# jasvob/BundleAdjustment_Benchmarks

Hardware: AMD Instinct MI355X
Metric: LM iterations/sec (higher is better)
Workload: dtype f64; 1 GPU; CHOLESKY solver, BAL problem-257-65132 (K=225911) synthetic(seed=1004), f64

## Files before the change

### bundleadjustment_benchmarks_amd/csrc/ba_internal.h

```cpp
#ifndef BA_INTERNAL_H
#define BA_INTERNAL_H

#include "../../include/ba_mi355x.h"

#include <cstdint>
#include <vector>

struct ba_problem {
    int N = 0, M = 0, K = 0;
    std::vector<int> cam_idx, pt_idx;
    std::vector<double> meas;
    std::vector<double> cams9;
    std::vector<double> pts;
};

struct ba_structure {
    int N = 0;
    int M = 0, K = 0;
    int p0 = 0, p1 = 0;
    int o0 = 0, o1 = 0;
    int Ml = 0, Kl = 0;
    bool was_sorted = true;
    std::vector<int> perm;
    std::vector<int> obs_cam, obs_pt;
    std::vector<int> pt_ptr;
    int kmax = 0;
    std::vector<int> qr_pts;
    int qr_bucket_ptr[6] = {0, 0, 0, 0, 0, 0};
    int npairs = 0;
    std::vector<int> pair_hi, pair_lo;
    long long E = 0;
    std::vector<int> ent_r, ent_c;
    int chunk_len = 64;
    int nchunks = 0;
    std::vector<int> chunk_ptr;
    std::vector<int> chunk_pair;
    std::vector<int> pair_chunk_ptr;
    int ndchunks = 0;
    std::vector<int> dchunk_ptr;
    std::vector<int> dchunk_cam;
    std::vector<int> cam_dchunk_ptr;
    std::vector<int> cam_obs;
};

int ba_build_structure(const ba_problem *p, int shard_rank, int shard_world, int chunk_len, int dchunk_len, ba_structure *out, bool pairs = true);

int ba_covisibility(int N, int M, const int *pt_ptr, const int *obs_cam, int track_max, std::vector<int> &pairs, std::vector<int> &weight);


#define BA_CHUNK 64
#define BA_CHUNK_SINGLE (1 << 16)
#define BA_SHARE_CHUNK 256
#define BA_SHARE_LOCAL 8

void ba_plan_eval_ranges(const ba_structure &s, std::vector<int> &eb);

struct ba_schur_plan {
    int grid = 1, nband = 1;
    std::vector<int> wave_ptr;
    std::vector<int> chunk_info;
    std::vector<int> ent;
    std::vector<int> red_pairs;
};
void ba_plan_schur(const ba_structure &s, int wgs_per_cu, int num_cus, int bands, int window, ba_schur_plan &out);

struct ba_forest_plan {
    int ntrees = 0, nodes = 0, kept = 0, dropped = 0, largest = 0, width = 6;
    std::vector<int> tree_ptr, node_cam, node_par ;
    std::vector<int> node_rec;
    std::vector<unsigned char> in_tree;
    std::vector<int> edge_ptr, edge_oo;
};
int ba_plan_forest(const ba_structure &s, const std::vector<int> &rp_pairs, int kind, int max_tree, ba_forest_plan &out);

struct ba_share_plan {
    int nslots = 0, nwide = 0, largest = 0;
    std::vector<int> desc;
    std::vector<int> wide;
};
void ba_plan_share_slots(int ngroups, int nchunks, const int *gptr, const int *cptr, const int *cgrp, ba_share_plan &out);

void ba_plan_relpose_csr(int N, int n, const int *pairs, std::vector<int> &ptr, std::vector<int> &inc);

size_t ba_plan_owner_offsets(int Dp, int nb, int world, std::vector<int> &off);

int ba_rccl_init(void **comm_out, const void *id128, int rank, int world);
void ba_rccl_destroy(void *comm);
int ba_rccl_allreduce(void *comm, void *buf, size_t count, int f64, int op, void *stream);
int ba_rccl_broadcast(void *comm, void *buf, size_t count, int f64, int root, void *stream);
int ba_rccl_reduce_scatter(void *comm, void *buf, size_t count_per_rank, int f64, int rank, void *stream);

#endif
```

### bundleadjustment_benchmarks_amd/csrc/ba_kernels.hip.h

```cpp
#ifndef BA_KERNELS_HIP_H
#define BA_KERNELS_HIP_H

#include <hip/hip_runtime.h>

#include "ba_internal.h"
#include "ba_mfma.hip.h"

#define BA_REC 32
#define BA_REC_DINV 27
#define BA_SLAB 96
#define BA_EPS_PSI 1e-15

__device__ __forceinline__ double tsqrt(double x) { return sqrt(x); }
__device__ __forceinline__ float tsqrt(float x) { return sqrtf(x); }
__device__ __forceinline__ double tsin(double x) { return sin(x); }
__device__ __forceinline__ float tsin(float x) { return sinf(x); }
__device__ __forceinline__ double tcos(double x) { return cos(x); }
__device__ __forceinline__ float tcos(float x) { return cosf(x); }
#ifndef BA_SENTINEL_DEFINED
#define BA_SENTINEL_DEFINED
template <typename T> __device__ __forceinline__ T ba_sentinel();
template <> __device__ __forceinline__ double ba_sentinel<double>() { return __hiloint2double(-1, -1); }
template <> __device__ __forceinline__ float ba_sentinel<float>() { return __int_as_float(-1); }
__device__ __forceinline__ bool ba_is_sentinel(double v) { return __double2hiint(v) == -1 && __double2loint(v) == -1; }
// ... 346 lines not shown
            T U[6] = {0, 0, 0, 0, 0, 0}, g[3] = {0, 0, 0};
            for (int s = 0; s < kk; s++) {
#pragma unroll
                for (int q = 0; q < 6; q++) U[q] += cu[q][tl + s];
#pragma unroll
                for (int q = 0; q < 3; q++) g[q] -= cu[6 + q][tl + s];
            }
#pragma unroll
            for (int q = 0; q < 6; q++) fa.U0[(size_t)q * Ml + pj] = U[q];
#pragma unroll
            for (int q = 0; q < 3; q++) fa.gp[(size_t)q * Ml + pj] = g[q];
            if (FUSE >= 2) {
                const ba_chol3_t<T> c3 = ba_chol3<T>(U[0], U[1], U[2], U[3], U[4], U[5], g[0], g[1], g[2], *fa.lam);
                const size_t M = (size_t)Ml;
                fa.dinv[pj] = c3.i0; fa.dinv[M + pj] = c3.i1; fa.dinv[2 * M + pj] = c3.i2;
                fa.tvec[pj] = c3.t0; fa.tvec[M + pj] = c3.t1; fa.tvec[2 * M + pj] = c3.t2;
                fa.tri[pj] = 1; fa.tri[M + pj] = c3.l10; fa.tri[2 * M + pj] = c3.l20;
                fa.tri[3 * M + pj] = 1; fa.tri[4 * M + pj] = c3.l21; fa.tri[5 * M + pj] = 1;
                pf[0][tl] = c3.l10; pf[1][tl] = c3.l20; pf[2][tl] = c3.l21; pf[3][tl] = c3.i0; pf[4][tl] = c3.i1; pf[5][tl] = c3.i2;
            }
        }
        if constexpr (FUSE >= 2) {
            __syncthreads();
            if constexpr (COOP) {
                static_assert(16 * ba_stage<T, BA_REC>::S <= 9 * 256 / 4 && 16 * ba_stage<T, 20>::S <= 9 * 256 / 4, "a wavefront's image");
                const int w0 = 64 * (tl >> 6), left = b1 - b0 - w0;
                const int nw = __builtin_amdgcn_readfirstlane(left < 0 ? 0 : left > 64 ? 64 : left);
                T *img = &cu[0][0] + (tl >> 6) * (9 * 256 / 4);
                {
                    T a[20];
#pragma unroll
                    for (int q = 0; q < 18; q++) a[q] = Aj[q];
                    a[18] = ej[0]; a[19] = ej[1];
                    ba_store_run<T, 20, 16>(img, a, nw, JcA + (size_t)(b0 + w0) * 20);
                }
                T z[BA_REC];
                if (valid) {
                    const int fl = pfirst - b0;
                    ba_chol_z<T>(Aj, Bj, pf[0][fl], pf[1][fl], pf[2][fl], pf[3][fl], pf[4][fl], pf[5][fl], z);
                }
                ba_store_run<T, BA_REC, 16>(img, z, nw, fa.rec + (size_t)(b0 + w0) * BA_REC);
            } else if (valid) {
                const int fl = pfirst - b0;
                ba_chol_record<T>(Aj, Bj, pf[0][fl], pf[1][fl], pf[2][fl], pf[3][fl], pf[4][fl], pf[5][fl], fa.rec + (size_t)i * BA_REC);
            }
            if (blockIdx.x == 0 && threadIdx.x == 0) *fa.fresh = 1;
        }
    }
}

template <typename T>
__global__ __launch_bounds__(256) void k_stats(int K, int N, int Ml, const T *__restrict__ cam, const T *__restrict__ pts,
                                               const int *__restrict__ obs_cam, const int *__restrict__ obs_pt,
                                               const T *__restrict__ meas, T tau, T *__restrict__ partial )
{
    __shared__ T red[4];
    const int i = blockIdx.x * 256 + threadIdx.x;
    T v0 = 0, v1 = 0, v2 = 0, v3 = 0;
    if (i < K) {
        const int ci = obs_cam[i], pj = obs_pt[i];
        T c[15];
#pragma unroll
        for (int k = 0; k < 15; k++) c[k] = cam[(size_t)k * N + ci];
        const T X0 = pts[pj], X1 = pts[(size_t)Ml + pj], X2 = pts[2 * (size_t)Ml + pj];
        const T XX0 = c[0] * X0 + c[1] * X1 + c[2] * X2 + c[9];
        const T XX1 = c[3] * X0 + c[4] * X1 + c[5] * X2 + c[10];
        const T XX2 = c[6] * X0 + c[7] * X1 + c[8] * X2 + c[11];
        const T xu0 = XX0 / XX2, xu1 = XX1 / XX2;
        const T r2u = xu0 * xu0 + xu1 * xu1;
        const T kr = 1 + c[13] * r2u + c[14] * r2u * r2u;
        const T d0 = c[12] * (kr * xu0) - meas[i], d1 = c[12] * (kr * xu1) - meas[(size_t)K + i];
        const T err = tsqrt(d0 * d0 + d1 * d1);
        const T tau2 = tau * tau, tau4 = tau2 * tau2;
        v0 = err;
        if (err <= tau) { v1 = err; v2 = 1; }
        const T q2 = err, q4 = q2 * q2;
        v3 = (q2 < tau2) ? q2 * ((T)3.0 - (T)3.0 * q2 / tau2 + q4 / tau4) / (T)6.0 : tau2 / (T)6.0;
    }
    v0 = block_reduce<T, false>(v0, red);
    v1 = block_reduce<T, false>(v1, red);
    v2 = block_reduce<T, false>(v2, red);
    v3 = block_reduce<T, false>(v3, red);
    if (threadIdx.x == 0) {
        const size_t g = gridDim.x;
        partial[blockIdx.x] = v0; partial[g + blockIdx.x] = v1; partial[2 * g + blockIdx.x] = v2; partial[3 * g + blockIdx.x] = v3;
    }
}

struct ba_red_job { const void *src; int n; int op; int dst; };
struct ba_red_jobs { ba_red_job j[8]; };

template <typename T> __device__ __forceinline__ void ba_reduce_job(const ba_red_job &jb, T *__restrict__ scal, T *red)
{
    const T *src = (const T *)jb.src;
    T a = 0;
    if (jb.op == 0) {
        for (int k = threadIdx.x; k < jb.n; k += 256) a += src[k];
        a = block_reduce<T, false>(a, red);
    } else {
        for (int k = threadIdx.x; k < jb.n; k += 256) a = tmax(a, src[k]);
        a = block_reduce<T, true>(a, red);
    }
    if (threadIdx.x == 0) scal[jb.dst] = a;
}

template <typename T> __global__ __launch_bounds__(256) void k_reduce_scalars(ba_red_jobs jobs, T *__restrict__ scal, const int *__restrict__ go = nullptr,
                                                                              long long *__restrict__ stamp = nullptr)
{
    __shared__ T red[4];
    if (!(go && *go == 0)) ba_reduce_job<T>(jobs.j[blockIdx.x], scal, red);
    if (stamp && blockIdx.x == 0 && threadIdx.x == 0) *stamp = (long long)wall_clock64();
}

template <typename T>
__device__ __forceinline__ void ba_point_prep_block(int bid, int Ml, int K, const int *__restrict__ pt_ptr, const T *__restrict__ Jp,
                                                    const T *__restrict__ r, T *__restrict__ U0, T *__restrict__ gp, T *__restrict__ partial_dmax)
{
    __shared__ T red[4];
    const int j = bid * 256 + threadIdx.x;
    T dm = 0;
    if (j < Ml) {
        T U[6] = {0, 0, 0, 0, 0, 0}, g[3] = {0, 0, 0};
        const int e = pt_ptr[j + 1];
        for (int i = pt_ptr[j]; i < e; i++) {
            T B[6];
#pragma unroll
            for (int q = 0; q < 6; q++) B[q] = Jp[(size_t)q * K + i];
            const T r0 = r[i], r1 = r[(size_t)K + i];
            T u[9];
            ba_pt_terms<T>(B, r0, r1, u);
#pragma unroll
            for (int q = 0; q < 6; q++) U[q] += u[q];
#pragma unroll
            for (int q = 0; q < 3; q++) g[q] -= u[6 + q];
        }
#pragma unroll
        for (int q = 0; q < 6; q++) U0[(size_t)q * Ml + j] = U[q];
#pragma unroll
        for (int q = 0; q < 3; q++) gp[(size_t)q * Ml + j] = g[q];
        dm = tmax(U[0], tmax(U[3], U[5]));
    }
    dm = block_reduce<T, true>(dm, red);
    if (threadIdx.x == 0) partial_dmax[bid] = dm;
}
template <typename T>
__global__ __launch_bounds__(256) void k_point_prep(int Ml, int K, const int *__restrict__ pt_ptr, const T *__restrict__ Jp,
                                                    const T *__restrict__ r, T *__restrict__ U0, T *__restrict__ gp,
                                                    T *__restrict__ partial_dmax, const int *__restrict__ go = nullptr)
{
    if (go && *go == 0) return;
    ba_point_prep_block<T>(blockIdx.x, Ml, K, pt_ptr, Jp, r, U0, gp, partial_dmax);
}

template <typename T>
__device__ __forceinline__ void ba_cam_gram_block(int bid, int ndchunks, int K, const int *__restrict__ dchunk_ptr, const int *__restrict__ cam_obs,
                                                  const T *__restrict__ JcA, T *__restrict__ dslab)
{
    __shared__ T xch[8][27][33];
    const int gl = threadIdx.x >> 5, g = bid * 8 + gl, sub = threadIdx.x & 31;
    const bool gok = g < ndchunks;
    const int e0 = gok ? dchunk_ptr[g] : 0, len = gok ? dchunk_ptr[g + 1] - e0 : 0;
    T v[54];
#pragma unroll
    for (int q = 0; q < 54; q++) v[q] = 0;
    if (sub < len) {
        const T *rec = JcA + (size_t)cam_obs[e0 + sub] * 20;
        T a0[9], a1[9];
#pragma unroll
        for (int c = 0; c < 9; c++) { a0[c] = rec[c]; a1[c] = rec[9 + c]; }
        const T r0 = rec[18], r1 = rec[19];
        int q = 0;
#pragma unroll
        for (int c = 0; c < 9; c++)
#pragma unroll
            for (int c2 = 0; c2 <= c; c2++) v[q++] = a0[c] * a0[c2] + a1[c] * a1[c2];
#pragma unroll
        for (int c = 0; c < 9; c++) v[45 + c] = -(a0[c] * r0 + a1[c] * r1);
    }
#pragma unroll
    for (int pass = 0; pass < 2; pass++) {
        __syncthreads();
#pragma unroll
        for (int q = 0; q < 27; q++) xch[gl][q][sub] = v[27 * pass + q];
        __syncthreads();
        if (gok && sub < 27) {
            T a = 0;
#pragma unroll
            for (int l = 0; l < 32; l++) a += xch[gl][sub][l];
            dslab[(size_t)g * BA_SLAB + 27 * pass + sub] = a;
        }
    }
}
template <typename T>
__global__ __launch_bounds__(256) void k_cam_gram(int ndchunks, int K, const int *__restrict__ dchunk_ptr,
                                                  const int *__restrict__ cam_obs, const T *__restrict__ JcA,
                                                  T *__restrict__ dslab, const int *__restrict__ go = nullptr)
{
    if (go && *go == 0) return;
    ba_cam_gram_block<T>(blockIdx.x, ndchunks, K, dchunk_ptr, cam_obs, JcA, dslab);
}
template <typename T>
__global__ __launch_bounds__(256) void k_grad_prep(int gM, int Ml, int K, const int *__restrict__ pt_ptr, const T *__restrict__ Jp, const T *__restrict__ r,
                                                   T *__restrict__ U0, T *__restrict__ gp, T *__restrict__ partial_dmax, int ndchunks,
                                                   const int *__restrict__ dchunk_ptr, const int *__restrict__ cam_obs, const T *__restrict__ JcA,
                                                   T *__restrict__ dslab, const int *__restrict__ go = nullptr)
{
    if (go && *go == 0) return;
    if ((int)blockIdx.x < gM) ba_point_prep_block<T>(blockIdx.x, Ml, K, pt_ptr, Jp, r, U0, gp, partial_dmax);
    else ba_cam_gram_block<T>(blockIdx.x - gM, ndchunks, K, dchunk_ptr, cam_obs, JcA, dslab);
}

template <typename T>
__global__ __launch_bounds__(256) void k_cam_gram_reduce(int N, const int *__restrict__ cam_dchunk_ptr,
                                                         const T *__restrict__ dslab, T *__restrict__ V ,
                                                         T *__restrict__ gc , const int *__restrict__ go = nullptr,
                                                         ba_red_job tail = ba_red_job{nullptr, 0, 0, 0}, T *__restrict__ scal = nullptr,
                                                         long long *__restrict__ stamp = nullptr)
{
    __shared__ T red[4];
    if (tail.src && blockIdx.x == gridDim.x - 1) {
        if (!(go && *go == 0)) ba_reduce_job<T>(tail, scal, red);
        if (stamp && threadIdx.x == 0) *stamp = (long long)wall_clock64();
        return;
    }
    if (go && *go == 0) return;
    const int idx = blockIdx.x * 256 + threadIdx.x;
    const int a = idx / BA_SLAB, e = idx - a * BA_SLAB;
    if (a >= N || e >= 54) return;
    T s4[4] = {0, 0, 0, 0};
    const int c0 = cam_dchunk_ptr[a], c1 = cam_dchunk_ptr[a + 1];
    int c = c0;
    for (; c + 15 < c1; c += 16) {
        T x[16];
#pragma unroll
        for (int u = 0; u < 16; u++) x[u] = dslab[(size_t)(c + u) * BA_SLAB + e];
#pragma unroll
        for (int u = 0; u < 16; u++) s4[u & 3] += x[u];
    }
    for (; c + 3 < c1; c += 4) {
#pragma unroll
        for (int u = 0; u < 4; u++) s4[u] += dslab[(size_t)(c + u) * BA_SLAB + e];
    }
    for (; c < c1; c++) s4[0] += dslab[(size_t)c * BA_SLAB + e];
    const T s = (s4[0] + s4[1]) + (s4[2] + s4[3]);
    if (e < 45) {
        int rr = 0;
        while ((rr + 1) * (rr + 2) / 2 <= e) rr++;
        const int cc = e - rr * (rr + 1) / 2;
        V[(size_t)a * 81 + 9 * rr + cc] = s;
        V[(size_t)a * 81 + 9 * cc + rr] = s;
    } else
        gc[9 * a + e - 45] = s;
}

template <typename T> __global__ __launch_bounds__(256) void k_vdiag(int N, const T *__restrict__ V, T *__restrict__ out)
{
    const int c = blockIdx.x * 256 + threadIdx.x;
    if (c < 9 * N) out[c] = V[(size_t)(c / 9) * 81 + 10 * (c % 9)];
}

template <typename T, bool MARQ = false, bool COOP = false>
__global__ __launch_bounds__(256) void k_elim_chol(int K, int Ml, const int *__restrict__ obs_pt, const int *__restrict__ pt_ptr,
                                                   const T *__restrict__ JcA , const T *__restrict__ Jp, const T *__restrict__ U0,
                                                   const T *__restrict__ gp, const T *__restrict__ lam, T *__restrict__ rec,
                                                   T *__restrict__ dinv, T *__restrict__ tvec, T *__restrict__ tri,
                                                   const int *__restrict__ fresh = nullptr ,
                                                   ba_damp_args<T> da = ba_damp_args<T>{})
{
    if (fresh && *fresh != 0) return;
    const int i0 = blockIdx.x * 256 + threadIdx.x;
    if (!COOP && i0 >= K) return;
    const int w0 = (int)blockIdx.x * 256 + (threadIdx.x & 192);
    if (COOP && w0 >= K) return;
    const bool valid = i0 < K;
    const int i = valid ? i0 : K - 1;
    const T lambda = *lam;
    const int j = obs_pt[i];
    const size_t M = (size_t)Ml;
    ba_chol3_t<T> c3;
    if constexpr (MARQ) {
        const T u0 = U0[j], u3 = U0[3 * M + j], u5 = U0[5 * M + j];
        c3 = ba_chol3<T>(u0, U0[M + j], U0[2 * M + j], u3, U0[4 * M + j], u5, gp[j], gp[M + j], gp[2 * M + j],
                         ba_damp<true, T>(lambda, u0, da), ba_damp<true, T>(lambda, u3, da), ba_damp<true, T>(lambda, u5, da));
    } else
        c3 = ba_chol3<T>(U0[j], U0[M + j], U0[2 * M + j], U0[3 * M + j], U0[4 * M + j], U0[5 * M + j],
                         gp[j], gp[M + j], gp[2 * M + j], lambda);
    if (valid && i == pt_ptr[j]) {
        dinv[j] = c3.i0; dinv[M + j] = c3.i1; dinv[2 * M + j] = c3.i2;
        tvec[j] = c3.t0; tvec[M + j] = c3.t1; tvec[2 * M + j] = c3.t2;
        tri[j] = 1; tri[M + j] = c3.l10; tri[2 * M + j] = c3.l20;
        tri[3 * M + j] = 1; tri[4 * M + j] = c3.l21; tri[5 * M + j] = 1;
    }
    T A[18], B[6];
#pragma unroll
    for (int q = 0; q < 6; q++) B[q] = Jp[(size_t)q * K + i];
    {
        typedef T vec_t __attribute__((ext_vector_type(16 / sizeof(T))));
        constexpr int VW = 16 / sizeof(T);
        const vec_t *src = (const vec_t *)(JcA + (size_t)i * 20);
#pragma unroll
        for (int q = 0; q < 20 / VW; q++) {
            const vec_t v = src[q];
#pragma unroll
            for (int u = 0; u < VW; u++)
                if (VW * q + u < 18) A[VW * q + u] = v[u];
        }
    }
    if constexpr (COOP) {
        __shared__ alignas(16) T stage[4][16 * ba_stage<T, BA_REC>::S];
        const int nw = __builtin_amdgcn_readfirstlane(K - w0 > 64 ? 64 : K - w0);
        T z[BA_REC];
        ba_chol_z<T>(A, B, c3.l10, c3.l20, c3.l21, c3.i0, c3.i1, c3.i2, z);
        ba_store_run<T, BA_REC, 16>(stage[threadIdx.x >> 6], z, nw, rec + (size_t)w0 * BA_REC);
    } else
    ba_chol_record<T>(A, B, c3.l10, c3.l20, c3.l21, c3.i0, c3.i1, c3.i2, rec + (size_t)i * BA_REC);
}

template <typename T, int LPP> __device__ __forceinline__ T group_sum(T v)
{
#pragma unroll
    for (int off = LPP / 2; off > 0; off >>= 1) v += __shfl_xor(v, off, LPP);
    return v;
}

template <typename T, int LPP, int SL>
__global__ __launch_bounds__(256) void k_elim_qr(int npts, const int *__restrict__ pt_list, int Ml, int K, const int *__restrict__ pt_ptr,
                                                 const T *__restrict__ Jc, const T *__restrict__ Jp, const T *__restrict__ r,
                                                 const T *__restrict__ lam, T *__restrict__ rec, T *__restrict__ dinv,
                                                 T *__restrict__ tvec, T *__restrict__ tri, const int *__restrict__ go = nullptr,
                                                 T *__restrict__ q1obs = nullptr ,
                                                 T *__restrict__ q1lam = nullptr ,
                                                 int *__restrict__ pperm = nullptr )
{
    if (go && *go == 0) return;
    const int gid = (blockIdx.x * 256 + threadIdx.x) / LPP, lg = threadIdx.x % LPP;
    const int j = pt_list[gid < npts ? gid : npts - 1];
    const int b = pt_ptr[j], k = pt_ptr[j + 1] - b;
    const T sl = tsqrt(*lam);
    T V[SL][6], Q[SL][6];
    bool ok[SL];
#pragma unroll
    for (int s = 0; s < SL; s++) {
// ... 154 lines not shown
        }
    }
    T Ql[3][3] = {{1, 0, 0}, {0, 1, 0}, {0, 0, 1}}, QR[3][3] = {{0, 0, 0}, {0, 0, 0}, {0, 0, 0}};
#pragma unroll
    for (int h = 2; h >= 0; h--)
#pragma unroll
        for (int c = 0; c < 3; c++) {
            const T w = (Ql[h][c] + W[h][0] * QR[0][c] + W[h][1] * QR[1][c] + W[h][2] * QR[2][c]) * tau[h];
            Ql[h][c] -= w;
#pragma unroll
            for (int r = 0; r < 3; r++) QR[r][c] -= W[h][r] * w;
        }
    const T m0 = tvec0[j], m1 = tvec0[(size_t)Ml + j], m2 = tvec0[2 * (size_t)Ml + j];
    T t[3];
#pragma unroll
    for (int c = 0; c < 3; c++) t[c] = QR[0][c] * m0 + QR[1][c] * m1 + QR[2][c] * m2;
    if (i == pt_ptr[j]) {
#pragma unroll
        for (int c = 0; c < 3; c++) { dinv[(size_t)c * Ml + j] = 1; tvec[(size_t)c * Ml + j] = t[c]; }
        tri[j] = Rt[0][0]; tri[(size_t)Ml + j] = Rt[0][1]; tri[2 * (size_t)Ml + j] = Rt[0][2];
        tri[3 * (size_t)Ml + j] = Rt[1][1]; tri[4 * (size_t)Ml + j] = Rt[1][2]; tri[5 * (size_t)Ml + j] = Rt[2][2];
        if (mQl) {
#pragma unroll
            for (int h = 0; h < 3; h++)
#pragma unroll
                for (int c = 0; c < 3; c++) { mQl[9 * (size_t)j + 3 * h + c] = Ql[h][c]; mQR[9 * (size_t)j + 3 * h + c] = QR[h][c]; }
        }
    }
    const T *z = rec0 + (size_t)i * BA_REC;
    T *o = rec + (size_t)i * BA_REC;
#pragma unroll
    for (int c = 0; c < 9; c++) {
        const T a0 = z[3 * c], a1 = z[3 * c + 1], a2 = z[3 * c + 2];
        const T z0 = a0 * QR[0][0] + a1 * QR[1][0] + a2 * QR[2][0], z1 = a0 * QR[0][1] + a1 * QR[1][1] + a2 * QR[2][1],
                z2 = a0 * QR[0][2] + a1 * QR[1][2] + a2 * QR[2][2];
        o[3 * c] = z0; o[3 * c + 1] = z1; o[3 * c + 2] = z2;
    }
    o[BA_REC_DINV] = 1; o[BA_REC_DINV + 1] = 1; o[BA_REC_DINV + 2] = 1;
}

template <typename T>
__global__ __launch_bounds__(256) void k_more_build(int K, int Ml, int D, const int *__restrict__ obs_cam, const int *__restrict__ obs_pt,
                                                    const int *__restrict__ pt_ptr, const T *__restrict__ rec0, const T *__restrict__ rec,
                                                    const T *__restrict__ mQl, const T *__restrict__ mQR, const T *__restrict__ tvec0,
                                                    const T *__restrict__ tvec, T *__restrict__ A, size_t lda)
{
    const int ia = blockIdx.x * 256 + threadIdx.x;
    if (ia >= K) return;
    const int j = obs_pt[ia], a = obs_cam[ia], b = pt_ptr[j], e = pt_ptr[j + 1];
    for (int i2 = b; i2 < ia; i2++)
        if (obs_cam[i2] == a) return;
    const size_t r0 = 6 * (size_t)j;
    T Ql[9], QR[9];
#pragma unroll
    for (int q = 0; q < 9; q++) { Ql[q] = mQl[9 * (size_t)j + q]; QR[q] = mQR[9 * (size_t)j + q]; }
    T z0[27], z[27];
#pragma unroll
    for (int q = 0; q < 27; q++) { z0[q] = rec0[(size_t)ia * BA_REC + q]; z[q] = rec[(size_t)ia * BA_REC + q]; }
    for (int i2 = ia + 1; i2 < e; i2++)
        if (obs_cam[i2] == a) {
#pragma unroll
            for (int q = 0; q < 27; q++) { z0[q] += rec0[(size_t)i2 * BA_REC + q]; z[q] += rec[(size_t)i2 * BA_REC + q]; }
        }
    T *colbase = A + (size_t)(9 * a) * lda + r0;
#pragma unroll
    for (int c = 0; c < 9; c++) {
        const T z_0 = z[3 * c], z_1 = z[3 * c + 1], z_2 = z[3 * c + 2];
#pragma unroll
        for (int rr = 0; rr < 3; rr++) {
            colbase[(size_t)c * lda + rr] = -(Ql[3 * rr] * z_0 + Ql[3 * rr + 1] * z_1 + Ql[3 * rr + 2] * z_2);
            colbase[(size_t)c * lda + 3 + rr] = z0[3 * c + rr] - (QR[3 * rr] * z_0 + QR[3 * rr + 1] * z_1 + QR[3 * rr + 2] * z_2);
        }
    }
    if (ia == pt_ptr[j]) {
        const size_t M = (size_t)Ml;
        const T m0 = tvec0[j], m1 = tvec0[M + j], m2 = tvec0[2 * M + j], t0 = tvec[j], t1 = tvec[M + j], t2 = tvec[2 * M + j];
        const T mq[3] = {m0, m1, m2};
        T *rhs = A + (size_t)D * lda + r0;
#pragma unroll
        for (int rr = 0; rr < 3; rr++) {
            rhs[rr] = -(Ql[3 * rr] * t0 + Ql[3 * rr + 1] * t1 + Ql[3 * rr + 2] * t2);
            rhs[3 + rr] = mq[rr] - (QR[3 * rr] * t0 + QR[3 * rr + 1] * t1 + QR[3 * rr + 2] * t2);
        }
    }
}
template <typename T>
__global__ __launch_bounds__(256) void k_more_tail(int Ml, int D, const T *__restrict__ R22buf, const T *__restrict__ lam, T *__restrict__ A, size_t lda)
{
    const int c = blockIdx.x;
    const size_t rR = 6 * (size_t)Ml, rL = rR + (size_t)D;
    const int top = c < D ? c : D - 1;
    for (int i = threadIdx.x; i <= top; i += 256) A[(size_t)c * lda + rR + i] = R22buf[(size_t)c * D + i];
    if (c < D && threadIdx.x == 0) A[(size_t)c * lda + rL + c] = tsqrt(*lam);
}
template <typename T>
__global__ __launch_bounds__(256) void k_copy_r22(int D, const T *__restrict__ A, size_t lda, T *__restrict__ R22buf, const int *__restrict__ go)
{
    if (go && *go == 0) return;
    const int c = blockIdx.x;
    const int top = c < D ? c : D - 1;
    for (int i = threadIdx.x; i < D; i += 256) R22buf[(size_t)c * D + i] = i <= top ? A[(size_t)c * lda + i] : (T)0;
}

template <typename T>
__global__ __launch_bounds__(256) void k_dbg_resid(int rows, int D, const T *__restrict__ A, size_t lda, const T *__restrict__ y, T *__restrict__ r)
{
    const int i = blockIdx.x * 256 + threadIdx.x;
    if (i >= rows) return;
    T a = A[(size_t)D * lda + i];
    for (int c = 0; c < D; c++) a -= A[(size_t)c * lda + i] * y[c];
    r[i] = a;
}
template <typename T>
__global__ __launch_bounds__(256) void k_dbg_atv(int rows, int D, const T *__restrict__ A, size_t lda, const T *__restrict__ v, T *__restrict__ out)
{
    __shared__ T red[4];
    const int c = blockIdx.x;
    T a = 0;
    for (int r = threadIdx.x; r < rows; r += 256) a += A[(size_t)c * lda + r] * v[r];
    a = block_reduce<T, false>(a, red);
    if (threadIdx.x == 0) out[c] = a;
}

typedef int ba_v2i __attribute__((ext_vector_type(2)));
__device__ __forceinline__ double ba_bufload(__amdgpu_buffer_rsrc_t r, unsigned off, const double *)
{
    return __builtin_bit_cast(double, __builtin_amdgcn_raw_buffer_load_b64(r, (int)off, 0, 0));
}
__device__ __forceinline__ float ba_bufload(__amdgpu_buffer_rsrc_t r, unsigned off, const float *)
{
    return __builtin_bit_cast(float, __builtin_amdgcn_raw_buffer_load_b32(r, (int)off, 0, 0));
}
typedef int ba_v4i __attribute__((ext_vector_type(4)));
__device__ __forceinline__ void ba_bufload3(__amdgpu_buffer_rsrc_t r, unsigned off, double &x0, double &x1, double &x2)
{
    const ba_v4i lo = __builtin_amdgcn_raw_buffer_load_b128(r, (int)off, 0, 0);
    const ba_v2i hi = __builtin_amdgcn_raw_buffer_load_b64(r, (int)(off + 16), 0, 0);
    x0 = __builtin_bit_cast(double, ba_v2i{lo.x, lo.y});
    x1 = __builtin_bit_cast(double, ba_v2i{lo.z, lo.w});
    x2 = __builtin_bit_cast(double, hi);
}
__device__ __forceinline__ void ba_bufload3(__amdgpu_buffer_rsrc_t r, unsigned off, float &x0, float &x1, float &x2)
{
    x0 = ba_bufload(r, off, (const float *)nullptr);
    x1 = ba_bufload(r, off + 4, (const float *)nullptr);
    x2 = ba_bufload(r, off + 8, (const float *)nullptr);
}
template <typename T, bool SCALED >
__global__ __launch_bounds__(256) __attribute__((amdgpu_waves_per_eu(4))) void k_schur_pairs(const int *__restrict__ wave_ptr, int nband, const int4 *__restrict__ chunk_info,
                                                     const int2 *__restrict__ ent, const T *__restrict__ rec, unsigned rec_bytes,
                                                     const T *__restrict__ tvec, int Ml, T *__restrict__ slab, const T *__restrict__ V,
                                                     const T *__restrict__ gc, int D, int ld, T *__restrict__ S)
{
    const int lane = threadIdx.x & 63;
    const int wq = ((blockIdx.x % nband) * (gridDim.x / nband) + blockIdx.x / nband) * 4 + (threadIdx.x >> 6);
    int slot = wave_ptr[wq];
    const int slot1 = wave_ptr[wq + 1];
    if (slot >= slot1) return;
    const __amdgpu_buffer_rsrc_t rsrc = __builtin_amdgcn_make_buffer_rsrc(const_cast<T *>(rec), 0, (int)rec_bytes, 0x00020000);
    constexpr unsigned SZ = sizeof(T), RB = BA_REC * SZ, OOB = 0xfffffff0u - 64 * SZ;
    const int i = lane & 15, k = lane >> 4;
    const bool la = i < 9;
    const unsigned lane_off = 3 * i * SZ;
    typedef typename ba_acc<T>::type acc_t;
    auto entry_of = [&](const int4 ci) {
        const int n = ci.y & 0xffff;
        return ent[ci.x + (lane < n ? lane : n - 1)];
    };
    int4 ci0 = chunk_info[slot];
    int4 ci1 = chunk_info[min(slot + 1, slot1 - 1)];
    int2 en0 = entry_of(ci0);
    for (; slot < slot1; slot++) {
        const int2 en1 = entry_of(ci1);
        const int4 ci2 = chunk_info[min(slot + 2, slot1 - 1)];
        const int n = ci0.y & 0xffff;
        const int hi = ci0.z & 0xffff, lo = (unsigned)ci0.z >> 16, g = ci0.w;
        const bool diag = hi == lo;
        const int ia_l = en0.x, ib_l = en0.y;
        acc_t acc;
#pragma unroll
        for (int v = 0; v < 4; v++) acc[v] = 0;
        constexpr int GB = 2;
        struct batch_t { T a[3 * GB], d[3 * GB], b[3 * GB]; };
        auto fetch = [&](int t0, batch_t &o) {
#pragma unroll
            for (int u = 0; u < GB; u++) {
                const int e = 4 * (t0 + u) + k;
                const bool ok = e < n;
                const int es = ok ? e : n - 1;
                const int ia = __shfl(ia_l, es, 64), ibr = __shfl(ib_l, es, 64);
                const bool self = ibr < 0;
                const unsigned ra = (unsigned)ia * RB, rb = (unsigned)(self ? ia : ibr) * RB;
                const unsigned oa = (ok && la) ? ra + lane_off : OOB, ob = (ok && la) ? rb + lane_off : OOB;
                const unsigned od = (ok && la) ? ra + BA_REC_DINV * SZ : OOB;
                ba_bufload3(rsrc, oa, o.a[3 * u], o.a[3 * u + 1], o.a[3 * u + 2]);
                if (SCALED) ba_bufload3(rsrc, od, o.d[3 * u], o.d[3 * u + 1], o.d[3 * u + 2]);
                ba_bufload3(rsrc, ob, o.b[3 * u], o.b[3 * u + 1], o.b[3 * u + 2]);
                if (diag && i == 9 && ok && self) {
#pragma unroll
                    for (int m = 0; m < 3; m++) o.b[3 * u + m] = tvec[(size_t)m * Ml + (~ibr)];
                }
            }
        };
        auto multiply = [&](const batch_t &o) {
#pragma unroll
            for (int q = 0; q < 3 * GB; q++) acc = ba_mfma(SCALED ? o.a[q] * o.d[q] : o.a[q], o.b[q], acc);
        };
        const int ngroups = (n + 3) >> 2;
        batch_t b0, b1;
        fetch(0, b0);
        for (int t0 = 0;;) {
            if (t0 + GB < ngroups) fetch(t0 + GB, b1);
            multiply(b0);
            t0 += GB;
            if (t0 >= ngroups) break;
            if (t0 + GB < ngroups) fetch(t0 + GB, b0);
            multiply(b1);
            t0 += GB;
            if (t0 >= ngroups) break;
        }
        if (ci0.y & BA_CHUNK_SINGLE) {
#pragma unroll
            for (int v = 0; v < 4; v++) {
                const int r = ba_crow<T>(k, v);
                if (r >= 9) continue;
                if (i < 9) {
                    T val = -acc[v];
                    if (diag) val += V[(size_t)hi * 81 + 9 * r + i];
                    S[(size_t)(9 * lo + i) * ld + 9 * hi + r] = val;
                } else if (i == 9 && diag) {
                    const T gg = gc[9 * hi + r];
                    S[(size_t)(9 * hi + r) * ld + D] = gg - acc[v];
                    S[(size_t)(9 * hi + r) * ld + D + 1] = gg;
                }
            }
        } else {
            T *o = slab + (size_t)g * BA_SLAB;
#pragma unroll
            for (int v = 0; v < 4; v++) {
                const int r = ba_crow<T>(k, v);
                if (r >= 9) continue;
                if (i < 9) o[9 * r + i] = acc[v];
                else if (i == 9) o[81 + r] = acc[v];
            }
        }
        ci0 = ci1; ci1 = ci2; en0 = en1;
    }
}

template <typename T, bool MARQ = false>
__global__ __launch_bounds__(192) void k_schur_reduce(int nred, const int *__restrict__ red_pairs, int D, int ld, const int *__restrict__ pair_hi,
                                                      const int *__restrict__ pair_lo, const int *__restrict__ pair_chunk_ptr,
                                                      const T *__restrict__ slab, const T *__restrict__ V,
                                                      const T *__restrict__ gc, T *__restrict__ S, const T *__restrict__ lam = nullptr,
                                                      int post_blocks = 0, int Dp = 0, T *__restrict__ gc_out = nullptr, T *__restrict__ xarm = nullptr,
                                                      ba_damp_args<T> da = ba_damp_args<T>{})
{
    if (post_blocks && blockIdx.x >= gridDim.x - post_blocks) {
        const int c = (blockIdx.x - (gridDim.x - post_blocks)) * 3 + (threadIdx.x >> 6), lane = threadIdx.x & 63;
        if (c >= Dp) return;
        T *col = S + (size_t)c * ld;
        if (lane == 0) {
            xarm[c] = ba_sentinel<T>();
            xarm[Dp + c] = ba_sentinel<T>();
            if (c < D) gc_out[c] = gc[c];
        }
        if (c < D) {
            for (int rr = D + 1 + lane; rr < Dp; rr += 64) col[rr] = 0;
        } else {
            for (int rr = c + lane; rr < Dp; rr += 64) col[rr] = (rr == c) ? (T)1 : (T)0;
        }
        return;
    }
    const int idx = blockIdx.x * 192 + threadIdx.x;
    const int q = idx / BA_SLAB, e = idx - q * BA_SLAB;
    if (q >= nred || e >= 90) return;
    const int p = red_pairs[q];
    const int hi = pair_hi[p], lo = pair_lo[p];
    if (e >= 81 && hi != lo) return;
    T s4[4] = {0, 0, 0, 0};
    const int c1 = pair_chunk_ptr[p + 1];
    int c = pair_chunk_ptr[p];
    for (; c + 15 < c1; c += 16) {
        T x[16];
#pragma unroll
        for (int u = 0; u < 16; u++) x[u] = slab[(size_t)(c + u) * BA_SLAB + e];
#pragma unroll
        for (int u = 0; u < 16; u++) s4[u & 3] += x[u];
    }
    for (; c + 3 < c1; c += 4) {
#pragma unroll
        for (int u = 0; u < 4; u++) s4[u] += slab[(size_t)(c + u) * BA_SLAB + e];
    }
    for (; c < c1; c++) s4[0] += slab[(size_t)c * BA_SLAB + e];
    const T s = (s4[0] + s4[1]) + (s4[2] + s4[3]);
    if (e < 81) {
        const int rr = e / 9, cc = e - 9 * rr;
        T v = -s;
        if (hi == lo) v += V[(size_t)hi * 81 + e];
        if constexpr (MARQ) { if (lam && hi == lo && rr == cc) v += ba_damp<true, T>(*lam, V[(size_t)hi * 81 + e], da); }
        else if (lam && hi == lo && rr == cc) v += *lam;
        S[(size_t)(9 * lo + cc) * ld + 9 * hi + rr] = v;
    } else {
        const int cc = e - 81;
        const T g = gc[9 * hi + cc];
        S[(size_t)(9 * hi + cc) * ld + D] = g - s;
        if (!lam) S[(size_t)(9 * hi + cc) * ld + D + 1] = g;
    }
}

template <typename T, bool MARQ = false>
__global__ __launch_bounds__(256) void k_post_reduce(int D, int Dp, int ld, const T *__restrict__ lam, T *__restrict__ S, T *__restrict__ gc_out,
                                                     T *__restrict__ xarm, const T *__restrict__ V = nullptr, ba_damp_args<T> da = ba_damp_args<T>{})
{
    const int c = blockIdx.x * 4 + (threadIdx.x >> 6), lane = threadIdx.x & 63;
    if (c >= Dp) return;
    T *col = S + (size_t)c * ld;
    if (lane == 0) {
        xarm[c] = ba_sentinel<T>();
        xarm[Dp + c] = ba_sentinel<T>();
    }
    if (c < D) {
        if (lane == 0) {
            col[c] += ba_damp<MARQ, T>(*lam, MARQ ? V[(size_t)(c / 9) * 81 + 10 * (c % 9)] : (T)0, da);
            gc_out[c] = col[D + 1];
        }
        for (int rr = D + 1 + lane; rr < Dp; rr += 64) col[rr] = 0;
    } else {
        for (int rr = c + lane; rr < Dp; rr += 64) col[rr] = (rr == c) ? (T)1 : (T)0;
    }
}

template <typename T, bool UNPACK>
__global__ __launch_bounds__(256) void k_pack_lower(int Dp, int ld, T *__restrict__ S, T *__restrict__ buf, size_t ntail, T *__restrict__ scal,
                                                    int eloc, int etot)
{
    if (blockIdx.x == 0 && blockIdx.y == 0 && threadIdx.x == 0) {
        if (UNPACK) scal[etot] = buf[ntail];
        else buf[ntail] = scal[eloc];
    }
    const int c = blockIdx.y;
    const int p = c >> 6, r0 = p << 6;
    const int h = Dp - r0;
    const size_t off = (size_t)64 * ((size_t)p * Dp - (size_t)32 * p * (p - 1)) + (size_t)(c - r0) * h;
    for (int r = blockIdx.x * 256 + threadIdx.x; r < h; r += gridDim.x * 256) {
        if (UNPACK) S[(size_t)c * ld + r0 + r] = buf[off + r];
        else buf[off + r] = S[(size_t)c * ld + r0 + r];
    }
}

template <typename T, bool UNPACK>
__global__ __launch_bounds__(256) void k_pack_owner(int Dp, int D, int ld, T *__restrict__ S, T *__restrict__ buf, const int *__restrict__ own_off,
                                                    int world, int rank, size_t small, T *__restrict__ scal, int eloc, int etot)
{
    const int c = blockIdx.y;
    const int p = c >> 6, r0 = p << 6;
    const int h = Dp - r0;
    if (blockIdx.x == 0 && threadIdx.x == 0) {
        if (c == 0) { if (UNPACK) scal[etot] = buf[small + D]; else buf[small + D] = scal[eloc]; }
        if (c < D) { if (UNPACK) S[(size_t)c * ld + D + 1] = buf[small + c]; else buf[small + c] = S[(size_t)c * ld + D + 1]; }
    }
    if (UNPACK && p % world != rank) return;
    const size_t off = (size_t)64 * (size_t)own_off[p] + (size_t)(c - r0) * h;
    for (int r = blockIdx.x * 256 + threadIdx.x; r < h; r += gridDim.x * 256) {
        if (UNPACK) { if (r0 + r != D + 1 || c >= D) S[(size_t)c * ld + r0 + r] = buf[off + r]; }
        else buf[off + r] = S[(size_t)c * ld + r0 + r];
    }
}

template <typename T, int NB, bool UNSTAGE>
__global__ __launch_bounds__(256) void k_panel_stage(int h, int p0, int ld, T *__restrict__ S, T *__restrict__ Wp, T *__restrict__ Winv, T *__restrict__ stage)
{
    const int y = blockIdx.y;
    if (y == 2 * NB) {
        for (int q = blockIdx.x * 256 + threadIdx.x; q < NB * NB; q += gridDim.x * 256) {
            if (UNSTAGE) Winv[q] = stage[(size_t)2 * h * NB + q]; else stage[(size_t)2 * h * NB + q] = Winv[q];
        }
        return;
    }
    const int j = y < NB ? y : y - NB;
    T *src = (y < NB ? S + (size_t)(p0 + j) * ld : Wp + (size_t)j * ld) + p0;
    T *dst = stage + (size_t)(y < NB ? 0 : h * NB) + (size_t)j * h;
    for (int r = blockIdx.x * 256 + threadIdx.x; r < h; r += gridDim.x * 256) {
        if (UNSTAGE) src[r] = dst[r]; else dst[r] = src[r];
    }
}

struct ba_cam_retract_args { int N; const void *cam, *dxc, *gc; void *cam_test, *scal; int dst; };
struct ba_fix_args { const unsigned short *cmask; const unsigned char *pfix; };
template <typename T> struct ba_damp_diag { const T *U0, *V; ba_damp_args<T> da; };
template <typename T, bool MASK = false, bool MARQ = false>
__device__ __forceinline__ void ba_retract_cams(int N, const T *__restrict__ cam, const T *__restrict__ dxc, const T *__restrict__ gc,
                                                const T *__restrict__ lam, T *__restrict__ cam_test, T *__restrict__ scal, int dst, T *red,
                                                const unsigned short *__restrict__ cmask = nullptr, ba_damp_diag<T> dg = ba_damp_diag<T>{});

template <typename T, int LPP, bool MASK = false, bool MARQ = false>
__global__ __launch_bounds__(256) void k_backsub(int Ml, const int *__restrict__ pt_ptr, const int *__restrict__ obs_cam,
                                                 const T *__restrict__ rec, const T *__restrict__ dinv, const T *__restrict__ tvec,
                                                 const T *__restrict__ tri, const T *__restrict__ dxc, const T *__restrict__ gp,
                                                 const T *__restrict__ pts, const T *__restrict__ lam, T *__restrict__ dxp, T *__restrict__ pts_test,
// ... 3 lines not shown
{
    __shared__ T red[4];
    if (cr.N > 0 && (int)blockIdx.x == npart) {
        ba_retract_cams<T, MASK, MARQ>(cr.N, (const T *)cr.cam, (const T *)cr.dxc, (const T *)cr.gc, lam, (T *)cr.cam_test, (T *)cr.scal, cr.dst, red,
                                       fx.cmask, dg);
        return;
    }
    const int gid = (blockIdx.x * 256 + threadIdx.x) / LPP, lg = threadIdx.x % LPP;
    const int j = gid < Ml ? gid : Ml - 1;
    const int b = pt_ptr[j], e = pt_ptr[j + 1];
    T s0 = 0, s1 = 0, s2 = 0;
    for (int i = b + lg; i < e; i += LPP) {
        const T *Z = rec + (size_t)i * BA_REC;
        const int ci = obs_cam[i];
        const T *dc = dxc + 9 * ci;
        const unsigned cm = MASK ? (unsigned)fx.cmask[ci] : 0u;
#pragma unroll
        for (int c = 0; c < 9; c++) {
            const T d = (MASK && ((cm >> c) & 1u)) ? (T)0 : dc[c];
            s0 += Z[3 * c] * d; s1 += Z[3 * c + 1] * d; s2 += Z[3 * c + 2] * d;
        }
    }
    s0 = group_sum<T, LPP>(s0); s1 = group_sum<T, LPP>(s1); s2 = group_sum<T, LPP>(s2);
    T rho = 0, dn = 0;
    if (gid < Ml && lg == 0 && b == e) {
        dxp[j] = 0; dxp[(size_t)Ml + j] = 0; dxp[2 * (size_t)Ml + j] = 0;
        pts_test[j] = pts[j]; pts_test[(size_t)Ml + j] = pts[(size_t)Ml + j]; pts_test[2 * (size_t)Ml + j] = pts[2 * (size_t)Ml + j];
    } else if (gid < Ml && lg == 0) {
        const T lambda = *lam;
        const T u0 = (tvec[j] - s0) * dinv[j], u1 = (tvec[(size_t)Ml + j] - s1) * dinv[(size_t)Ml + j],
                u2 = (tvec[2 * (size_t)Ml + j] - s2) * dinv[2 * (size_t)Ml + j];
        const T y2 = u2 / tri[5 * (size_t)Ml + j];
        const T y1 = (u1 - tri[4 * (size_t)Ml + j] * y2) / tri[3 * (size_t)Ml + j];
        const T y0 = (u0 - tri[(size_t)Ml + j] * y1 - tri[2 * (size_t)Ml + j] * y2) / tri[j];
        const int pp = pperm[j], q0 = pp & 3, q1 = (pp >> 2) & 3;
        T x0 = q0 == 0 ? y0 : q1 == 0 ? y1 : y2, x1 = q0 == 1 ? y0 : q1 == 1 ? y1 : y2, x2 = q0 == 2 ? y0 : q1 == 2 ? y1 : y2;
        const bool pfixed = MASK && fx.pfix[j] != 0;
        if (pfixed) { x0 = 0; x1 = 0; x2 = 0; }
        dxp[j] = x0; dxp[(size_t)Ml + j] = x1; dxp[2 * (size_t)Ml + j] = x2;
        pts_test[j] = pfixed ? pts[j] : pts[j] + x0;
        pts_test[(size_t)Ml + j] = pfixed ? pts[(size_t)Ml + j] : pts[(size_t)Ml + j] + x1;
        pts_test[2 * (size_t)Ml + j] = pfixed ? pts[2 * (size_t)Ml + j] : pts[2 * (size_t)Ml + j] + x2;
        if constexpr (MARQ) {
            const T d0 = ba_damp<true, T>(lambda, dg.U0[j], dg.da), d1 = ba_damp<true, T>(lambda, dg.U0[3 * (size_t)Ml + j], dg.da),
                    d2 = ba_damp<true, T>(lambda, dg.U0[5 * (size_t)Ml + j], dg.da);
            rho = x0 * (d0 * x0 + gp[j]) + x1 * (d1 * x1 + gp[(size_t)Ml + j]) + x2 * (d2 * x2 + gp[2 * (size_t)Ml + j]);
        } else
        rho = x0 * (lambda * x0 + gp[j]) + x1 * (lambda * x1 + gp[(size_t)Ml + j]) + x2 * (lambda * x2 + gp[2 * (size_t)Ml + j]);
        dn = x0 * x0 + x1 * x1 + x2 * x2;
    }
    rho = block_reduce<T, false>(rho, red);
    dn = block_reduce<T, false>(dn, red);
    if (threadIdx.x == 0) { partial[blockIdx.x] = rho; partial[npart + blockIdx.x] = dn; }
}

template <typename T, bool MASK, bool MARQ>
__device__ __forceinline__ void ba_retract_cams(int N, const T *__restrict__ cam, const T *__restrict__ dxc,
                                                const T *__restrict__ gc, const T *__restrict__ lam, T *__restrict__ cam_test,
                                                T *__restrict__ scal, int dst, T *red, const unsigned short *__restrict__ cmask,
                                                ba_damp_diag<T> dg)
{
    const T lambda = *lam;
    T rho = 0, dn = 0;
    for (int a = threadIdx.x; a < N; a += 256) {
        T p[9];
        const unsigned cm = MASK ? (unsigned)cmask[a] : 0u;
#pragma unroll
        for (int c = 0; c < 9; c++) {
            p[c] = dxc[9 * a + c];
            if (MASK && ((cm >> c) & 1u)) {
                p[c] = 0;
                ((T *)dxc)[9 * a + c] = 0;
            }
            if constexpr (MARQ) rho += p[c] * (ba_damp<true, T>(lambda, dg.V[(size_t)a * 81 + 10 * c], dg.da) * p[c] + gc[9 * a + c]);
            else rho += p[c] * (lambda * p[c] + gc[9 * a + c]);
            dn += p[c] * p[c];
        }
        T R0[9];
#pragma unroll
        for (int c = 0; c < 9; c++) R0[c] = cam[(size_t)c * N + a];
        const T th = tsqrt(p[3] * p[3] + p[4] * p[4] + p[5] * p[5]);
        T dR[9] = {1, 0, 0, 0, 1, 0, 0, 0, 1};
        if (th > (T)1e-6) {
            const T J[9] = {0, -p[5], p[4], p[5], 0, -p[3], -p[4], p[3], 0};
            const T c1 = tsin(th) / th, c2 = ((T)1.0 - tcos(th)) / (th * th);
#pragma unroll
            for (int rr = 0; rr < 3; rr++)
#pragma unroll
                for (int cc = 0; cc < 3; cc++) {
                    T j2 = 0;
#pragma unroll
                    for (int k = 0; k < 3; k++) j2 += J[3 * rr + k] * J[3 * k + cc];
                    dR[3 * rr + cc] = dR[3 * rr + cc] + c1 * J[3 * rr + cc] + c2 * j2;
                }
        }
        if (MASK && (cm & 0x38u)) {
#pragma unroll
            for (int c = 0; c < 9; c++) cam_test[(size_t)c * N + a] = R0[c];
        } else {
#pragma unroll
        for (int rr = 0; rr < 3; rr++)
#pragma unroll
            for (int cc = 0; cc < 3; cc++) {
                T s = 0;
#pragma unroll
                for (int k = 0; k < 3; k++) s += dR[3 * rr + k] * R0[3 * k + cc];
                cam_test[(size_t)(3 * rr + cc) * N + a] = s;
            }
        }
        if constexpr (MASK) {
#pragma unroll
            for (int c = 0; c < 9; c++) {
                if (c >= 3 && c < 6) continue;
                const size_t o = (size_t)(c < 3 ? 9 + c : 6 + c) * N + a;
                cam_test[o] = ((cm >> c) & 1u) ? cam[o] : cam[o] + p[c];
            }
        } else {
#pragma unroll
        for (int c = 0; c < 3; c++) cam_test[(size_t)(9 + c) * N + a] = cam[(size_t)(9 + c) * N + a] + p[c];
        cam_test[(size_t)12 * N + a] = cam[(size_t)12 * N + a] + p[6];
        cam_test[(size_t)13 * N + a] = cam[(size_t)13 * N + a] + p[7];
        cam_test[(size_t)14 * N + a] = cam[(size_t)14 * N + a] + p[8];
        }
    }
    rho = block_reduce<T, false>(rho, red);
    dn = block_reduce<T, false>(dn, red);
    if (threadIdx.x == 0) { scal[dst] = rho; scal[dst + 1] = dn; }
}

template <typename T, bool MASK = false, bool MARQ = false>
__global__ __launch_bounds__(256) void k_retract_cams(int N, const T *__restrict__ cam, const T *__restrict__ dxc,
                                                      const T *__restrict__ gc, const T *__restrict__ lam, T *__restrict__ cam_test,
                                                      T *__restrict__ scal, int dst, const unsigned short *__restrict__ cmask = nullptr,
                                                      ba_damp_diag<T> dg = ba_damp_diag<T>{})
{
    __shared__ T red[4];
    ba_retract_cams<T, MASK, MARQ>(N, cam, dxc, gc, lam, cam_test, scal, dst, red, cmask, dg);
}

#define BA_LM_RING 64
#define BA_DEV_FAILED (-100)
template <typename T> struct ba_lm_dev {
    T lambda, lambda_inc, energy, hist0, hist1;
    T lam_min, lam_max, tol_fun, inc_base;
    int iter, trials, fun_evals, status, stop;
    int go;
    int fresh;
    int max_iter, max_fun_ev, max_trials, deverr;
    long long t_ctl, t_end;
    int timed;
    int prev_go;
    int prev_code;
    int rec_fresh;
};
struct ba_lm_row { double iter, accepted, f, rho, lambda, lambda_used, e_test, dx_norm, trial_ticks, ctl_ticks_prev, prev_go, stop; };
struct ba_lm_host { int done, stop, status, pad; ba_lm_row rows[BA_LM_RING]; };
struct ba_lm_slots { int energy, etest, rho_p, rho_c, dn_p, dn_c, lambda, err, guard, world; };

#define BA_LM_JOBS 3
template <typename T>
__global__ __launch_bounds__(256 * BA_LM_JOBS) void k_lm_control(T *__restrict__ scal, ba_lm_dev<T> *__restrict__ lm, ba_lm_host *__restrict__ host,
                                                                 ba_lm_slots sl, ba_red_jobs jobs, int njobs)
{
    if (njobs > 0) {
        __shared__ T red[BA_LM_JOBS][4];
        const int q = threadIdx.x >> 8, t = threadIdx.x & 255;
        T a = 0;
        if (q < njobs) {
            const T *src = (const T *)jobs.j[q].src;
            for (int k = t; k < jobs.j[q].n; k += 256) a += src[k];
        }
        a = wave_reduce<T, false>(a);
        if ((t & 63) == 0) red[q][t >> 6] = a;
        __syncthreads();
        if (threadIdx.x == 0)
            for (int j = 0; j < njobs; j++) scal[jobs.j[j].dst] = ((red[j][0] + red[j][1]) + red[j][2]) + red[j][3];
    }
    if (threadIdx.x != 0) return;
    const long long now = (long long)wall_clock64();
    ba_lm_dev<T> s = *lm;
    if (s.stop) {
        if (s.go) lm->go = 0;
        return;
    }
    if (s.fresh) {
        s.energy = scal[sl.energy];
        s.fresh = 0;
        s.fun_evals++;
    }
    const T e_test = scal[sl.etest];
    const T rs = scal[sl.rho_p] + scal[sl.rho_c];
    const T dn = scal[sl.dn_p] + scal[sl.dn_c];
    s.fun_evals++;
    const int t = s.trials++;
    const T lam_used = s.lambda;
    ba_lm_row row;
    row.trial_ticks = s.timed ? (double)(now - s.t_end) : -1.0;
    row.ctl_ticks_prev = s.timed ? (double)(s.t_end - s.t_ctl) : -1.0;
    row.prev_go = s.prev_go;
    s.t_ctl = now;
    s.timed = 1;
    row.iter = s.iter; row.f = (double)s.energy; row.lambda_used = (double)lam_used; row.e_test = (double)e_test; row.dx_norm = sqrt((double)dn);
    int go = 0;
    bool failed = false;
    if (scal[sl.guard] != (T)(sl.world * s.prev_code)) {
        s.deverr = BA_DEVERR_DIVERGED;
        failed = true;
    } else if (scal[sl.err] != (T)0) {
        s.deverr = scal[sl.err] >= (T)BA_DEVERR_SWEEP ? BA_DEVERR_SWEEP : BA_DEVERR_ROW_FLAG;
        failed = true;
    }
    scal[sl.err] = 0;
    if (failed) {
        s.status = BA_DEV_FAILED;
        s.stop = 1;
        row.accepted = 0; row.rho = 0; row.lambda = (double)s.lambda;
    } else if (e_test < s.energy) {
        const T rho = (s.energy - e_test) / rs;
        const T tmv = (T)2.0 * rho - (T)1.0;
        const T mul = (T)1.0 - tmv * tmv * tmv;
        const T third = (T)1.0 / (T)3.0;
        s.lambda *= (mul > third ? mul : third);
        s.lambda = s.lambda > s.lam_min ? s.lambda : s.lam_min;
        row.accepted = 1; row.rho = (double)rho; row.lambda = (double)s.lambda;
        s.lambda_inc = s.inc_base;
        s.energy = e_test;
        if (s.iter % 2) s.hist1 = s.energy; else s.hist0 = s.energy;
        const T maxf = s.hist0 > s.hist1 ? s.hist0 : s.hist1;
        const T diff = s.energy > maxf ? s.energy - maxf : maxf - s.energy;
        if (s.iter > 2 && diff < s.tol_fun * s.energy) {
            s.status = 0;
            s.stop = 1;
        } else {
            go = 1;
            s.iter++;
            s.fresh = 1;
            if (s.iter > s.max_iter) { s.status = 3; s.stop = 1; }
            else if (s.fun_evals > s.max_fun_ev) { s.status = 2; s.stop = 1; }
        }
    } else {
        row.accepted = 0; row.rho = 0; row.lambda = (double)s.lambda;
        if (s.lambda > s.lam_max) { s.status = 1; s.stop = 1; }
        else {
            s.lambda *= s.lambda_inc;
            s.lambda_inc = sizeof(T) == 8 ? (T)pow((double)s.lambda_inc, 1.5) : (T)powf((float)s.lambda_inc, 1.5f);
        }
    }
    if (!s.stop && s.max_trials > 0 && s.trials >= s.max_trials) { s.stop = 1; s.status = -1; }
    s.go = go;
    s.prev_go = go;
    s.prev_code = (row.accepted != 0 ? 1 : 0) + 2 * (s.stop != 0 ? 1 : 0);
    scal[sl.guard] = (T)s.prev_code;
    scal[sl.lambda] = s.lambda;
    row.stop = failed ? 2.0 : (s.stop ? 1.0 : 0.0);
    s.rec_fresh = 0;
    *lm = s;
    host->rows[t % BA_LM_RING] = row;
    host->stop = s.stop;
    host->status = s.status;
    __threadfence_system();
    __hip_atomic_store(&host->done, t + 1, __ATOMIC_RELEASE, __HIP_MEMORY_SCOPE_SYSTEM);
}

__global__ void k_spin(long long ticks)
{
    const long long t0 = (long long)wall_clock64();
    while ((long long)wall_clock64() - t0 < ticks) __builtin_amdgcn_s_sleep(64);
}

template <typename T>
__global__ __launch_bounds__(256) void k_commit(int ncam, int npts, const T *__restrict__ cam_test, const T *__restrict__ pts_test,
                                                T *__restrict__ cam, T *__restrict__ pts, const int *__restrict__ go)
{
    if (go && *go == 0) return;
    const int idx = blockIdx.x * 256 + threadIdx.x;
    if (idx < ncam) cam[idx] = cam_test[idx];
    else if (idx - ncam < npts) pts[idx - ncam] = pts_test[idx - ncam];
}

#endif
```

### bundleadjustment_benchmarks_amd/csrc/ba_solver.hip

```cpp
#include "ba_internal.h"
#include "ba_kernels.hip.h"
#include "ba_dense.hip.h"
#include "ba_qr.hip.h"
#include "ba_pcg.hip.h"
#include "ba_cov.hip.h"
#include "ba_pcg_multi.hip.h"
#include "ba_pcg_share.hip.h"
#include "ba_prior.hip.h"
#include "ba_relpose.hip.h"

#include <algorithm>
#include <chrono>
#include <cmath>
#include <cstdio>
#include <cstdlib>
#include <cstring>
#include <new>
#include <numeric>
#include <string>
#include <type_traits>

#define HIPCHK(x)                                                                                   \
    do {                                                                                            \
        hipError_t e_ = (x);                                                                        \
        if (e_ != hipSuccess) {                                                                     \
            fprintf(stderr, "ba_mi355x: %s failed: %s (%s:%d)\n", #x, hipGetErrorString(e_), __FILE__, __LINE__); \
            return BA_ERR_HIP;                                                                      \
        }                                                                                           \
    } while (0)

namespace {

constexpr int NB = BA_NB;
constexpr int NAUG = 3;
constexpr int NSCAL = 24;
enum { SC_ENERGY = 0, SC_DMAX_P = 1, SC_ETEST = 2, SC_RHO_P = 3, SC_DN_P = 4,
       SC_GUARD = 5 ,
       SC_ERR = 6 ,
       SC_DMAX_C = 7, SC_ST0 = 8 , SC_LAMBDA = 12 ,
       SC_ZERO = 13 ,
       SC_ELOC = 15 ,
       SC_RHO_C = 16, SC_DN_C = 17 };
constexpr int N_STEP_SCALARS = 5;
enum { EV_T0 = 0, EV_T1, EV_T2, EV_T3, EV_T4, EV_T5, EV_T6, EV_L0, EV_L1, EV_N };
constexpr int RING_EV = 8;
constexpr int RING_NE = 6;

template <typename F> void with_flag(bool b, F &&f)
{
    if (b) f(std::bool_constant<true>{});
    else f(std::bool_constant<false>{});
}
template <typename F> void with_flags(bool a, bool b, F &&f)
{
    with_flag(a, [&](auto A) { with_flag(b, [&](auto B) { f(A, B); }); });
}
template <int V> using int_c = std::integral_constant<int, V>;

template <typename T> struct DevBuf {
    T *p = nullptr;
    size_t n = 0;
    int alloc(size_t count)
    {
        n = count;
        if (count == 0) return BA_OK;
        hipError_t e = hipMalloc((void **)&p, sizeof(T) * count);
        if (e != hipSuccess) { p = nullptr; return e == hipErrorOutOfMemory ? BA_ERR_NOMEM : BA_ERR_HIP; }
        return BA_OK;
    }
    int upload(const std::vector<T> &h)
    {
        int rc = alloc(h.size());
        if (rc) return rc;
        if (!h.empty() && hipMemcpy(p, h.data(), sizeof(T) * h.size(), hipMemcpyHostToDevice) != hipSuccess) return BA_ERR_HIP;
        return BA_OK;
    }
    int upload_ints(const std::vector<int> &h)
    {
        static_assert(sizeof(T) % sizeof(int) == 0 && std::is_trivially_copyable<T>::value, "not a record of ints");
        int rc = alloc(h.size() / (sizeof(T) / sizeof(int)));
        if (rc) return rc;
        if (!h.empty() && hipMemcpy(p, h.data(), sizeof(int) * h.size(), hipMemcpyHostToDevice) != hipSuccess) return BA_ERR_HIP;
        return BA_OK;
    }
    void release()
    {
        if (p) (void)hipFree(p);
        p = nullptr; n = 0;
    }
    void swap(DevBuf &o) { std::swap(p, o.p); std::swap(n, o.n); }
    ~DevBuf() { release(); }
};

struct SolverBase {
    virtual ~SolverBase() {}
    virtual int init(const ba_problem *p, ba_solver_kind kind, int rank, int world) = 0;
    virtual int linearize(double *energy, double *diag_max) = 0;
    virtual int try_step(double lambda, double *e_test, double *rho_scale, double *dx_norm) = 0;
    virtual int accept() = 0;
    virtual int stats(double *out4) = 0;
    virtual int get(int what, double *out, size_t n) = 0;
    virtual int set_state(const double *cam15, const double *pts) = 0;
    virtual void set_stream_hook() {}
    virtual int minimize(const ba_lm_params *lm, ba_trial_cb cb, void *user, ba_result *out) = 0;
    virtual int time_phase(int phase, int reps, double lambda, double *ms) = 0;
    virtual int selftest(int which) = 0;
    virtual int set_pcg(int max_iter, double rel_tol) = 0;
    virtual int pcg_stats(ba_pcg_stats *out, int reset) = 0;
    virtual int set_pcg_model_tol(double eta) = 0;
    virtual int pcg_stop_stats(ba_pcg_stop_stats *out, int reset) = 0;
    virtual int set_damping(int kind, double diag_min, double diag_max) = 0;
    virtual int get_damping(int *kind, double *diag_min, double *diag_max) = 0;
    virtual int set_precond(int kind, int max_tree) = 0;
    virtual int precond_info(long long *out6, int *fallback_trees) = 0;
    virtual int set_shared(const int *group_of) = 0;
    virtual int shared_info(long long *out4) = 0;
    virtual int set_constant(const unsigned short *cam_mask, const unsigned char *pt_fixed) = 0;
    virtual int set_loss(int kind, double scale) = 0;
    virtual int set_obs_weights(const double *w) = 0;
    virtual int set_priors(int type, int n, const int *ids, const double *x0, const double *info) = 0;
    virtual int prior_energy(double *out3) = 0;
    virtual int set_relposes(int n, const int *pairs, const double *R0, const double *t0, const double *Lr, const double *Lt) = 0;
    virtual int relpose_energy(double *out2) = 0;
    virtual size_t device_bytes() const = 0;
    virtual int cov_compute(double lambda) = 0;
    virtual int cov_get(int n_pairs, const int *cam_pairs, double *cam_cov, int n_pts, const int *pt_ids, double *pt_cov) = 0;
    virtual int cov_timing(double *ms4) = 0;
    virtual int cov_pcg(double lambda, int max_iter, double rel_tol, int n_pairs, const int *cam_pairs, double *cam_cov, int n_pts, const int *pt_ids,
                        double *pt_cov, ba_cov_pcg_stats *stats) = 0;
    bool poisoned = false;
    int recoveries = 0;
    ba_allreduce_fn ar_fn = nullptr;
    void *ar_user = nullptr;
    void *comm = nullptr;
    hipStream_t st = nullptr;
    bool own_stream = false;
    bool keep = false;
    ba_structure sx;
    ba_timing tm{};
    int rank = 0, world = 1;
};

template <typename T> void host_rodrigues(const T *om, T *R)
{
    const T th = std::sqrt(om[0] * om[0] + om[1] * om[1] + om[2] * om[2]);
    for (int i = 0; i < 9; i++) R[i] = (i % 4 == 0) ? (T)1 : (T)0;
    if (std::fabs(th) > (T)1e-6) {
        const T J[9] = {0, -om[2], om[1], om[2], 0, -om[0], -om[1], om[0], 0};
        T J2[9];
        for (int i = 0; i < 3; i++)
            for (int j = 0; j < 3; j++) {
                T a = 0;
                for (int k = 0; k < 3; k++) a += J[i * 3 + k] * J[k * 3 + j];
                J2[i * 3 + j] = a;
            }
        const T c1 = std::sin(th) / th, c2 = ((T)1.0 - std::cos(th)) / (th * th);
        for (int i = 0; i < 9; i++) R[i] = R[i] + c1 * J[i] + c2 * J2[i];
    }
}

template <typename T> struct Solver final : SolverBase {
    ba_solver_kind kind = BA_CHOLESKY;
    int N = 0, D = 0, Dp = 0, ld = 0, Ml = 0, Kl = 0;
    T tau = (T)0.5;
    DevBuf<int> d_obs_cam, d_obs_pt, d_pt_ptr, d_pair_hi, d_pair_lo, d_pair_chunk_ptr,
        d_dchunk_ptr, d_cam_dchunk_ptr, d_cam_obs, d_qr_pts, d_flags, d_pperm ;
    DevBuf<int4> d_chunk_info;
    DevBuf<int2> d_ent;
    DevBuf<int> d_wave_ptr;
    DevBuf<int> d_red_pairs;
    int schur_window = 0;
    int nred = 0;
    bool no_fold = false;
    bool rec_coop = true;
    int schur_grid = 1, schur_wgs = 4 , schur_bands = 8, schur_nband = 1;
    DevBuf<T> d_r, d_Jc, d_Jp, d_JcA, d_U0, d_gp, d_V, d_gc, d_rec0, d_dinv0, d_tvec0, d_tri0;
    DevBuf<T> d_cam[2], d_pts[2], d_meas, d_gcg, d_dslab, d_rec, d_dinv, d_tvec, d_tri,
        d_slab, d_S, d_pack, d_Skeep, d_Wp, d_Winv, d_dxc, d_dxp, d_part_e, d_part_pm, d_part_bs, d_part_st, d_scal;
    DevBuf<ba_lm_dev<T>> d_lm;
    DevBuf<T> d_qA, d_qtau, d_q1obs, d_q1lam;
    size_t q_lda = 0, q_tau_stride = 0;
    hipStream_t st_qr = nullptr;
    hipEvent_t ev_qr[2] = {nullptr, nullptr};
    ba_qr_side qr_side() const
    {
        ba_qr_side sd;
        sd.st2 = st_qr; sd.ev_chunk = ev_qr[0]; sd.ev_apply = ev_qr[1];
        return sd;
    }
    int q_rows = 0;
    bool more_qr_on = true;
    bool dense_qr() const { return kind == BA_QRKIT || kind == BA_QRSPQR || more_qr(); }
    bool chol_elim() const { return kind == BA_CHOLESKY || kind == BA_ITERSCHUR; }
    bool iterative() const { return kind == BA_ITERSCHUR; }
    bool more_qr() const { return kind == BA_MOREQR && more_qr_on; }
    DevBuf<T> d_mQl, d_mQR, d_R22;
    int outer_rows() const { return 2 * Kl + 3 * Ml + D; }
    int inner_rows() const { return more_qr() ? 6 * Ml + 2 * D : outer_rows(); }
    DevBuf<T> d_qB;
    size_t qb_ld() const { return (size_t)world * D + 64; }
    size_t qb_nmat() const { return qb_ld() * (size_t)(D + 1); }
    size_t qb_count() const { return qb_nmat() + (size_t)D + 1; }
    ba_lm_host *h_log = nullptr, *d_log = nullptr;
    T h_scal[NSCAL];
    T *h_lam = nullptr;
    hipGraphExec_t g_trial = nullptr, g_a = nullptr, g_b = nullptr, g_ctl = nullptr;
    bool use_graph = true;
    hipEvent_t ev[EV_N] = {};
    struct EvSlot { hipEvent_t e[RING_NE]; };
    EvSlot ring[RING_EV] = {};
    int gK = 0, gM = 0, gB = 0;
    int gE = 0;
    bool fuse = false;
    DevBuf<int> d_eb;
    bool have_step = false;
    bool step_level = false;
    int num_cus = 256;
    double wall_khz = 1e5;
    bool safe_factor = false;
    ba_ldlt_plan ldlt_plan;
    DevBuf<int> d_ldlt_jobs;
    int fault_rowflag = 0;
    double spin_next_s = 0;
    double watchdog_s = 600;

    ~Solver() override
    {
        if (poisoned) return;
        for (auto &e : ev)
            if (e) (void)hipEventDestroy(e);
        for (auto &sl : ring)
            for (auto &e : sl.e)
                if (e) (void)hipEventDestroy(e);
        drop_trial_graphs();
        if (h_lam) (void)hipHostFree(h_lam);
        if (h_log) (void)hipHostFree((void *)h_log);
        if (comm) ba_rccl_destroy(comm);
        if (own_stream && st) (void)hipStreamDestroy(st);
        if (st_qr) (void)hipStreamDestroy(st_qr);
        for (hipEvent_t e : ev_qr) if (e) (void)hipEventDestroy(e);
    }

    int init(const ba_problem *p, ba_solver_kind k, int rk, int wd) override
    {
        kind = k; rank = rk; world = wd;
        more_qr_on = !(getenv("BA_MOREQR_QR") != nullptr && atoi(getenv("BA_MOREQR_QR")) == 0);
        if (iterative() && wd > 1) return BA_ERR_ARG;
        int rc = ba_build_structure(p, rk, wd, BA_CHUNK, 32 , &sx,  !iterative());
        if (rc) return rc;
        N = p->N; D = 9 * N; Ml = sx.Ml; Kl = sx.Kl;
        Dp = ((D + NAUG + NB - 1) / NB) * NB;
        ld = Dp + 64;
        gK = (Kl + 255) / 256; gM = (Ml + 255) / 256;
        if (gK < 1) gK = 1;
        if (gM < 1) gM = 1;
        gB = (int)(((size_t)Ml * 8 + 255) / 256);
        if (gB < 1) gB = 1;
        gE = gK;
        std::vector<int> eb;
        ba_plan_eval_ranges(sx, eb);
        if (!eb.empty()) {
            gE = (int)eb.size() - 1;
            if ((rc = d_eb.upload(eb))) return rc;
            fuse = getenv("BA_NO_FUSE") == nullptr;
        }
        if (!chol_elim() && sx.kmax > 1024) return BA_ERR_ARG;
        if (!st) { HIPCHK(hipStreamCreateWithFlags(&st, hipStreamNonBlocking)); own_stream = true; }
        for (auto &e : ev) HIPCHK(hipEventCreate(&e));
        for (auto &sl : ring)
            for (auto &e : sl.e) HIPCHK(hipEventCreate(&e));
        HIPCHK(hipHostMalloc((void **)&h_lam, sizeof(T)));
        HIPCHK(hipHostMalloc((void **)&h_log, sizeof(ba_lm_host), hipHostMallocMapped | hipHostMallocCoherent));
        memset((void *)h_log, 0, sizeof(ba_lm_host));
        HIPCHK(hipHostGetDevicePointer((void **)&d_log, (void *)h_log, 0));
        use_graph = getenv("BA_NO_GRAPH") == nullptr;
        no_fold = getenv("BA_NO_FOLD") != nullptr;
        rec_coop = getenv("BA_REC_PLAIN") == nullptr;
        dbg_qrcheck = getenv("BA_DBG_QRCHECK") != nullptr;
        dist_factor = getenv("BA_DIST_FACTOR") != nullptr && atoi(getenv("BA_DIST_FACTOR")) != 0;
        if (const char *wd = getenv("BA_WATCHDOG_S")) { const double v = atof(wd); if (v > 0) watchdog_s = v; }
        {
            int dev = 0;
            hipDeviceProp_t pr;
            if (hipGetDevice(&dev) == hipSuccess && hipGetDeviceProperties(&pr, dev) == hipSuccess && pr.multiProcessorCount > 0)
                num_cus = pr.multiProcessorCount;
            int khz = 0;
            if (hipDeviceGetAttribute(&khz, hipDeviceAttributeWallClockRate, dev) == hipSuccess && khz > 0) wall_khz = khz;
        }
#define UP(buf, vec) if ((rc = buf.upload(vec))) return rc
        UP(d_obs_cam, sx.obs_cam); UP(d_obs_pt, sx.obs_pt); UP(d_pt_ptr, sx.pt_ptr); UP(d_pair_hi, sx.pair_hi);
        UP(d_pair_lo, sx.pair_lo);
        UP(d_pair_chunk_ptr, sx.pair_chunk_ptr); UP(d_dchunk_ptr, sx.dchunk_ptr); UP(d_cam_dchunk_ptr, sx.cam_dchunk_ptr);
        UP(d_cam_obs, sx.cam_obs); UP(d_qr_pts, sx.qr_pts);
#undef UP
        if (!iterative()) {
            if ((unsigned long long)Kl * BA_REC * sizeof(T) > (256ull << 20)) { schur_wgs = 2; schur_window = 1; }
            if (const char *ev = getenv("BA_SCHUR_WGS")) schur_wgs = std::max(1, std::min(8, atoi(ev)));
            if (const char *ev = getenv("BA_SCHUR_BANDS")) schur_bands = atoi(ev);
            if (const char *ev = getenv("BA_SCHUR_WINDOW")) schur_window = std::max(0, atoi(ev));
            if (N > 65535) return BA_ERR_ARG;
            if ((unsigned long long)Kl * BA_REC * sizeof(T) >= 0xf0000000ull) return BA_ERR_ARG;
            {
                int nb = 0;
                const hipError_t oe = kind == BA_CHOLESKY ? hipOccupancyMaxActiveBlocksPerMultiprocessor(&nb, k_schur_pairs<T, true>, 256, 0)
                                                          : hipOccupancyMaxActiveBlocksPerMultiprocessor(&nb, k_schur_pairs<T, false>, 256, 0);
                if (oe == hipSuccess && nb >= 1) schur_wgs = std::min(schur_wgs, nb);
            }
            ba_schur_plan sp;
            ba_plan_schur(sx, schur_wgs, num_cus, schur_bands, schur_window, sp);
            schur_grid = sp.grid; schur_nband = sp.nband;
            if ((rc = d_wave_ptr.upload(sp.wave_ptr))) return rc;
            nred = (int)sp.red_pairs.size();
            if ((rc = d_red_pairs.upload(sp.red_pairs))) return rc;
            static_assert(sizeof(int4) == 4 * sizeof(int) && sizeof(int2) == 2 * sizeof(int), "ba_schur_plan: 4 ints per chunk, 2 per entry");
            if ((rc = d_chunk_info.upload_ints(sp.chunk_info)) || (rc = d_ent.upload_ints(sp.ent))) return rc;
        }
        std::vector<T> cam((size_t)15 * N), pts((size_t)3 * (Ml > 0 ? Ml : 1)), meas((size_t)2 * (Kl > 0 ? Kl : 1));
        for (int i = 0; i < N; i++) {
            const double *c = &p->cams9[9 * (size_t)i];
            T om[3] = {(T)c[0], (T)c[1], (T)c[2]}, R[9];
            host_rodrigues<T>(om, R);
            for (int q = 0; q < 9; q++) cam[(size_t)q * N + i] = R[q];
            for (int q = 0; q < 3; q++) cam[(size_t)(9 + q) * N + i] = (T)c[3 + q];
            const T f = (T)c[6], k1 = (T)c[7], k2 = (T)c[8], f2 = f * f;
            cam[(size_t)12 * N + i] = -f / (T)1.0;
            cam[(size_t)13 * N + i] = k1 * f2;
            cam[(size_t)14 * N + i] = k2 * f2 * f2;
        }
        for (int j = 0; j < Ml; j++)
            for (int q = 0; q < 3; q++) pts[(size_t)q * Ml + j] = (T)p->pts[3 * (size_t)(sx.p0 + j) + q];
        for (int i = 0; i < Kl; i++) {
            const int src = sx.perm[sx.o0 + i];
            meas[i] = (T)p->meas[2 * (size_t)src];
            meas[(size_t)Kl + i] = (T)p->meas[2 * (size_t)src + 1];
        }
        if ((rc = d_cam[0].upload(cam)) || (rc = d_cam[1].upload(cam)) || (rc = d_pts[0].upload(pts)) ||
            (rc = d_pts[1].upload(pts)) || (rc = d_meas.upload(meas)))
            return rc;
        const size_t K1 = Kl > 0 ? Kl : 1, M1 = Ml > 0 ? Ml : 1;
#define AL(buf, n) if ((rc = buf.alloc(n))) return rc
        AL(d_r, 2 * K1); if (!chol_elim()) AL(d_Jc, 18 * K1);  AL(d_JcA, 20 * K1); AL(d_Jp, 6 * K1); AL(d_U0, 6 * M1); AL(d_gp, 3 * M1);
        AL(d_V, (size_t)81 * N); AL(d_gc, (size_t)D);
        if (kind == BA_MOREQR) { AL(d_rec0, (size_t)BA_REC * K1); AL(d_dinv0, 3 * M1); AL(d_tvec0, 3 * M1); AL(d_tri0, 6 * M1); }
        if ((rc = d_lm.alloc(1))) return rc;
        if ((rc = d_pperm.upload(std::vector<int>(M1, 0 | (1 << 2) | (2 << 4))))) return rc;
        if (dense_qr()) {
            {
                int dev = 0, lim = 0;
                HIPCHK(hipGetDevice(&dev));
                HIPCHK(hipDeviceGetAttribute(&lim, hipDeviceAttributeMaxSharedMemoryPerBlock, dev));
                if (sizeof(T) * ((size_t)D + 64 + 64 * 64) > (size_t)lim) return BA_ERR_ARG;
            }
            {
                const char *ev = getenv("BA_QR_HW_SQRT");
                const int on = ev ? atoi(ev) : 0;
                HIPCHK(hipMemcpyToSymbol(HIP_SYMBOL(ba_qr_hw_sqrt_flag), &on, sizeof(int)));
            }
            q_rows = std::max(outer_rows(), inner_rows());
            if (more_qr()) { AL(d_mQl, 9 * M1); AL(d_mQR, 9 * M1); AL(d_R22, (size_t)D * (D + 1)); }
            if (!getenv("BA_QR_ONE_STREAM")) {
                HIPCHK(hipStreamCreateWithFlags(&st_qr, hipStreamNonBlocking));
                for (auto &e : ev_qr) HIPCHK(hipEventCreateWithFlags(&e, hipEventDisableTiming));
            }
            q_lda = (size_t)q_rows + 64;
            q_tau_stride = (size_t)((std::max(q_rows, world * D) + ba_qr_cfg<T>::CH - 1) / ba_qr_cfg<T>::CH + 2) * BA_QR_PB * BA_QR_PB;
            AL(d_qA, q_lda * (size_t)(D + 1)); AL(d_qtau, BA_QR_TAU_LEVELS * q_tau_stride); AL(d_q1obs, 6 * K1); AL(d_q1lam, 9 * M1);
            if (world > 1) AL(d_qB, qb_count());
        }
        AL(d_gcg, (size_t)D); AL(d_dslab, (size_t)BA_SLAB * (sx.ndchunks > 0 ? sx.ndchunks : 1));
        AL(d_rec, (size_t)BA_REC * K1); AL(d_dinv, 3 * M1); AL(d_tvec, 3 * M1); AL(d_tri, 6 * M1);
        if (iterative()) {
            pcg_gc = (N + 255) / 256; pcg_gq = (int)(((size_t)9 * N + 255) / 256);
            if (pcg_gc < 1) pcg_gc = 1;
            if (pcg_gq < 1) pcg_gq = 1;
            AL(d_dxc, (size_t)D); AL(d_dxp, 3 * M1);
            AL(d_pcg_M, (size_t)81 * N); AL(d_pcg_b, (size_t)D); AL(d_pcg_r, (size_t)D); AL(d_pcg_z, (size_t)D); AL(d_pcg_p, (size_t)D);
            AL(d_pcg_y, (size_t)D); AL(d_pcg_w, 3 * M1);
            if ((rc = d_pcg_part.alloc((size_t)6 * pcg_gc + 2 * (size_t)pcg_gq))) return rc;
            if ((rc = d_pcg.alloc(1))) return rc;
            HIPCHK(hipMemset(d_pcg.p, 0, sizeof(ba_pcg_dev)));
        } else {
            AL(d_slab, (size_t)BA_SLAB * (sx.nchunks > 0 ? sx.nchunks : 1));
            AL(d_S, (size_t)ld * (Dp + 64)); AL(d_Wp, (size_t)ba_ldlt_wp_panels(D, NB) * ld * NB);  AL(d_Winv, (size_t)((D + NB - 1) / NB) * NB * NB); AL(d_dxc, (size_t)2 * Dp + 2 * NB);  AL(d_dxp, 3 * M1);
            if ((rc = d_flags.alloc((size_t)Dp / NB + 2))) return rc;
            ldlt_plan = ba_ldlt_make_plan(D + 1, D, NB);
            if ((rc = d_ldlt_jobs.upload(ldlt_plan.jobs))) return rc;
            ldlt_plan.d_jobs = d_ldlt_jobs.p;
        }
        AL(d_part_e, (size_t)gE); AL(d_part_pm, (size_t)gM);
        AL(d_part_bs, (size_t)2 * gB); AL(d_part_st, (size_t)4 * gK); AL(d_scal, NSCAL);
#undef AL
        if (d_S.p) HIPCHK(hipMemset(d_S.p, 0, sizeof(T) * d_S.n));
        if (d_Wp.p) HIPCHK(hipMemset(d_Wp.p, 0, sizeof(T) * d_Wp.n));
        HIPCHK(hipMemset(d_scal.p, 0, sizeof(T) * NSCAL));
        HIPCHK(hipMemset(d_dxc.p, 0, sizeof(T) * d_dxc.n));
        HIPCHK(hipMemset(d_part_bs.p, 0, sizeof(T) * d_part_bs.n));
        HIPCHK(hipMemset(d_part_e.p, 0, sizeof(T) * d_part_e.n));
        HIPCHK(hipMemset(d_part_pm.p, 0, sizeof(T) * d_part_pm.n));
        HIPCHK(hipDeviceSynchronize());
        return BA_OK;
    }

    int allreduce(void *buf, size_t count, int op)
    {
        if (world <= 1 && !comm) return BA_OK;
        if (comm) return ba_rccl_allreduce(comm, buf, count, sizeof(T) == 8, op, (void *)st);
        if (!ar_fn) return BA_ERR_COMM;
        return ar_fn(ar_user, buf, count, sizeof(T) == 8 ? BA_F64 : BA_F32, op, (void *)st) ? BA_ERR_COMM : BA_OK;
    }
    bool sharded() const { return world > 1 || comm != nullptr; }
    int bcast(void *buf, size_t count, int root)
    {
        if (world <= 1 && !comm) return BA_OK;
        if (comm) return ba_rccl_broadcast(comm, buf, count, sizeof(T) == 8, root, (void *)st);
        if (!ar_fn) return BA_ERR_COMM;
        return ar_fn(ar_user, buf, count, sizeof(T) == 8 ? BA_F64 : BA_F32, BA_OP_BCAST | (root << 8), (void *)st) ? BA_ERR_COMM : BA_OK;
    }
    int reduce_scatter(void *buf, size_t count_per_rank)
    {
        if (world <= 1 && !comm) return BA_OK;
        if (comm) return ba_rccl_reduce_scatter(comm, buf, count_per_rank, sizeof(T) == 8, rank, (void *)st);
        if (!ar_fn) return BA_ERR_COMM;
        return ar_fn(ar_user, buf, count_per_rank, sizeof(T) == 8 ? BA_F64 : BA_F32, BA_OP_REDUCE_SCATTER, (void *)st) ? BA_ERR_COMM : BA_OK;
    }

    int fetch_scalars()
    {
        HIPCHK(hipMemcpyAsync(h_scal, d_scal.p, sizeof(T) * NSCAL, hipMemcpyDeviceToHost, st));
        HIPCHK(hipStreamSynchronize(st));
        return check_device_error();
    }

    int check_device_error()
    {
        if (h_scal[SC_ERR] == (T)0) return BA_OK;
        report_device_error((int)h_scal[SC_ERR]);
        h_scal[SC_ERR] = 0;
        (void)hipMemsetAsync(d_scal.p + SC_ERR, 0, sizeof(T), st);
        return BA_ERR_HIP;
    }
    static void report_device_error(int code)
    {
        fprintf(stderr, "ba_mi355x: device error %d: %s\n", code,
                code == BA_DEVERR_DIVERGED ? "k_lm_control: the shards did not take the same accept / stop decision"
                : code >= BA_DEVERR_SWEEP  ? "k_ldlt_backflow: an unknown of the backward sweep was never published"
                                           : "k_ldlt_step: the look-ahead update of a row block was never announced");
    }

    double ev_ms(hipEvent_t a, hipEvent_t b)
    {
        float ms = 0;
        if (hipEventElapsedTime(&ms, a, b) != hipSuccess) return 0;
        return ms;
    }
    double ev_ms(int a, int b) { return ev_ms(ev[a], ev[b]); }

    void launch_eval(bool jac, int which, const int *go = nullptr, bool commit = false, bool fused = false)
    {
        const T tau2 = loss_scale * loss_scale;
        ba_fuse_args<T> fa{};
        fa.eb = d_eb.p;
        fa.pt_ptr = d_pt_ptr.p; fa.lam = d_scal.p + SC_LAMBDA; fa.U0 = d_U0.p; fa.gp = d_gp.p;
        fa.rec = d_rec.p; fa.dinv = d_dinv.p; fa.tvec = d_tvec.p; fa.tri = d_tri.p; fa.fresh = &d_lm.p->rec_fresh;
        fa.cmask = d_cmask.p; fa.pfix = d_pfix.p;
        fa.wobs = d_wobs.p; fa.loss = loss_kind; fa.lscale = loss_scale;
        const bool eval_coop = rec_coop && !(sizeof(T) == 4 && gE <= 2 * num_cus);
        auto launch = [&](auto JAC, auto FUSE, auto SOA, auto MASK, auto MODEL) {
            hipLaunchKernelGGL((k_eval<T, JAC(), FUSE(), SOA(), MASK(), MODEL()>), dim3(gE), dim3(256), 0, st, Kl, N, Ml, d_cam[which].p, d_pts[which].p,
                               d_obs_cam.p, d_obs_pt.p, d_meas.p, tau2, d_r.p, d_Jc.p, d_Jp.p, d_JcA.p, d_part_e.p, go, commit ? d_cam[0].p : (T *)nullptr,
                               commit ? d_pts[0].p : (T *)nullptr, fa);
        };
        auto linearisation = [&](auto FUSE, auto SOA) {
            with_flags(masked, model(), [&](auto MASK, auto MODEL) { launch(std::true_type{}, FUSE, SOA, MASK, MODEL); });
        };
        constexpr std::false_type aos{};
        constexpr std::true_type soa{};
        if (!jac) with_flag(model(), [&](auto MODEL) { launch(std::false_type{}, int_c<0>{}, soa, std::false_type{}, MODEL); });
        else if (chol_elim()) {
            if (!(fused && fuse)) linearisation(int_c<0>{}, aos);
            else if (eval_coop) linearisation(int_c<3>{}, aos);
            else linearisation(int_c<2>{}, aos);
        }
        else if (fused && fuse) linearisation(int_c<1>{}, soa);
        else linearisation(int_c<0>{}, soa);
    }

    void launch_grad(const int *go = nullptr, const ba_red_job *tail = nullptr, bool points = true )
    {
        if (!points) {
            if (sx.ndchunks > 0)
                hipLaunchKernelGGL((k_cam_gram<T>), dim3((sx.ndchunks + 7) / 8), dim3(256), 0, st, sx.ndchunks, Kl,
                                   d_dchunk_ptr.p, d_cam_obs.p, d_JcA.p, d_dslab.p, go);
        } else if (sx.ndchunks > 0 && gM <= 2 * num_cus && !no_fold)
            hipLaunchKernelGGL((k_grad_prep<T>), dim3(gM + (sx.ndchunks + 7) / 8), dim3(256), 0, st, gM, Ml, Kl, d_pt_ptr.p, d_Jp.p, d_r.p, d_U0.p, d_gp.p,
                               d_part_pm.p, sx.ndchunks, d_dchunk_ptr.p, d_cam_obs.p, d_JcA.p, d_dslab.p, go);
        else {
            hipLaunchKernelGGL((k_point_prep<T>), dim3(gM), dim3(256), 0, st, Ml, Kl, d_pt_ptr.p, d_Jp.p, d_r.p, d_U0.p, d_gp.p, d_part_pm.p, go);
            if (sx.ndchunks > 0)
                hipLaunchKernelGGL((k_cam_gram<T>), dim3((sx.ndchunks + 7) / 8), dim3(256), 0, st, sx.ndchunks, Kl,
                                   d_dchunk_ptr.p, d_cam_obs.p, d_JcA.p, d_dslab.p, go);
        }
        hipLaunchKernelGGL((k_cam_gram_reduce<T>), dim3((N * BA_SLAB + 255) / 256 + (tail ? 1 : 0)), dim3(256), 0, st, N, d_cam_dchunk_ptr.p,
                           d_dslab.p, d_V.p, d_gc.p, go, tail ? *tail : ba_red_job{nullptr, 0, 0, 0}, d_scal.p, tail ? &d_lm.p->t_end : (long long *)nullptr);
    }

    void launch_linearisation(int which, const int *go, bool commit, bool fused, const ba_red_job *tail, bool points)
    {
        launch_eval(true, which, go, commit, fused);
        launch_grad(go, tail, points);
        if (priors()) launch_prior(true, which, go);
        if (relposes()) launch_relpose(true, which, go);
    }

    int linearize(double *energy, double *diag_max) override
    {
        int rc;
        cov_valid = false;
        if ((rc = linearize_enqueue(diag_max != nullptr, nullptr))) return rc;
        mask_pending = false;
        if (more_qr() && (rc = more_outer_finish(nullptr))) return rc;
        if (sharded()) {
            HIPCHK(hipMemcpyAsync(d_scal.p + SC_ENERGY, d_scal.p + SC_ELOC, sizeof(T), hipMemcpyDeviceToDevice, st));
            if ((rc = allreduce(d_scal.p + SC_ENERGY, 1, 0))) return rc;
        }
        if (diag_max && (rc = allreduce(d_scal.p + SC_DMAX_P, 1, 1))) return rc;
        if ((rc = fetch_scalars())) return rc;
        HIPCHK(hipGetLastError());
        tm.linearize_ms += ev_ms(EV_L0, EV_L1);
        tm.n_linearize++;
        if (energy) *energy = (double)h_scal[SC_ENERGY];
        if (diag_max) *diag_max = std::max((double)h_scal[SC_DMAX_P], (double)h_scal[SC_DMAX_C]);
        have_lin = true;
        return BA_OK;
    }

    int linearize_enqueue(bool want_dmax, const int *go)
    {
        int rc;
        if (!go) HIPCHK(hipEventRecord(ev[EV_L0], st));
        ba_red_jobs jobs{};
        int nj = 0;
        jobs.j[nj++] = {d_part_e.p, gE + 3 * gP + 2 * gR, 0, sharded() ? SC_ELOC : SC_ENERGY};
        const bool tail = go != nullptr && !want_dmax && kind != BA_MOREQR && !priors() && !relposes();
        const bool fz = fuse && go != nullptr && !want_dmax;
        launch_linearisation(go ? 1 : 0, go, go != nullptr, fz, tail ? &jobs.j[0] : nullptr, !fz);
        if (kind == BA_MOREQR) {
            launch_elim_qr(d_scal.p + SC_ZERO, d_rec0.p, d_dinv0.p, d_tvec0.p, d_tri0.p, go,  more_qr());
            if (more_qr() && (rc = launch_more_outer(go))) return rc;
        }
        if (tail) { have_step = false; return BA_OK; }
        if (want_dmax) {
            T *tmp = d_dxc.p;
            hipLaunchKernelGGL((k_vdiag<T>), dim3((D + 255) / 256), dim3(256), 0, st, N, d_V.p, tmp);
            if ((rc = allreduce(tmp, (size_t)D, 0))) return rc;
            jobs.j[nj++] = {d_part_pm.p, gM + gP, 1, SC_DMAX_P};
            jobs.j[nj++] = {tmp, D, 1, SC_DMAX_C};
        }
        hipLaunchKernelGGL((k_reduce_scalars<T>), dim3(nj), dim3(256), 0, st, jobs, d_scal.p, go, &d_lm.p->t_end);
        if (!go) HIPCHK(hipEventRecord(ev[EV_L1], st));
        have_step = false;
        return BA_OK;
    }

    void launch_eliminate()
    {
        if (chol_elim()) {
            with_flags(marq(), rec_coop, [&](auto MARQ, auto COOP) {
                hipLaunchKernelGGL((k_elim_chol<T, MARQ(), COOP()>), dim3(gK), dim3(256), 0, st, Kl, Ml, d_obs_pt.p, d_pt_ptr.p, d_JcA.p, d_Jp.p,
                                   d_U0.p, d_gp.p, d_scal.p + SC_LAMBDA, d_rec.p, d_dinv.p, d_tvec.p, d_tri.p,
                                   fused_records() ? (const int *)&d_lm.p->rec_fresh : (const int *)nullptr, damp_args());
            });
        } else if (kind == BA_MOREQR) {
            if (Kl > 0)
                hipLaunchKernelGGL((k_more_trial<T>), dim3(gK), dim3(256), 0, st, Kl, Ml, d_obs_pt.p, d_pt_ptr.p, d_scal.p + SC_LAMBDA,
                                   d_rec0.p, d_tri0.p, d_tvec0.p, d_rec.p, d_dinv.p, d_tvec.p, d_tri.p, d_mQl.p, d_mQR.p);
        } else {
            launch_elim_qr(d_scal.p + SC_LAMBDA, d_rec.p, d_dinv.p, d_tvec.p, d_tri.p, nullptr, dense_qr());
        }
    }

    void launch_elim_qr(const T *lam, T *rec, T *dinv, T *tvec, T *tri, const int *go, bool thin_q = false)
    {
        T *qo = thin_q ? d_q1obs.p : nullptr, *ql = thin_q ? d_q1lam.p : nullptr;
#define BA_QR(B, L, SLOTS)                                                                                                       \
        if (sx.qr_bucket_ptr[B + 1] > sx.qr_bucket_ptr[B]) {                                                                   \
            const int np_ = sx.qr_bucket_ptr[B + 1] - sx.qr_bucket_ptr[B];                                                       \
            hipLaunchKernelGGL((k_elim_qr<T, L, SLOTS>), dim3(((size_t)np_ * L + 255) / 256), dim3(256), 0, st, np_,           \
                               d_qr_pts.p + sx.qr_bucket_ptr[B], Ml, Kl, d_pt_ptr.p, d_Jc.p, d_Jp.p, d_r.p, lam, rec, dinv, tvec, tri, go, qo, ql, d_pperm.p); \
        }
        BA_QR(0, 8, 4)
        BA_QR(1, 16, 4)
        BA_QR(2, 32, 4)
        BA_QR(3, 64, 4)
        BA_QR(4, 64, 16)
#undef BA_QR
    }

    bool post_folded() const { return !sharded() && nred > 0 && !no_fold; }
    bool ctl_reduces() const { return !sharded() && !no_fold; }

    void launch_schur()
    {
        const T *lamf = post_folded() ? d_scal.p + SC_LAMBDA : nullptr;
        if (sx.nchunks > 0) {
            const dim3 gp(schur_grid);
#define BA_PAIRS(SC) hipLaunchKernelGGL((k_schur_pairs<T, SC>), gp, dim3(256), 0, st, d_wave_ptr.p, schur_nband, d_chunk_info.p, d_ent.p, d_rec.p, \
                                                  (unsigned)(sizeof(T) * d_rec.n), d_tvec.p, Ml, d_slab.p, d_V.p, d_gc.p, D, ld, d_S.p)
            if (kind == BA_CHOLESKY) BA_PAIRS(true); else BA_PAIRS(false);
#undef BA_PAIRS
        }
        const int post_blocks = lamf ? (Dp + 2) / 3 : 0;
        const long long nthr = (long long)nred * BA_SLAB;
        if (nred > 0)
            with_flag(marq(), [&](auto MARQ) {
                hipLaunchKernelGGL((k_schur_reduce<T, MARQ()>), dim3((unsigned)((nthr + 191) / 192) + post_blocks), dim3(192), 0, st, nred, d_red_pairs.p, D,
                                   ld, d_pair_hi.p, d_pair_lo.p, d_pair_chunk_ptr.p, d_slab.p, d_V.p, d_gc.p, d_S.p, lamf, post_blocks, Dp, d_gcg.p, d_dxc.p,
                                   damp_args());
            });
        if (relposes())
            hipLaunchKernelGGL((k_relpose_schur<T>), dim3((unsigned)(((size_t)n_rp * 36 + 255) / 256)), dim3(256), 0, st, n_rp, (const int *)d_rp_pair.p,
                               (const T *)d_rp_rec.p, ld, d_S.p);
    }

    bool dist_factor = false;
    DevBuf<T> d_stage;
    DevBuf<int> d_own_off;
    size_t own_chunk = 0;
    bool dist_on() const { return dist_factor && sharded() && !dense_qr(); }
    int dist_setup()
    {
        if (d_own_off.p) return BA_OK;
        static_assert(NB == 64, "k_pack_owner counts its offsets in units of 64 scalars");
        std::vector<int> off;
        own_chunk = ba_plan_owner_offsets(Dp, NB, world, off);
        int rc;
        if ((rc = d_own_off.upload(off))) return rc;
        if ((rc = d_pack.alloc((size_t)world * own_chunk + (size_t)D + 2))) return rc;
        return d_stage.alloc((size_t)(2 * (size_t)ld + NB) * NB);
    }
    size_t dist_small_off() const { return (size_t)world * own_chunk; }
    int launch_dist_pack()
    {
        int rc;
        if ((rc = dist_setup())) return rc;
        HIPCHK(hipMemsetAsync(d_pack.p, 0, sizeof(T) * (size_t)world * own_chunk, st));
        const dim3 g((Dp + 255) / 256 > 8 ? 8 : (Dp + 255) / 256, Dp);
        hipLaunchKernelGGL((k_pack_owner<T, false>), g, dim3(256), 0, st, Dp, D, ld, d_S.p, d_pack.p, d_own_off.p, world, rank, dist_small_off(), d_scal.p,
                           (int)SC_ELOC, (int)SC_ENERGY);
        return BA_OK;
    }
    int launch_dist_unpack()
    {
        const dim3 g((Dp + 255) / 256 > 8 ? 8 : (Dp + 255) / 256, Dp);
        hipLaunchKernelGGL((k_pack_owner<T, true>), g, dim3(256), 0, st, Dp, D, ld, d_S.p, d_pack.p, d_own_off.p, world, rank, dist_small_off(), d_scal.p,
                           (int)SC_ELOC, (int)SC_ENERGY);
        return BA_OK;
    }
    int dist_exchange()
    {
        int rc;
        if ((rc = reduce_scatter(d_pack.p, own_chunk))) return rc;
        return allreduce(d_pack.p + dist_small_off(), (size_t)D + 1, 0);
    }
    int launch_factor_solve_dist()
    {
        const int nrows = D + 1, ncols = D, nblk = (ncols + NB - 1) / NB;
        int rc;
        for (int p = 0; p < nblk; p++) {
            const int p0 = p * NB, below = nrows - (p0 + NB), npanel = below > 0 ? (below + 63) / 64 : 1, owner = p % world;
            const int h = Dp - p0;
            T *wcol = d_Wp.p, *winv = d_Winv.p + (size_t)p * NB * NB;
            const dim3 gs((h + 255) / 256, 2 * NB + 1);
            if (owner == rank) {
                hipLaunchKernelGGL((k_ldlt_panel<T, NB>), dim3(npanel), dim3(256), 0, st, nrows, ncols, ld, p0, d_S.p, wcol, winv, (int *)nullptr, 0);
                hipLaunchKernelGGL((k_panel_stage<T, NB, false>), gs, dim3(256), 0, st, h, p0, ld, d_S.p, wcol, winv, d_stage.p);
            }
            if ((rc = bcast(d_stage.p, (size_t)(2 * h + NB) * NB, owner))) return rc;
            if (owner != rank) hipLaunchKernelGGL((k_panel_stage<T, NB, true>), gs, dim3(256), 0, st, h, p0, ld, d_S.p, wcol, winv, d_stage.p);
            const int p1 = p0 + NB;
            if (p1 < ncols) {
                const int nti = (nrows - p1 + 63) / 64, ntj = (ncols - p1 + 63) / 64;
                hipLaunchKernelGGL((k_ldlt_update<T, NB>), dim3(ntj, nti), dim3(256), 0, st, nrows, ncols, ld, p0, d_S.p, (const T *)wcol, world, rank);
            }
        }
        ba_ldlt_backsweep<T, NB>(st, D, ld, D, d_S.p, d_Winv.p, d_dxc.p, d_dxc.p + Dp,  true, num_cus, d_scal.p + SC_ERR,  true);
        return BA_OK;
    }
    void launch_factor_solve() { launch_factor(); launch_backsweep(); }

    void launch_qrkit_build()
    {
        if (more_qr()) { launch_more_build(); return; }
        (void)hipMemsetAsync(d_qA.p, 0, sizeof(T) * d_qA.n, st);
        const int nthr = std::max(Kl, D);
        hipLaunchKernelGGL((k_qrkit_build<T>), dim3((nthr + 255) / 256), dim3(256), 0, st, Kl, Ml, D, d_obs_cam.p, d_obs_pt.p, d_pt_ptr.p, d_Jc.p, d_r.p,
                           d_rec.p, d_q1obs.p, d_q1lam.p, d_tvec.p, d_scal.p + SC_LAMBDA, d_qA.p, q_lda, rank == 0 ? 1 : 0);
    }
    void launch_more_build()
    {
        (void)hipMemsetAsync(d_qA.p, 0, sizeof(T) * d_qA.n, st);
        if (Kl > 0)
            hipLaunchKernelGGL((k_more_build<T>), dim3(gK), dim3(256), 0, st, Kl, Ml, D, d_obs_cam.p, d_obs_pt.p, d_pt_ptr.p, d_rec0.p, d_rec.p, d_mQl.p, d_mQR.p,
                               d_tvec0.p, d_tvec.p, d_qA.p, q_lda);
        if (rank == 0) hipLaunchKernelGGL((k_more_tail<T>), dim3(D + 1), dim3(256), 0, st, Ml, D, d_R22.p, d_scal.p + SC_LAMBDA, d_qA.p, q_lda);
    }
    int launch_more_outer(const int *go)
    {
        (void)hipMemsetAsync(d_qA.p, 0, sizeof(T) * d_qA.n, st);
        if (Kl > 0)
            hipLaunchKernelGGL((k_qrkit_build<T>), dim3((std::max(Kl, D) + 255) / 256), dim3(256), 0, st, Kl, Ml, D, d_obs_cam.p, d_obs_pt.p, d_pt_ptr.p, d_Jc.p, d_r.p,
                               d_rec0.p, d_q1obs.p, d_q1lam.p, d_tvec0.p, d_scal.p + SC_ZERO, d_qA.p, q_lda, 0, go);
        ba_qr_side sd = qr_side();
        sd.go = go;
        ba_qr_factor<T>(st, d_qA.p, q_lda, outer_rows(), D, d_qtau.p, q_tau_stride, sd);
        if (sharded()) {
            int rc;
            if (!d_qB.p && (rc = d_qB.alloc(qb_count()))) return rc;
            HIPCHK(hipMemsetAsync(d_qB.p, 0, sizeof(T) * qb_nmat(), st));
            hipLaunchKernelGGL((k_qr_stack_pack<T>), dim3(D + 2), dim3(256), 0, st, (const T *)d_qA.p, q_lda, D, rank, d_qB.p, qb_ld(), qb_nmat(), (const T *)d_gc.p,
                               (const T *)d_scal.p, (int)SC_ELOC);
        }
        return BA_OK;
    }
    int more_outer_finish(const int *go)
    {
        if (sharded()) {
            int rc;
            if ((rc = allreduce(d_qB.p, qb_count(), 0))) return rc;
            ba_qr_side sd = qr_side();
            sd.go = go;
            ba_qr_factor<T>(st, d_qB.p, qb_ld(), world * D, D, d_qtau.p, q_tau_stride, sd);
            hipLaunchKernelGGL((k_copy_r22<T>), dim3(D + 1), dim3(256), 0, st, D, (const T *)d_qB.p, qb_ld(), d_R22.p, go);
        } else
            hipLaunchKernelGGL((k_copy_r22<T>), dim3(D + 1), dim3(256), 0, st, D, (const T *)d_qA.p, q_lda, d_R22.p, go);
        return BA_OK;
    }
    bool dbg_qrcheck = false;
    DevBuf<T> d_qAcopy, d_dbgr, d_dbg2;
    void launch_qrkit_solve()
    {
        const bool chk = dbg_qrcheck && step_level;
        if (chk) {
            if (!d_qAcopy.p) { (void)d_qAcopy.alloc(d_qA.n); (void)d_dbgr.alloc(q_lda); (void)d_dbg2.alloc((size_t)2 * D); }
            (void)hipMemcpyAsync(d_qAcopy.p, d_qA.p, sizeof(T) * d_qA.n, hipMemcpyDeviceToDevice, st);
        }
        ba_qr_solve<T>(st, d_qA.p, q_lda, inner_rows(), D, d_qtau.p, q_tau_stride, d_dxc.p, qr_side());
        if (chk) {
            const int rows = inner_rows();
            hipLaunchKernelGGL((k_dbg_resid<T>), dim3((rows + 255) / 256), dim3(256), 0, st, rows, D, (const T *)d_qAcopy.p, q_lda, (const T *)d_dxc.p, d_dbgr.p);
            hipLaunchKernelGGL((k_dbg_atv<T>), dim3(D), dim3(256), 0, st, rows, D, (const T *)d_qAcopy.p, q_lda, (const T *)d_dbgr.p, d_dbg2.p);
            hipLaunchKernelGGL((k_dbg_atv<T>), dim3(D), dim3(256), 0, st, rows, D, (const T *)d_qAcopy.p, q_lda, (const T *)(d_qAcopy.p + (size_t)D * q_lda), d_dbg2.p + D);
        }
        (void)hipMemcpyAsync(d_gcg.p, d_gc.p, sizeof(T) * (size_t)D, hipMemcpyDeviceToDevice, st);
    }
    int launch_qr_stack_pack()
    {
        int rc;
// ... 254 lines not shown
        with_flag(marq(), [&](auto MARQ) {
            hipLaunchKernelGGL((k_pcg_prec_reduce<T, MARQ()>), dim3((unsigned)(((size_t)N * BA_SLAB + 255) / 256)), dim3(256), 0, st, N, d_cam_dchunk_ptr.p,
                               d_dslab.p, d_V.p, d_gc.p, d_scal.p + SC_LAMBDA, Bm ? Bm : d_pcg_M.p, rhs ? rhs : d_pcg_b.p, gc_out ? gc_out : d_gcg.p,
                               damp_args());
        });
    }
    void launch_pcg_prep()
    {
        launch_pcg_blocks();
        if (share_on()) launch_share<false>(d_pcg_b.p);
        const bool forest = forest_on();
        if (forest) {
            if (fo.width == 9) launch_forest_edges();
            launch_forest_factor();
        }
        with_flag(forest, [&](auto FOREST) {
            hipLaunchKernelGGL((k_pcg_prec_inv<T, FOREST()>), dim3(pcg_gc), dim3(256), 0, st, N, d_pcg_M.p, d_pcg_b.p, d_dxc.p, d_pcg_r.p, d_pcg_z.p, d_pcg_p.p,
                               pcg_part_rz(), pcg_part_rr(), FOREST() ? (const unsigned char *)fo.in_tree.p : nullptr);
        });
        if (forest) launch_forest_apply<true>(pcg_part_rz() + pcg_gc);
        if (share_on()) launch_share<false>(d_pcg_z.p);
        if (qstop_on()) hipLaunchKernelGGL(k_pcg_start_q, dim3(1), dim3(256), 0, st, pcg_part_rr(), pcg_gc, d_pcg.p, d_pcg_part_s.p);
        else
        hipLaunchKernelGGL(k_pcg_start, dim3(1), dim3(256), 0, st, pcg_part_rr(), pcg_gc, d_pcg.p);
    }
    template <bool FINAL> void launch_pcg_matvec(int k, double tol2)
    {
        const T *lam = d_scal.p + SC_LAMBDA;
        if (Ml > 0)
            with_flag(!FINAL && qstop_on(), [&](auto QS) {
                if constexpr (decltype(QS)::value)
                    hipLaunchKernelGGL((k_pcg_point_q<T, 8>), dim3((unsigned)(((size_t)Ml * 8 + 255) / 256)), dim3(256), 0, st, k, Ml, d_pt_ptr.p, d_obs_cam.p,
                                       d_rec.p, d_dinv.p, d_pcg_z.p, d_pcg_p.p, pcg_part_rz(), pcg_part_rr(), pcg_gc, pcg_gz(), tol2, d_pcg.p, d_pcg_w.p,
                                       pcg_eta, (const double *)d_pcg_part_s.p);
                else
            hipLaunchKernelGGL((k_pcg_point<T, 8, FINAL>), dim3((unsigned)(((size_t)Ml * 8 + 255) / 256)), dim3(256), 0, st, k, Ml, d_pt_ptr.p, d_obs_cam.p,
                               d_rec.p, d_dinv.p, d_pcg_z.p, d_pcg_p.p, d_dxc.p, pcg_part_rz(), pcg_part_rr(), pcg_gc, pcg_gz(), tol2, d_pcg.p, d_pcg_w.p);
            });
        if (sx.ndchunks > 0)
            hipLaunchKernelGGL((k_pcg_cam_chunks<T, FINAL>), dim3((sx.ndchunks + 7) / 8), dim3(256), 0, st, sx.ndchunks, d_dchunk_ptr.p, d_cam_obs.p,
                               d_obs_pt.p, d_rec.p, Ml, d_pcg_w.p, d_dslab.p, d_pcg.p);
        with_flag(marq(), [&](auto MARQ) {
            hipLaunchKernelGGL((k_pcg_cam<T, FINAL, MARQ()>), dim3(pcg_gq), dim3(256), 0, st, k, N, d_cam_dchunk_ptr.p, d_dslab.p, d_V.p, lam, d_pcg_z.p, d_pcg_p.p,
                               d_dxc.p, d_pcg_b.p, pcg_part_rz(), pcg_gz(), d_pcg_y.p, FINAL ? pcg_part_res() : pcg_part_py(), d_pcg.p, damp_args());
        });
        if (relposes())
            hipLaunchKernelGGL((k_pcg_relpose<T, FINAL>), dim3(pcg_gq), dim3(256), 0, st, k, N, relpose_csr(), (const T *)d_pcg_z.p, (const T *)d_pcg_p.p,
                               (const T *)d_dxc.p, (const T *)d_pcg_b.p, (const double *)pcg_part_rz(), pcg_gz(), d_pcg_y.p,
                               FINAL ? pcg_part_res() : pcg_part_py(), (const ba_pcg_dev *)d_pcg.p);
        if (share_on()) {
            launch_share<!FINAL>(d_pcg_y.p);
            if (FINAL)
                hipLaunchKernelGGL((k_pcg_share_res<T>), dim3(pcg_gq), dim3(256), 0, st, N, (const T *)d_pcg_b.p, (const T *)d_pcg_y.p, pcg_part_res());
        }
    }
    void launch_pcg_solve()
    {
        const double tol2 = pcg_rel_tol * pcg_rel_tol;
        for (int k = 0; k < pcg_max_iter; k++) {
            launch_pcg_matvec<false>(k, tol2);
            with_flag(forest_on(), [&](auto FOREST) {
                if (qstop_on())
                    hipLaunchKernelGGL((k_pcg_update_q<T, FOREST()>), dim3(pcg_gc), dim3(256), 0, st, k, N, d_pcg_M.p, d_pcg_y.p, d_pcg_z.p, d_pcg_p.p,
                                       d_dxc.p, d_pcg_r.p, pcg_part_rz(), pcg_part_rr(), pcg_part_py(), pcg_gc, pcg_gz(), pcg_gq, d_pcg.p,
                                       FOREST() ? (const unsigned char *)fo.in_tree.p : nullptr, (const T *)d_pcg_b.p, d_pcg_part_s.p);
                else
                hipLaunchKernelGGL((k_pcg_update<T, FOREST()>), dim3(pcg_gc), dim3(256), 0, st, k, N, d_pcg_M.p, d_pcg_y.p, d_pcg_z.p, d_pcg_p.p, d_dxc.p,
                                   d_pcg_r.p, pcg_part_rz(), pcg_part_rr(), pcg_part_py(), pcg_gc, pcg_gz(), pcg_gq, d_pcg.p,
                                   FOREST() ? (const unsigned char *)fo.in_tree.p : nullptr);
            });
            if (forest_on()) launch_forest_apply<false>(pcg_part_rz() + (size_t)((k + 1) % 3) * pcg_gz() + pcg_gc);
            if (share_on()) launch_share<true>(d_pcg_z.p);
        }
        launch_pcg_matvec<true>(pcg_max_iter, tol2);
        if (qstop_on())
            hipLaunchKernelGGL(k_pcg_finish_q, dim3(1), dim3(256), 0, st, pcg_max_iter, pcg_part_rr(), pcg_gc, pcg_part_res(), pcg_gq, tol2, d_pcg.p,
                               step_level ? (const int *)nullptr : (const int *)&d_lm.p->stop, (const double *)d_pcg_part_s.p);
        else
        hipLaunchKernelGGL(k_pcg_finish, dim3(1), dim3(256), 0, st, pcg_max_iter, pcg_part_rr(), pcg_gc, pcg_part_res(), pcg_gq, tol2, d_pcg.p,
                           step_level ? (const int *)nullptr : (const int *)&d_lm.p->stop);
    }
    int set_pcg(int max_iter, double rel_tol) override
    {
        if (!iterative() || max_iter < 1 || !(rel_tol > 0 && rel_tol < 1)) return BA_ERR_ARG;
        pcg_max_iter = max_iter; pcg_rel_tol = rel_tol;
        if (g_trial) { (void)hipGraphExecDestroy(g_trial); g_trial = nullptr; }
        return BA_OK;
    }
    int set_pcg_model_tol(double eta) override
    {
        if (!iterative() || !(eta >= 0 && eta < 1)) return BA_ERR_ARG;
        if (eta > 0 && !d_pcg_part_s.p) {
            HIPCHK(hipStreamSynchronize(st));
            int rc;
            if ((rc = d_pcg_part_s.alloc((size_t)3 * pcg_gc))) { d_pcg_part_s.release(); return rc; }
            HIPCHK(hipMemset(d_pcg_part_s.p, 0, sizeof(double) * d_pcg_part_s.n));
        }
        if (eta != pcg_eta && g_trial) { (void)hipGraphExecDestroy(g_trial); g_trial = nullptr; }
        pcg_eta = eta;
        return BA_OK;
    }
    int pcg_stop_stats(ba_pcg_stop_stats *out, int reset) override
    {
        if (!iterative()) return BA_ERR_ARG;
        ba_pcg_dev h{};
        HIPCHK(hipStreamSynchronize(st));
        HIPCHK(hipMemcpy(&h, d_pcg.p, sizeof h, hipMemcpyDeviceToHost));
        if (out) {
            out->by_residual = h.by_residual; out->by_model = h.by_model; out->at_cap = h.at_cap;
            out->last_rule = h.last_rule; out->last_zeta = h.last_zeta; out->last_model = h.last_model;
        }
        if (reset) {
            h.by_residual = 0; h.by_model = 0; h.at_cap = 0; h.last_rule = 0; h.last_zeta = 0; h.last_model = 0;
            HIPCHK(hipMemcpy(d_pcg.p, &h, sizeof h, hipMemcpyHostToDevice));
        }
        return BA_OK;
    }
    int damp_kind = BA_DAMP_IDENTITY;
    double damp_min = BA_DAMP_DIAG_MIN_DEFAULT, damp_max = BA_DAMP_DIAG_MAX_DEFAULT;
    bool damp_off = false;
    bool marq() const { return damp_kind == BA_DAMP_MARQUARDT && !damp_off; }
    ba_damp_args<T> damp_args() const { return ba_damp_args<T>{(T)damp_min, (T)damp_max}; }
    ba_damp_diag<T> damp_diag() const { return ba_damp_diag<T>{(const T *)d_U0.p, (const T *)d_V.p, damp_args()}; }
    struct DampOff {
        bool &f, was;
        explicit DampOff(bool &flag) : f(flag), was(flag) { f = true; }
        ~DampOff() { f = was; }
    };
    int set_damping(int k, double dmin, double dmax) override
    {
        if (k == BA_DAMP_IDENTITY) {
            if (damp_kind != k) drop_trial_graphs();
            damp_kind = k;
            return BA_OK;
        }
        if (k != BA_DAMP_MARQUARDT || !chol_elim() || sharded()) return BA_ERR_ARG;
        if (dmin == 0) dmin = BA_DAMP_DIAG_MIN_DEFAULT;
        if (dmax == 0) dmax = BA_DAMP_DIAG_MAX_DEFAULT;
        const T tmin_ = (T)dmin, tmax_ = (T)dmax;
        if (!(tmin_ > 0) || !(tmin_ <= tmax_) || !std::isfinite((double)tmin_) || !std::isfinite((double)tmax_)) return BA_ERR_ARG;
        drop_trial_graphs();
        damp_kind = k; damp_min = (double)tmin_; damp_max = (double)tmax_;
        return BA_OK;
    }
    int get_damping(int *k, double *dmin, double *dmax) override
    {
        if (k) *k = damp_kind;
        if (dmin) *dmin = damp_min;
        if (dmax) *dmax = damp_max;
        return BA_OK;
    }
    void drop_trial_graphs()
    {
        for (hipGraphExec_t *g : {&g_trial, &g_a, &g_b, &g_ctl})
            if (*g) { (void)hipGraphExecDestroy(*g); *g = nullptr; }
    }
    int pcg_stats(ba_pcg_stats *out, int reset) override
    {
        if (!iterative()) return BA_ERR_ARG;
        ba_pcg_dev h{};
        HIPCHK(hipStreamSynchronize(st));
        HIPCHK(hipMemcpy(&h, d_pcg.p, sizeof h, hipMemcpyDeviceToHost));
        if (out) {
            out->solves = h.solves; out->total_iters = h.total_iters; out->last_iters = h.last_iters;
            out->last_converged = h.last_converged; out->last_rel_residual = h.last_rel_residual;
        }
        if (reset) {
            h.solves = 0; h.total_iters = 0; h.last_iters = 0; h.last_converged = 0; h.last_rel_residual = 0;
            HIPCHK(hipMemcpy(d_pcg.p, &h, sizeof h, hipMemcpyHostToDevice));
        }
        return BA_OK;
    }
    template <typename B> static size_t bytes_of(const B &b) { return b.p ? sizeof(*b.p) * b.n : 0; }
    size_t device_bytes() const override
    {
        size_t n = 0;
        for (const auto *b : {&d_obs_cam, &d_obs_pt, &d_pt_ptr, &d_pair_hi, &d_pair_lo, &d_pair_chunk_ptr, &d_dchunk_ptr, &d_cam_dchunk_ptr, &d_cam_obs,
                              &d_qr_pts, &d_flags, &d_ldlt_jobs, &d_pperm, &d_wave_ptr, &d_red_pairs, &d_eb, &d_own_off})
            n += bytes_of(*b);
        for (const auto *b : {&d_r, &d_Jc, &d_Jp, &d_JcA, &d_U0, &d_gp, &d_V, &d_gc, &d_rec0, &d_dinv0, &d_tvec0, &d_tri0, &d_cam[0], &d_cam[1],
                              &d_pts[0], &d_pts[1], &d_meas, &d_gcg, &d_dslab, &d_rec, &d_dinv, &d_tvec, &d_tri, &d_slab, &d_S, &d_pack, &d_Skeep,
                              &d_Wp, &d_Winv, &d_dxc, &d_dxp, &d_part_e, &d_part_pm, &d_part_bs, &d_part_st, &d_scal, &d_qA, &d_qtau, &d_q1obs,
                              &d_q1lam, &d_mQl, &d_mQR, &d_R22, &d_qB, &d_qAcopy, &d_dbgr, &d_dbg2, &d_stage, &d_pcg_M, &d_pcg_b, &d_pcg_r,
                              &d_pcg_z, &d_pcg_p, &d_pcg_y, &d_pcg_w})
            n += bytes_of(*b);
        return n + bytes_of(d_chunk_info) + bytes_of(d_ent) + bytes_of(d_lm) + bytes_of(d_pcg_part) + bytes_of(d_pcg_part_s) + bytes_of(d_pcg) + bytes_of(d_cmask) +
               bytes_of(d_pfix) + bytes_of(d_cov) + bytes_of(d_cov_flag) + mc_bytes() + bytes_of(d_wobs) + prior_bytes() + relpose_bytes() + fo.bytes() + sh.bytes();
    }

    DevBuf<T> d_cov;
    DevBuf<int> d_cov_flag;
    bool cov_valid = false;
    bool have_lin = false;
    double cov_lambda = 0, cov_ms[4] = {0, 0, 0, 0};
    int cov_ld() const { return ((Dp + D + NAUG + NB - 1) / NB) * NB + 64; }
    size_t cov_nmat() const { return (size_t)cov_ld() * (Dp + 64); }
    T *cov_wp() const { return d_cov.p + cov_nmat(); }
    T *cov_winv() const { return cov_wp() + (size_t)cov_ld() * NB; }
    T *cov_dv() const { return cov_winv() + (size_t)((D + NB - 1) / NB) * NB * NB; }
    T *cov_sc() const { return cov_dv() + Dp; }
    T *cov_dxsave() const { return cov_sc() + Dp; }
    size_t cov_count() const { return cov_nmat() + (size_t)cov_ld() * NB + (size_t)((D + NB - 1) / NB) * NB * NB + 2 * (size_t)Dp + d_dxc.n; }

    void launch_cov_eliminate(int *flag)
    {
        launch_eliminate();
        if (masked && d_pfix.p)
            hipLaunchKernelGGL((k_cov_fixed_records<T>), dim3((std::max(Kl, Ml) + 255) / 256), dim3(256), 0, st, Kl, Ml, (int)BA_REC, (const int *)d_obs_pt.p,
                               (const unsigned char *)d_pfix.p, d_rec.p, d_dinv.p, d_tvec.p, d_tri.p);
        if (Ml <= 0) return;
        if (priors())
            hipLaunchKernelGGL((k_cov_points_check_u0<T>), dim3(gM), dim3(256), 0, st, Ml, (const T *)d_U0.p, (const unsigned char *)d_pfix.p,
                               (const T *)(d_scal.p + SC_LAMBDA), flag);
        else
            hipLaunchKernelGGL((k_cov_points_check<T>), dim3(gM), dim3(256), 0, st, Ml, Kl, (const int *)d_pt_ptr.p, (const T *)d_Jp.p,
                               (const unsigned char *)d_pfix.p, (const T *)(d_scal.p + SC_LAMBDA), flag);
    }
    bool cov_request_ok(int n_pairs, const int *cam_pairs, const double *cam_cov, int n_pts, const int *pt_ids, const double *pt_cov) const
    {
        if (n_pairs < 0 || n_pts < 0 || (n_pairs > 0 && (!cam_pairs || !cam_cov)) || (n_pts > 0 && (!pt_ids || !pt_cov))) return false;
        for (int q = 0; q < 2 * n_pairs; q++)
            if (cam_pairs[q] < 0 || cam_pairs[q] >= N) return false;
        for (int q = 0; q < n_pts; q++)
            if (pt_ids[q] < 0 || pt_ids[q] >= Ml) return false;
        return true;
    }

    int cov_compute(double lambda) override
    {
        if constexpr (!std::is_same<T, double>::value) return BA_ERR_ARG;
        else {
            if ((kind != BA_CHOLESKY && kind != BA_QRCHOL) || sharded() || !have_lin || mask_pending || !(lambda >= 0) || !std::isfinite(lambda))
                return BA_ERR_ARG;
            const DampOff identity(damp_off);
            cov_valid = false;
            int rc;
            if (!d_cov.p) {
                if ((rc = d_cov.alloc(cov_count())) || (rc = d_cov_flag.alloc(1))) {
                    (void)hipGetLastError();
                    d_cov.release(); d_cov_flag.release();
                    return rc;
                }
            }
            const int ldc = cov_ld();
            int flag = 0;
            HIPCHK(hipMemsetAsync(d_cov_flag.p, 0, sizeof(int), st));
            if ((rc = set_lambda((T)lambda))) return rc;
            HIPCHK(hipEventRecord(ev[EV_T0], st));
            HIPCHK(hipMemcpyAsync(cov_dxsave(), d_dxc.p, sizeof(T) * d_dxc.n, hipMemcpyDeviceToDevice, st));
            launch_cov_eliminate(d_cov_flag.p);
            launch_schur();
            launch_post_reduce();
            HIPCHK(hipMemcpyAsync(d_dxc.p, cov_dxsave(), sizeof(T) * d_dxc.n, hipMemcpyDeviceToDevice, st));
            HIPCHK(hipMemsetAsync(d_cov.p, 0, sizeof(T) * cov_nmat(), st));
            hipLaunchKernelGGL((k_cov_scale<T>), dim3((D + 255) / 256), dim3(256), 0, st, D, ld, (const T *)d_S.p, (const unsigned short *)d_cmask.p,
                               cov_sc(), d_cov_flag.p);
            hipLaunchKernelGGL((k_cov_stage<T>), dim3(((D + NB - 1) / NB) * NB), dim3(256), 0, st, D, Dp, ld, (const T *)d_S.p, (const T *)cov_sc(), ldc, d_cov.p);
            HIPCHK(hipEventRecord(ev[EV_T1], st));
            HIPCHK(hipMemcpyAsync(&flag, d_cov_flag.p, sizeof(int), hipMemcpyDeviceToHost, st));
            HIPCHK(hipStreamSynchronize(st));
            if (flag) return BA_ERR_SINGULAR;
            ba_ldlt_factor<T, NB>(st, Dp + D, ((D + NB - 1) / NB) * NB , ldc, d_cov.p, cov_wp(), cov_winv(), (int *)nullptr, 0, (T *)nullptr,  true, 0);
            HIPCHK(hipEventRecord(ev[EV_T2], st));
            hipLaunchKernelGGL((k_cov_diag<T>), dim3((Dp + 255) / 256), dim3(256), 0, st, D, Dp, ldc, (const T *)d_cov.p, (const T *)cov_sc(), cov_dv(), d_cov_flag.p);
            const int nt = (D + 63) / 64;
            hipLaunchKernelGGL((k_cov_syrk<T>), dim3(nt * (nt + 1) / 2), dim3(256), 0, st, D, Dp, ldc, d_cov.p, (const T *)cov_dv());
            HIPCHK(hipEventRecord(ev[EV_T3], st));
            HIPCHK(hipMemcpyAsync(&flag, d_cov_flag.p, sizeof(int), hipMemcpyDeviceToHost, st));
            HIPCHK(hipStreamSynchronize(st));
            HIPCHK(hipGetLastError());
            cov_ms[0] = ev_ms(EV_T0, EV_T1); cov_ms[1] = ev_ms(EV_T1, EV_T2); cov_ms[2] = ev_ms(EV_T2, EV_T3);
            if (flag) return BA_ERR_SINGULAR;
            cov_lambda = lambda;
            cov_valid = true;
            return BA_OK;
        }
    }

    int cov_get(int n_pairs, const int *cam_pairs, double *cam_cov, int n_pts, const int *pt_ids, double *pt_cov) override
    {
        if constexpr (!std::is_same<T, double>::value) return BA_ERR_ARG;
        else {
            if (!cov_valid || !cov_request_ok(n_pairs, cam_pairs, cam_cov, n_pts, pt_ids, pt_cov)) return BA_ERR_ARG;
            const int ldc = cov_ld();
            int rc;
            HIPCHK(hipStreamSynchronize(st));
            if (n_pairs > 0) {
                DevBuf<int> d_idx;
                DevBuf<double> d_out;
                if ((rc = d_idx.alloc((size_t)2 * n_pairs)) || (rc = d_out.alloc((size_t)81 * n_pairs))) { (void)hipGetLastError(); return rc; }
                HIPCHK(hipMemcpy(d_idx.p, cam_pairs, sizeof(int) * 2 * (size_t)n_pairs, hipMemcpyHostToDevice));
                hipLaunchKernelGGL((k_cov_get_cams<T>), dim3((unsigned)(((size_t)81 * n_pairs + 255) / 256)), dim3(256), 0, st, n_pairs, (const int *)d_idx.p, ldc,
                                   (const T *)d_cov.p, (const unsigned short *)d_cmask.p, d_out.p);
                HIPCHK(hipStreamSynchronize(st));
                HIPCHK(hipMemcpy(cam_cov, d_out.p, sizeof(double) * 81 * (size_t)n_pairs, hipMemcpyDeviceToHost));
            }
            if (n_pts > 0) {
                DevBuf<int> d_idx;
                DevBuf<double> d_out;
                if ((rc = d_idx.alloc((size_t)n_pts)) || (rc = d_out.alloc((size_t)9 * n_pts))) { (void)hipGetLastError(); return rc; }
                HIPCHK(hipMemcpy(d_idx.p, pt_ids, sizeof(int) * (size_t)n_pts, hipMemcpyHostToDevice));
                HIPCHK(hipEventRecord(ev[EV_T4], st));
                if (priors())
                    hipLaunchKernelGGL((k_cov_points_u0<T, true>), dim3(n_pts), dim3(64), 0, st, n_pts, (const int *)d_idx.p, Kl, (const int *)d_pt_ptr.p,
                                       (const int *)d_obs_cam.p, (const T *)d_JcA.p, (const T *)d_Jp.p, (const unsigned char *)d_pfix.p, (T)cov_lambda, ldc,
                                       (const T *)d_cov.p, d_out.p, (const T *)d_U0.p, Ml);
                else if (chol_elim())
// ... 365 lines not shown
            if ((rc = nlone.upload(lone))) { (void)hipGetLastError(); return rc; }
        }
        if (n > 0) {
            std::vector<int> hid(ids, ids + n);
            std::vector<T> hx((size_t)3 * n), hi((size_t)ni * n);
            for (size_t q = 0; q < hx.size(); q++) hx[q] = (T)x0[q];
            for (size_t q = 0; q < hi.size(); q++) hi[q] = (T)info[q];
            if ((rc = nid.upload(hid)) || (rc = nx0.upload(hx)) || (rc = ninfo.upload(hi))) { (void)hipGetLastError(); return rc; }
        }
        if (gp_new != gP) {
            if ((rc = npe.alloc((size_t)gE + 3 * (size_t)gp_new + 2 * (size_t)gR)) || (rc = npm.alloc((size_t)gM + gp_new)) ||
                (rc = npr.alloc(3 * (size_t)gp_new))) { (void)hipGetLastError(); return rc; }
            HIPCHK(hipMemset(npe.p, 0, sizeof(T) * npe.n));
            HIPCHK(hipMemset(npm.p, 0, sizeof(T) * npm.n));
            if (npr.p) HIPCHK(hipMemset(npr.p, 0, sizeof(T) * npr.n));
            d_part_e.swap(npe); d_part_pm.swap(npm); d_part_pr.swap(npr);
            gP = gp_new;
        }
        d_pr_id[type].swap(nid); d_pr_x0[type].swap(nx0); d_pr_info[type].swap(ninfo);
        if (type == 0) d_pr_lonely.swap(nlone);
        n_pr[type] = n;
        return model_changed();
    }
    int kept_energy(const T *part, int q, int g, double *out)
    {
        if (!chol_elim() || sharded() || !have_lin || mask_pending) return BA_ERR_ARG;
        std::vector<T> h;
        int rc;
        if (g > 0 && (rc = dl(part, (size_t)q * g, h))) return rc;
        for (int r = 0; r < q; r++) {
            T a = 0;
            for (int b = 0; b < g; b++) a += h[(size_t)r * g + b];
            out[r] = (double)a;
        }
        return BA_OK;
    }
    int prior_energy(double *out3) override { return kept_energy(d_part_pr.p, 3, gP, out3); }

    DevBuf<int> d_rp_pair, d_rp_ptr, d_rp_inc;
    DevBuf<T> d_rp_R0, d_rp_t0, d_rp_Lr, d_rp_Lt, d_rp_rec, d_part_rp;
    int n_rp = 0, gR = 0;
    bool relposes() const { return n_rp > 0; }
    size_t relpose_bytes() const
    {
        return bytes_of(d_rp_pair) + bytes_of(d_rp_ptr) + bytes_of(d_rp_inc) + bytes_of(d_rp_R0) + bytes_of(d_rp_t0) + bytes_of(d_rp_Lr) +
               bytes_of(d_rp_Lt) + bytes_of(d_rp_rec) + bytes_of(d_part_rp);
    }
    ba_relpose_csr<T> relpose_csr() const { return ba_relpose_csr<T>{d_rp_ptr.p, d_rp_inc.p, d_rp_pair.p, d_rp_rec.p}; }
    void launch_relpose(bool lin, int which, const int *go)
    {
        ba_relpose_args<T> ra{n_rp, d_rp_pair.p, d_rp_R0.p, d_rp_t0.p, d_rp_Lr.p, d_rp_Lt.p};
        with_flags(lin, masked && d_cmask.p, [&](auto LIN, auto MASKED) {
            hipLaunchKernelGGL((k_relpose<T, LIN(), LIN() && MASKED()>), dim3(gR), dim3(256), 0, st, ra, N, (const T *)d_cam[which].p, d_rp_rec.p,
                               d_part_e.p + gE + 3 * gP, d_part_rp.p, go, (const unsigned short *)d_cmask.p);
        });
        if (!lin) return;
        hipLaunchKernelGGL((k_relpose_gather<T>), dim3((unsigned)(((size_t)N * BA_RP_ENT + 255) / 256)), dim3(256), 0, st, N, relpose_csr(), d_V.p, d_gc.p, go);
    }
    int set_relposes(int n, const int *pairs, const double *R0, const double *t0, const double *Lr, const double *Lt) override
    {
        if (!chol_elim() || sharded() || n < 0 || (n > 0 && (!pairs || !R0 || !t0 || !Lr || !Lt))) return BA_ERR_ARG;
        {
            std::vector<long long> seen;
            seen.reserve((size_t)n);
            for (int q = 0; q < n; q++) {
                const int a = pairs[2 * q], b = pairs[2 * q + 1];
                if (a < 0 || b < 0 || a >= N || b >= N || a == b) return BA_ERR_ARG;
                seen.push_back((long long)std::max(a, b) * N + std::min(a, b));
            }
            std::sort(seen.begin(), seen.end());
            if (std::adjacent_find(seen.begin(), seen.end()) != seen.end()) return BA_ERR_ARG;
        }
        auto finite = [](const double *v, size_t cnt) {
            for (size_t q = 0; q < cnt; q++)
                if (!std::isfinite(v[q]) || !std::isfinite((T)v[q])) return false;
            return true;
        };
        if (n > 0 && !(finite(R0, (size_t)9 * n) && finite(t0, (size_t)3 * n) && finite(Lr, (size_t)9 * n) && finite(Lt, (size_t)9 * n))) return BA_ERR_ARG;
        for (int q = 0; q < n; q++) {
            const double *R = R0 + 9 * (size_t)q;
            double dev = 0;
            for (int i = 0; i < 3; i++)
                for (int j = 0; j < 3; j++)
                    dev = std::max(dev, std::fabs(R[3 * i] * R[3 * j] + R[3 * i + 1] * R[3 * j + 1] + R[3 * i + 2] * R[3 * j + 2] - (i == j ? 1.0 : 0.0)));
            const double det = R[0] * (R[4] * R[8] - R[5] * R[7]) - R[1] * (R[3] * R[8] - R[5] * R[6]) + R[2] * (R[3] * R[7] - R[4] * R[6]);
            if (!(dev <= 1e-6) || !(det > 0)) return BA_ERR_ARG;
        }
        HIPCHK(hipStreamSynchronize(st));
        const int gr_new = (n + 255) / 256;
        int rc;
        DevBuf<int> npair, nptr, ninc;
        DevBuf<T> nR0, nt0, nLr, nLt, nrec, npe, npr;
        if (n > 0) {
            std::vector<int> hp(pairs, pairs + 2 * (size_t)n), ptr, inc;
            ba_plan_relpose_csr(N, n, pairs, ptr, inc);
            auto conv = [](const double *v, size_t cnt) { std::vector<T> h(cnt); for (size_t q = 0; q < cnt; q++) h[q] = (T)v[q]; return h; };
            if ((rc = npair.upload(hp)) || (rc = nptr.upload(ptr)) || (rc = ninc.upload(inc)) || (rc = nR0.upload(conv(R0, (size_t)9 * n))) ||
                (rc = nt0.upload(conv(t0, (size_t)3 * n))) || (rc = nLr.upload(conv(Lr, (size_t)9 * n))) || (rc = nLt.upload(conv(Lt, (size_t)9 * n))) ||
                (rc = nrec.alloc((size_t)BA_RP_REC * n))) { (void)hipGetLastError(); return rc; }
            HIPCHK(hipMemset(nrec.p, 0, sizeof(T) * nrec.n));
        }
        std::vector<int> new_pairs(pairs, pairs + 2 * (size_t)n);
        Forest nf;
        if (iterative() && (rc = build_forest(new_pairs, precond_kind, precond_max_tree, nf))) return rc;
        if (gr_new != gR) {
            if ((rc = npe.alloc((size_t)gE + 3 * (size_t)gP + 2 * (size_t)gr_new)) || (rc = npr.alloc(2 * (size_t)gr_new))) { (void)hipGetLastError(); return rc; }
            HIPCHK(hipMemset(npe.p, 0, sizeof(T) * npe.n));
            if (npr.p) HIPCHK(hipMemset(npr.p, 0, sizeof(T) * npr.n));
            d_part_e.swap(npe); d_part_rp.swap(npr);
            gR = gr_new;
        }
        d_rp_pair.swap(npair); d_rp_ptr.swap(nptr); d_rp_inc.swap(ninc); d_rp_R0.swap(nR0); d_rp_t0.swap(nt0);
        d_rp_Lr.swap(nLr); d_rp_Lt.swap(nLt); d_rp_rec.swap(nrec);
        n_rp = n;
        fo.swap(nf);
        h_rp_pair.swap(new_pairs);
        return model_changed();
    }
    int relpose_energy(double *out2) override { return kept_energy(d_part_rp.p, 2, gR, out2); }

    ba_red_jobs test_energy_jobs() const
    {
        ba_red_jobs jobs{};
        jobs.j[0] = {d_part_e.p, gE + 3 * gP + 2 * gR, 0, SC_ETEST};
        jobs.j[1] = {d_part_bs.p, gB, 0, SC_RHO_P};
        jobs.j[2] = {d_part_bs.p + gB, gB, 0, SC_DN_P};
        return jobs;
    }
    void launch_test_energy(bool reduce = true)
    {
        launch_eval(false, 1);
        if (priors()) launch_prior(false, 1, nullptr);
        if (relposes()) launch_relpose(false, 1, nullptr);
        if (reduce) hipLaunchKernelGGL((k_reduce_scalars<T>), dim3(3), dim3(256), 0, st, test_energy_jobs(), d_scal.p, (const int *)nullptr);
    }

    size_t pack_count() const
    {
        const int nbc = Dp / NB;
        return (size_t)64 * ((size_t)nbc * Dp - (size_t)32 * nbc * (nbc - 1));
    }
    int launch_pack(bool unpack)
    {
        const size_t npk = pack_count();
        int rc;
        if (!d_pack.p && (rc = d_pack.alloc(npk + 1))) return rc;
        const dim3 gpk((Dp + 255) / 256 > 8 ? 8 : (Dp + 255) / 256, Dp);
        with_flag(unpack, [&](auto UNPACK) {
            hipLaunchKernelGGL((k_pack_lower<T, UNPACK()>), gpk, dim3(256), 0, st, Dp, ld, d_S.p, d_pack.p, npk, d_scal.p, (int)SC_ELOC, (int)SC_ENERGY);
        });
        return BA_OK;
    }

    void launch_assemble() { if (dense_qr()) launch_qrkit_build(); else launch_schur(); }
    int mark(int e) { if (step_level) HIPCHK(hipEventRecord(ev[e], st)); return BA_OK; }
    int launch_seg_a()
    {
        int rc;
        launch_eliminate();
        if ((rc = mark(EV_T1))) return rc;
        if (iterative()) { launch_pcg_prep(); return mark(EV_T2); }
        launch_assemble();
        if ((rc = mark(EV_T2))) return rc;
        if (dense_qr()) return sharded() ? launch_qr_stack_pack() : BA_OK;
        if (dist_on()) return launch_dist_pack();
        return sharded() ? launch_pack(false) : BA_OK;
    }
    int launch_seg_b()
    {
        int rc;
        if (dist_on()) { if ((rc = launch_dist_unpack())) return rc; }
        else if (sharded() && !dense_qr() && (rc = launch_pack(true))) return rc;
        if ((rc = mark(EV_T3))) return rc;
        if (iterative()) launch_pcg_solve();
        else if (dense_qr()) { if (sharded()) launch_qr_stack_solve(); else launch_qrkit_solve(); }
        else {
            launch_post_reduce();
            if (keep && step_level) {
                if (!d_Skeep.p && (rc = d_Skeep.alloc(d_S.n))) return rc;
                HIPCHK(hipMemcpyAsync(d_Skeep.p, d_S.p, sizeof(T) * d_S.n, hipMemcpyDeviceToDevice, st));
            }
            if (dist_on()) { if ((rc = launch_factor_solve_dist())) return rc; }
            else launch_factor_solve();
        }
        if ((rc = mark(EV_T4))) return rc;
        launch_backsub_retract();
        if (d_pr_lonely.n > 0) {
            with_flag(masked, [&](auto MASKED) {
                const unsigned char *pfix = MASKED() ? (const unsigned char *)d_pfix.p : nullptr;
                if (marq())
                    hipLaunchKernelGGL((k_prior_lonely_marq<T, MASKED()>), dim3(1), dim3(256), 0, st, (int)d_pr_lonely.n, (const int *)d_pr_lonely.p, Ml,
                                       (const T *)d_U0.p, (const T *)d_gp.p, (const T *)(d_scal.p + SC_LAMBDA), (const T *)d_pts[0].p, d_dxp.p, d_pts[1].p,
                                       d_part_bs.p, gB, pfix, damp_args());
                else
                    hipLaunchKernelGGL((k_prior_lonely<T, MASKED()>), dim3(1), dim3(256), 0, st, (int)d_pr_lonely.n, (const int *)d_pr_lonely.p, Ml,
                                       (const T *)d_U0.p, (const T *)d_gp.p, (const T *)(d_scal.p + SC_LAMBDA), (const T *)d_pts[0].p, d_dxp.p, d_pts[1].p,
                                       d_part_bs.p, gB, pfix);
            });
        }
        if ((rc = mark(EV_T5))) return rc;
        launch_test_energy(step_level || !ctl_reduces());
        return BA_OK;
    }
    int exchange() { return dist_on() ? dist_exchange() : allreduce(xchg_ptr(), xchg_count(), 0); }
    int launch_seg_ctl()
    {
        ba_lm_slots sl{SC_ENERGY, SC_ETEST, SC_RHO_P, SC_RHO_C, SC_DN_P, SC_DN_C, SC_LAMBDA, SC_ERR, SC_GUARD, world};
        hipLaunchKernelGGL((k_lm_control<T>), dim3(1), dim3(256 * BA_LM_JOBS), 0, st, d_scal.p, d_lm.p, d_log, sl, test_energy_jobs(), ctl_reduces() ? 3 : 0);
        int rc = linearize_enqueue(false, &d_lm.p->go);
        if (!rc && more_qr() && !sharded()) rc = more_outer_finish(&d_lm.p->go);
        return rc;
    }

    int try_step(double lambda_d, double *e_test, double *rho_scale, double *dx_norm) override
    {
        int rc;
        if (mask_pending) return BA_ERR_ARG;
        if ((rc = set_lambda((T)lambda_d))) return rc;
        HIPCHK(hipEventRecord(ev[EV_T0], st));
        step_level = true;
        if (!(rc = launch_seg_a()) && !(rc = exchange())) rc = launch_seg_b();
        step_level = false;
        if (rc) return rc;
        HIPCHK(hipEventRecord(ev[EV_T6], st));
        if ((rc = allreduce(d_scal.p + SC_ETEST, N_STEP_SCALARS, 0))) return rc;
        if ((rc = fetch_scalars())) return rc;
        HIPCHK(hipGetLastError());
        tm.eliminate_ms += ev_ms(EV_T0, EV_T1);
        tm.schur_ms += ev_ms(EV_T1, EV_T2);
        if (sharded()) tm.comm_ms += ev_ms(EV_T2, EV_T3);
        tm.factor_ms += ev_ms(EV_T3, EV_T4);
        tm.backsub_ms += ev_ms(EV_T4, EV_T5);
        tm.test_eval_ms += ev_ms(EV_T5, EV_T6);
        tm.trial_ms += ev_ms(EV_T0, EV_T6);
        tm.n_trials++;
        if (e_test) *e_test = (double)h_scal[SC_ETEST];
        if (rho_scale) *rho_scale = (double)(h_scal[SC_RHO_P] + h_scal[SC_RHO_C]);
        if (dx_norm) *dx_norm = std::sqrt((double)(h_scal[SC_DN_P] + h_scal[SC_DN_C]));
        have_step = true;
        return BA_OK;
    }

    int accept() override
    {
        if (!have_step) return BA_ERR_ARG;
        cov_valid = false;
        const int ncam = 15 * N, npts = 3 * Ml;
        hipLaunchKernelGGL((k_commit<T>), dim3((ncam + npts + 255) / 256), dim3(256), 0, st, ncam, npts, d_cam[1].p, d_pts[1].p, d_cam[0].p, d_pts[0].p,
                           (const int *)nullptr);
        HIPCHK(hipStreamSynchronize(st));
        have_step = false;
        return BA_OK;
    }

    int stats(double *out4) override
    {
        hipLaunchKernelGGL((k_stats<T>), dim3(gK), dim3(256), 0, st, Kl, N, Ml, d_cam[0].p, d_pts[0].p, d_obs_cam.p,
                           d_obs_pt.p, d_meas.p, tau, d_part_st.p);
        ba_red_jobs jobs{};
        for (int q = 0; q < 4; q++) jobs.j[q] = {d_part_st.p + (size_t)q * gK, gK, 0, SC_ST0 + q};
        hipLaunchKernelGGL((k_reduce_scalars<T>), dim3(4), dim3(256), 0, st, jobs, d_scal.p);
        int rc;
        if ((rc = allreduce(d_scal.p + SC_ST0, 4, 0))) return rc;
        if ((rc = fetch_scalars())) return rc;
        const double K = (double)sx.K;
        out4[0] = (double)(h_scal[SC_ST0] / (T)K);
        out4[1] = (double)(h_scal[SC_ST0 + 1] / h_scal[SC_ST0 + 2]);
        out4[2] = (double)h_scal[SC_ST0 + 2];
        out4[3] = (double)h_scal[SC_ST0 + 3];
        return BA_OK;
    }

    int dl(const T *src, size_t n, std::vector<T> &h)
    {
        h.resize(n);
        HIPCHK(hipStreamSynchronize(st));
        if (n) HIPCHK(hipMemcpy(h.data(), src, sizeof(T) * n, hipMemcpyDeviceToHost));
        return BA_OK;
    }

    static void soa_to_aos(const std::vector<T> &h, size_t n, int Q, double *out)
    {
        for (size_t i = 0; i < n; i++)
            for (int q = 0; q < Q; q++) out[Q * i + q] = h[q * n + i];
    }
    static std::vector<T> aos_to_soa(const double *in, size_t n, int Q)
    {
        std::vector<T> h(Q * n);
        for (size_t i = 0; i < n; i++)
            for (int q = 0; q < Q; q++) h[q * n + i] = (T)in[Q * i + q];
        return h;
    }

    int get(int what, double *out, size_t n) override
    {
        std::vector<T> h, h2;
        int rc;
        switch (what) {
        case BA_GET_RESIDUALS: {
            if (n != 2 * (size_t)Kl) return BA_ERR_ARG;
            if ((rc = dl(d_r.p, 2 * (size_t)Kl, h))) return rc;
            for (int i = 0; i < Kl; i++) { out[2 * (size_t)i] = h[i]; out[2 * (size_t)i + 1] = h[(size_t)Kl + i]; }
            return BA_OK;
        }
        case BA_GET_JC: {
            if (n != 18 * (size_t)Kl) return BA_ERR_ARG;
            if (chol_elim()) {
                if ((rc = dl(d_JcA.p, 20 * (size_t)Kl, h))) return rc;
                for (int i = 0; i < Kl; i++)
                    for (int q = 0; q < 18; q++) out[18 * (size_t)i + q] = h[20 * (size_t)i + q];
                return BA_OK;
            }
            if ((rc = dl(d_Jc.p, 18 * (size_t)Kl, h))) return rc;
            for (int i = 0; i < Kl; i++)
                for (int q = 0; q < 18; q++) out[18 * (size_t)i + q] = h[(size_t)q * Kl + i];
            return BA_OK;
        }
        case BA_GET_JP: {
            if (n != 6 * (size_t)Kl) return BA_ERR_ARG;
            if ((rc = dl(d_Jp.p, 6 * (size_t)Kl, h))) return rc;
            soa_to_aos(h, Kl, 6, out);
            return BA_OK;
        }
        case BA_GET_GRAD:
        case BA_GET_DX: {
            const bool grad = what == BA_GET_GRAD;
            if (n != 3 * (size_t)Ml + D) return BA_ERR_ARG;
            if ((rc = dl(grad ? d_gp.p : d_dxp.p, 3 * (size_t)Ml, h)) || (rc = dl(grad ? d_gc.p : d_dxc.p, D, h2))) return rc;
            soa_to_aos(h, Ml, 3, out);
            for (int c = 0; c < D; c++) out[3 * (size_t)Ml + c] = h2[c];
            return BA_OK;
        }
        case BA_GET_S:
        case BA_GET_RHS: {
            if (iterative()) {
                if (what == BA_GET_S || n != (size_t)D) return BA_ERR_ARG;
                if ((rc = dl(d_pcg_b.p, (size_t)D, h))) return rc;
                for (int c = 0; c < D; c++) out[c] = h[c];
                return BA_OK;
            }
            if (!d_Skeep.p) return BA_ERR_ARG;
            if ((rc = dl(d_Skeep.p, d_Skeep.n, h))) return rc;
            if (what == BA_GET_RHS) {
                if (n != (size_t)D) return BA_ERR_ARG;
                for (int c = 0; c < D; c++) out[c] = h[(size_t)c * ld + D];
            } else {
                if (n != (size_t)D * D) return BA_ERR_ARG;
                for (int c = 0; c < D; c++)
                    for (int rr = c; rr < D; rr++) out[(size_t)c * D + rr] = out[(size_t)rr * D + c] = h[(size_t)c * ld + rr];
            }
            return BA_OK;
        }
        case 11: {
            if (!dense_qr() || n != (size_t)D || !d_qA.p) return BA_ERR_ARG;
            HIPCHK(hipStreamSynchronize(st));
            std::vector<T> col(1);
            for (int c = 0; c < D; c++) {
                HIPCHK(hipMemcpy(col.data(), d_qA.p + (size_t)c * q_lda + c, sizeof(T), hipMemcpyDeviceToHost));
                out[c] = (double)col[0];
            }
            return BA_OK;
        }
        case 14: {
            if (!dense_qr() || n != (size_t)2 * D || !d_dbg2.p) return BA_ERR_ARG;
            std::vector<T> hh;
            int rcg;
            if ((rcg = dl(d_dbg2.p, (size_t)2 * D, hh))) return rcg;
            for (int c = 0; c < 2 * D; c++) out[c] = (double)hh[c];
            return BA_OK;
        }
        case 15:
        case 16: {
            const size_t rows = (size_t)inner_rows();
            const T *src = what == 15 ? d_qAcopy.p : d_qA.p;
            if (!dense_qr() || n != rows * (D + 1) || !src) return BA_ERR_ARG;
            HIPCHK(hipStreamSynchronize(st));
            std::vector<T> col(rows);
            for (int c = 0; c <= D; c++) {
                HIPCHK(hipMemcpy(col.data(), src + (size_t)c * q_lda, sizeof(T) * rows, hipMemcpyDeviceToHost));
                for (size_t i = 0; i < rows; i++) out[(size_t)c * rows + i] = (double)col[i];
            }
            return BA_OK;
        }
        case 17: {
            if (!dense_qr() || n != (size_t)BA_QR_TAU_LEVELS * q_tau_stride || !d_qtau.p) return BA_ERR_ARG;
            std::vector<T> hh;
            int rcg;
            if ((rcg = dl(d_qtau.p, n, hh))) return rcg;
            for (size_t c = 0; c < n; c++) out[c] = (double)hh[c];
            return BA_OK;
        }
        case 12: {
            if (!dense_qr() || n != (size_t)D * (D + 1) || !d_qA.p) return BA_ERR_ARG;
            HIPCHK(hipStreamSynchronize(st));
            std::vector<T> col((size_t)D);
            for (int c = 0; c <= D; c++) {
                HIPCHK(hipMemcpy(col.data(), d_qA.p + (size_t)c * q_lda, sizeof(T) * (size_t)D, hipMemcpyDeviceToHost));
                for (int i = 0; i < D; i++) out[(size_t)c * D + i] = (c < D && i > c) ? 0.0 : (double)col[i];
            }
            return BA_OK;
        }
        case BA_GET_CAMS:
        case BA_GET_CAMS_TEST: {
            if (n != 15 * (size_t)N) return BA_ERR_ARG;
            if ((rc = dl(d_cam[what == BA_GET_CAMS ? 0 : 1].p, 15 * (size_t)N, h))) return rc;
            soa_to_aos(h, N, 15, out);
            return BA_OK;
        }
        case BA_GET_POINTS:
        case BA_GET_POINTS_TEST: {
            if (n != 3 * (size_t)Ml) return BA_ERR_ARG;
            if ((rc = dl(d_pts[what == BA_GET_POINTS ? 0 : 1].p, 3 * (size_t)Ml, h))) return rc;
            soa_to_aos(h, Ml, 3, out);
            return BA_OK;
        }
        }
        return BA_ERR_ARG;
    }

    int set_state(const double *cam15, const double *pts) override
    {
        const std::vector<T> h = cam15 ? aos_to_soa(cam15, N, 15) : std::vector<T>();
        if (cam15 && share_on() && !share_equal(sh.h_gptr, sh.h_members, h.data(), N)) return BA_ERR_ARG;
        HIPCHK(hipStreamSynchronize(st));
        cov_valid = false;
        have_lin = false;
        if (cam15) HIPCHK(hipMemcpy(d_cam[0].p, h.data(), sizeof(T) * h.size(), hipMemcpyHostToDevice));
        if (pts && Ml > 0) {
            const std::vector<T> hp = aos_to_soa(pts, Ml, 3);
            HIPCHK(hipMemcpy(d_pts[0].p, hp.data(), sizeof(T) * hp.size(), hipMemcpyHostToDevice));
        }
        have_step = false;
        return BA_OK;
    }

    static constexpr int LM_DEPTH = 3;

    int capture(hipGraphExec_t *g, int (Solver::*seg)())
    {
        if (*g) return BA_OK;
        hipGraph_t gr = nullptr;
        HIPCHK(hipStreamBeginCapture(st, hipStreamCaptureModeThreadLocal));
        const int rc = (this->*seg)();
        const hipError_t e = hipStreamEndCapture(st, &gr);
        if (rc) { if (gr) (void)hipGraphDestroy(gr); return rc; }
        if (e != hipSuccess) { fprintf(stderr, "ba_mi355x: hipStreamEndCapture: %s\n", hipGetErrorString(e)); return BA_ERR_HIP; }
        const hipError_t ei = hipGraphInstantiate(g, gr, nullptr, nullptr, 0);
        (void)hipGraphDestroy(gr);
        if (ei != hipSuccess) { *g = nullptr; return BA_ERR_HIP; }
        return BA_OK;
    }
    int launch_seg_ab() { int rc = launch_seg_a(); return rc ? rc : launch_seg_b(); }
    int launch_seg_iter() { int rc = launch_seg_ab(); return rc ? rc : launch_seg_ctl(); }

    int run_seg(hipGraphExec_t *g, int (Solver::*seg)(), bool graphs)
    {
        if (!graphs) return (this->*seg)();
        int rc = capture(g, seg);
        if (rc) return rc;
        HIPCHK(hipGraphLaunch(*g, st));
        return BA_OK;
    }

    int enqueue_trial(int slot, bool graphs)
    {
        int rc;
        EvSlot &e = ring[slot];
        if (spin_next_s > 0) {
            hipLaunchKernelGGL(k_spin, dim3(1), dim3(64), 0, st, (long long)(spin_next_s * wall_khz * 1e3));
            spin_next_s = 0;
        }
        if (!sharded())
            return run_seg(&g_trial, &Solver::launch_seg_iter, graphs);
        HIPCHK(hipEventRecord(e.e[0], st));
        {
            if ((rc = run_seg(&g_a, &Solver::launch_seg_a, graphs))) return rc;
            HIPCHK(hipEventRecord(e.e[1], st));
            if ((rc = exchange())) return rc;
            HIPCHK(hipEventRecord(e.e[2], st));
            if ((rc = run_seg(&g_b, &Solver::launch_seg_b, graphs && !dist_on()))) return rc;
            HIPCHK(hipEventRecord(e.e[3], st));
            if ((rc = allreduce(d_scal.p + SC_ETEST, N_STEP_SCALARS, 0))) return rc;
        }
        HIPCHK(hipEventRecord(e.e[4], st));
        if ((rc = run_seg(&g_ctl, &Solver::launch_seg_ctl, graphs))) return rc;
        if (more_qr() && (rc = more_outer_finish(&d_lm.p->go))) return rc;
        HIPCHK(hipEventRecord(e.e[5], st));
        return BA_OK;
    }

    void harvest(int slot, bool accepted)
    {
        EvSlot &e = ring[slot];
        tm.trial_ms += ev_ms(e.e[0], e.e[4]);
        if (sharded()) tm.comm_ms += ev_ms(e.e[1], e.e[2]) + ev_ms(e.e[3], e.e[4]);
        tm.n_trials++;
        tm.n_graph_trials++;
        if (accepted) { tm.linearize_ms += ev_ms(e.e[4], e.e[5]); tm.n_linearize++; }
    }

    int minimize(const ba_lm_params *lmp, ba_trial_cb cb, void *user, ba_result *out) override
    {
        if (poisoned) return BA_ERR_HIP;
        ba_lm_params lm;
        if (lmp) lm = *lmp; else ba_lm_params_default(&lm);
        const auto tbeg = std::chrono::steady_clock::now();
        const ba_timing tm0 = tm;
        const bool talk = lm.verbose && rank == 0;
        if (talk) {
            printf("############################## Backtrack LevMarq ###############################\n");
            printf("--------------------------------------------------------------------------------\n");
            printf(" Iter%15s%15s%15s%15s%15s\n", "Status", "f", "rho", "lambda", "Elapsed");
            printf("--------------------------------------------------------------------------------\n");
        }
        int rc = BA_OK;
        ba_lm_dev<T> h{};
        h.lam_min = (T)lm.lambda_min; h.lam_max = (T)lm.lambda_max; h.tol_fun = (T)lm.tol_fun; h.inc_base = (T)lm.lambda_increase_base;
        h.lambda = (T)lm.lambda_init; h.lambda_inc = h.inc_base;
        h.max_iter = lm.max_iter; h.max_fun_ev = lm.max_fun_ev; h.max_trials = lm.max_trials;
        h.status = BA_RUNNING;
        h.iter = 1;
        int launched = 0, consumed = 0, harvested = 0;
        std::vector<char> acc_of(RING_EV, 0);
        if (h.iter > lm.max_iter) { h.status = BA_MAX_ITERS; h.stop = 1; }
        else if (lm.max_trials < 0) { h.stop = 1; }
        else {
            double e = 0, dmax = 0;
            if ((rc = linearize(&e, damp_kind == BA_DAMP_MARQUARDT ? nullptr : &dmax))) return rc;
            h.energy = (T)e;
            h.fun_evals = 1;
            if (damp_kind != BA_DAMP_MARQUARDT) h.lambda = kind == BA_MOREQR ? (T)(1e-6 * std::sqrt(dmax)) : (T)(1e-12 * dmax);
        }
        if (!h.stop && dist_on() && (rc = dist_setup())) return rc;
        if (!h.stop && sharded() && !dense_qr() && !d_pack.p && (rc = d_pack.alloc(pack_count() + 1))) return rc;
        if (!h.stop && sharded() && dense_qr() && !d_qB.p && (rc = d_qB.alloc(qb_count()))) return rc;
        if (!h.stop) {
            h_log->done = 0; h_log->stop = 0; h_log->status = BA_RUNNING;
            if ((rc = set_lambda(h.lambda))) return rc;
            static_assert(SC_ERR == SC_GUARD + 1, "cleared together");
            HIPCHK(hipMemsetAsync(d_scal.p + SC_GUARD, 0, 2 * sizeof(T), st));
            HIPCHK(hipMemcpyAsync(d_lm.p, &h, sizeof h, hipMemcpyHostToDevice, st));
            HIPCHK(hipStreamSynchronize(st));
            const bool graphs = use_graph && st != nullptr;
            auto tlast = std::chrono::steady_clock::now();
            auto drain = [&]() {
                const int done = __atomic_load_n(&h_log->done, __ATOMIC_ACQUIRE);
                while (consumed < done) {
                    const ba_lm_row r = h_log->rows[consumed % BA_LM_RING];
                    const auto tnow = std::chrono::steady_clock::now();
                    const double el = std::chrono::duration<double>(tnow - tlast).count();
                    tlast = tnow;
                    acc_of[consumed % RING_EV] = r.accepted != 0;
                    consumed++;
                    if (r.stop == 2.0) continue;
                    if (!sharded()) {
                        tm.n_graph_trials++;
                        if (r.trial_ticks >= 0) { tm.trial_ms += r.trial_ticks / wall_khz; tm.n_trials++; }
                        if (r.ctl_ticks_prev >= 0 && r.prev_go != 0) { tm.linearize_ms += r.ctl_ticks_prev / wall_khz; tm.n_linearize++; }
                    }
                    if (cb) cb(user, (int)r.iter, (int)r.accepted, r.f, r.rho, r.lambda, el);
                    if (talk)
                        printf("%5d%15s%15g%15g%15g%14gs\n", (int)r.iter, r.accepted != 0 ? "Accepted" : "Rejected", r.f, r.rho, r.lambda, el);
                }
                while (harvested + 1 < consumed) { if (sharded()) harvest(harvested % RING_EV, acc_of[harvested % RING_EV]); harvested++; }
                return done;
            };
            for (int attempt = 0;; attempt++) {
                auto tprog = std::chrono::steady_clock::now();
                int seen = consumed;
                while (true) {
                    const int done = drain();
                    if (done != seen) { seen = done; tprog = std::chrono::steady_clock::now(); }
                    bool may = !(lm.max_trials > 0 && launched >= lm.max_trials), final = !may;
                    if (may && launched >= LM_DEPTH) {
                        const int need = launched - LM_DEPTH;
                        if (done <= need) may = false;
                        else if (h_log->rows[need % BA_LM_RING].stop != 0.0) { may = false; final = true; }
                    }
                    if (may) {
                        if ((rc = enqueue_trial(launched % RING_EV, graphs))) break;
                        launched++;
                        continue;
                    }
                    if (final) break;
                    if (std::chrono::duration<double>(std::chrono::steady_clock::now() - tprog).count() > watchdog_s) {
                        fprintf(stderr, "ba_mi355x: no LM trial completed within %g s -- giving up on this solver (nothing is freed)\n", watchdog_s);
                        poisoned = true;
                        return BA_ERR_HIP;
                    }
                    __builtin_ia32_pause();
                }
                if (!rc) {
                    const auto tw = std::chrono::steady_clock::now();
                    hipError_t eq;
                    while ((eq = hipStreamQuery(st)) == hipErrorNotReady) {
                        (void)drain();
                        if (std::chrono::duration<double>(std::chrono::steady_clock::now() - tw).count() > watchdog_s) {
                            fprintf(stderr, "ba_mi355x: the stream did not drain within %g s -- giving up on this solver (nothing is freed)\n", watchdog_s);
                            poisoned = true;
                            return BA_ERR_HIP;
                        }
                        __builtin_ia32_pause();
                    }
                    if (eq != hipSuccess) { fprintf(stderr, "ba_mi355x: %s\n", hipGetErrorString(eq)); return BA_ERR_HIP; }
                } else {
                    const hipError_t es = hipStreamSynchronize(st);
                    if (es != hipSuccess) { fprintf(stderr, "ba_mi355x: %s\n", hipGetErrorString(es)); return BA_ERR_HIP; }
                }
                drain();
                while (harvested < consumed) { if (sharded()) harvest(harvested % RING_EV, acc_of[harvested % RING_EV]); harvested++; }
                if (rc) return rc;
                HIPCHK(hipMemcpy(&h, d_lm.p, sizeof h, hipMemcpyDeviceToHost));
                if (h.status != BA_DEV_FAILED) break;
                report_device_error(h.deverr);
                if (h.deverr == BA_DEVERR_DIVERGED) return BA_ERR_COMM;
                if (safe_factor || attempt > 0) return BA_ERR_HIP;
                fprintf(stderr, "ba_mi355x: repeating LM trial %d with the launch-per-step factorisation\n", h.trials - 1);
                safe_factor = true;
                recoveries++;
                for (hipGraphExec_t *g : {&g_trial, &g_b})
                    if (*g) { (void)hipGraphExecDestroy(*g); *g = nullptr; }
                h.trials -= 1; h.fun_evals -= 1;
                h.status = BA_RUNNING; h.stop = 0; h.deverr = 0; h.go = 0; h.timed = 0; h.prev_go = 0;
                {
                    const T code = (T)h.prev_code;
                    *h_lam = code;
                    HIPCHK(hipMemcpyAsync(d_scal.p + SC_GUARD, h_lam, sizeof(T), hipMemcpyHostToDevice, st));
                    HIPCHK(hipMemsetAsync(d_scal.p + SC_ERR, 0, sizeof(T), st));
                }
                HIPCHK(hipMemcpyAsync(d_lm.p, &h, sizeof h, hipMemcpyHostToDevice, st));
                HIPCHK(hipStreamSynchronize(st));
                launched = consumed = harvested = h.trials;
                if (lm.max_trials > 0) {  }
                __atomic_store_n(&h_log->done, h.trials, __ATOMIC_RELEASE);
                h_log->stop = 0; h_log->status = BA_RUNNING;
            }
            if (h.fresh) {
                if ((rc = fetch_scalars())) return rc;
                if (sharded()) {
                    HIPCHK(hipMemcpyAsync(d_scal.p + SC_ENERGY, d_scal.p + SC_ELOC, sizeof(T), hipMemcpyDeviceToDevice, st));
                    if ((rc = allreduce(d_scal.p + SC_ENERGY, 1, 0)) || (rc = fetch_scalars())) return rc;
                }
                h.energy = h_scal[SC_ENERGY];
            }
            HIPCHK(hipGetLastError());
        }
        if (talk) printf("--------------------------------------------------------------------------------\n");
        have_step = false;
        cov_valid = false;
        have_lin = false;
        if (out) {
            out->status = h.status; out->iterations = h.iter; out->trials = h.trials; out->fun_evals = h.fun_evals;
            out->energy = (double)h.energy; out->lambda = (double)h.lambda;
            out->seconds = std::chrono::duration<double>(std::chrono::steady_clock::now() - tbeg).count();
            const long long nt = tm.n_trials - tm0.n_trials, nl = tm.n_linearize - tm0.n_linearize;
            out->schur_ms = nt ? (tm.trial_ms - tm0.trial_ms) / nt : 0.0;
            out->linearize_ms = nl ? (tm.linearize_ms - tm0.linearize_ms) / nl : 0.0;
        }
        return rc;
    }

    int selftest(int which) override
    {
        if (iterative() && which != 3) return BA_ERR_ARG;
        if (which == 2) {
            if ((D + NB - 1) / NB < 2 || safe_factor) return BA_ERR_ARG;
            fault_rowflag = 1;
            for (hipGraphExec_t *g : {&g_trial, &g_b})
                if (*g) { (void)hipGraphExecDestroy(*g); *g = nullptr; }
            return BA_OK;
        }
        if (which == 3) {
            spin_next_s = 4.0;
            return BA_OK;
        }
        if (which != 1) return BA_ERR_ARG;
        const int nblk = (D + NB - 1) / NB, groups = (nblk + 1) / 2;
        if (groups < 2 || 2 * groups > num_cus) return BA_ERR_ARG;
        hipLaunchKernelGGL((k_fill_sentinel<T>), dim3((2 * Dp + 2 * NB + 255) / 256), dim3(256), 0, st, 2 * Dp + 2 * NB, d_dxc.p);
        hipLaunchKernelGGL((k_ldlt_backflow<T, NB>), dim3(2 * groups), dim3(256), 0, st, D, ld, D, nblk, d_S.p, d_Winv.p, d_dxc.p, d_dxc.p + Dp,
                           d_scal.p + SC_ERR, 1 << 10, groups - 1);
        have_step = false;
        return fetch_scalars();
    }

    int time_phase(int phase, int reps, double lambda_d, double *ms) override
    {
        if (reps < 1 || !ms) return BA_ERR_ARG;
        if (iterative() && (phase == 3 || phase == 6 || phase == 7)) return BA_ERR_ARG;
        if ((phase == 9 || phase == 10) && !(iterative() && forest_on() && (phase == 10 || fo.width == 9))) return BA_ERR_ARG;
        double acc_ms = 0;
        int rcl = set_lambda((T)lambda_d);
        if (rcl) return rcl;
        HIPCHK(hipStreamSynchronize(st));
        HIPCHK(hipEventRecord(ev[EV_T0], st));
        for (int k = 0; k < reps; k++) {
            switch (phase) {
            case 0: launch_eval(false, 0); break;
            case 1: launch_linearisation(0, nullptr, false, false, nullptr, true); break;
            case 2: launch_eliminate(); break;
            case 3: launch_assemble(); break;
            case 4:
                if (iterative()) { launch_pcg_prep(); launch_pcg_solve(); break; }
                launch_assemble();
                if (dense_qr()) launch_qrkit_solve();
                else { launch_post_reduce(); launch_factor_solve(); }
                break;
            case 5: launch_backsub_retract(); break;
            case 8:
                launch_linearisation(0, nullptr, false,  true, nullptr,  !fuse);
                break;
            case 9: launch_forest_edges(); break;
            case 10:
                launch_pcg_blocks();
                if (fo.width == 9) launch_forest_edges();
                HIPCHK(hipEventRecord(ev[EV_T2], st));
                launch_forest_factor();
                HIPCHK(hipEventRecord(ev[EV_T3], st));
                HIPCHK(hipStreamSynchronize(st));
                acc_ms += ev_ms(EV_T2, EV_T3);
                break;
            case 6:
            case 7:
                launch_assemble();
                if (dense_qr()) {
                    HIPCHK(hipEventRecord(ev[EV_T2], st));
                    if (phase == 6) launch_qrkit_solve();
                    HIPCHK(hipEventRecord(ev[EV_T3], st));
                    HIPCHK(hipStreamSynchronize(st));
                    acc_ms += ev_ms(EV_T2, EV_T3);
                    break;
                }
                launch_post_reduce();
                if (phase == 6) HIPCHK(hipEventRecord(ev[EV_T2], st));
                launch_factor();
                if (phase == 6) HIPCHK(hipEventRecord(ev[EV_T3], st));
                if (phase == 7) HIPCHK(hipEventRecord(ev[EV_T2], st));
                launch_backsweep();
                if (phase == 7) HIPCHK(hipEventRecord(ev[EV_T3], st));
                HIPCHK(hipStreamSynchronize(st));
                acc_ms += ev_ms(EV_T2, EV_T3);
                break;
            default: return BA_ERR_ARG;
            }
        }
        HIPCHK(hipEventRecord(ev[EV_T1], st));
        HIPCHK(hipStreamSynchronize(st));
        HIPCHK(hipGetLastError());
        *ms = ((phase == 6 || phase == 7 || phase == 10) ? acc_ms : ev_ms(EV_T0, EV_T1)) / reps;
        have_step = false;
        return BA_OK;
    }
};

}

struct ba_solver {
    SolverBase *impl = nullptr;
};

extern "C" {

int ba_device_info(int device, char *name, size_t n, int *cus)
{
    int cnt = 0;
    if (hipGetDeviceCount(&cnt) != hipSuccess || cnt <= 0) return BA_ERR_HIP;
    if (device < 0) { if (hipGetDevice(&device) != hipSuccess) return BA_ERR_HIP; }
    if (device >= cnt) return BA_ERR_ARG;
    hipDeviceProp_t pr;
    if (hipGetDeviceProperties(&pr, device) != hipSuccess) return BA_ERR_HIP;
    if (name && n) { snprintf(name, n, "%s (%s)", pr.name, pr.gcnArchName); }
    if (cus) *cus = pr.multiProcessorCount;
    return BA_OK;
}

int ba_solver_create(const ba_problem *p, ba_solver_kind kind, ba_scalar scalar, int device, int shard_rank, int shard_world,
                     ba_solver **out)
{
    if (!p || !out || shard_world < 1 || shard_rank < 0 || shard_rank >= shard_world) return BA_ERR_ARG;
    if (kind != BA_QRKIT && kind != BA_QRCHOL && kind != BA_CHOLESKY && kind != BA_MOREQR && kind != BA_QRSPQR && kind != BA_ITERSCHUR) return BA_ERR_ARG;
    if (kind == BA_ITERSCHUR && shard_world > 1) return BA_ERR_ARG;
    if (scalar != BA_F64 && scalar != BA_F32) return BA_ERR_ARG;
    *out = nullptr;
    int cnt = 0;
    if (hipGetDeviceCount(&cnt) != hipSuccess || cnt <= 0) {
        fprintf(stderr, "ba_mi355x: no HIP device -- the solver has no CPU path\n");
        return BA_ERR_HIP;
    }
    if (device >= 0) {
        if (device >= cnt) return BA_ERR_ARG;
        HIPCHK(hipSetDevice(device));
    }
    SolverBase *impl = (scalar == BA_F64) ? (SolverBase *)new (std::nothrow) Solver<double>() : (SolverBase *)new (std::nothrow) Solver<float>();
    if (!impl) return BA_ERR_NOMEM;
    int rc = impl->init(p, kind, shard_rank, shard_world);
    if (rc) { delete impl; return rc; }
    ba_solver *s = new (std::nothrow) ba_solver;
    if (!s) { delete impl; return BA_ERR_NOMEM; }
    s->impl = impl;
    *out = s;
    return BA_OK;
}

void ba_solver_free(ba_solver *s)
{
    if (!s) return;
    if (!s->impl->poisoned) delete s->impl;
    delete s;
}

int ba_solver_recoveries(const ba_solver *s) { return s ? s->impl->recoveries : -1; }

int ba_solver_set_allreduce(ba_solver *s, ba_allreduce_fn fn, void *user)
{
    if (!s) return BA_ERR_ARG;
    s->impl->ar_fn = fn; s->impl->ar_user = user;
    return BA_OK;
}

int ba_solver_comm_init(ba_solver *s, const void *id)
{
// ... 129 lines not shown
```

Baseline: 1458 LM iterations/s.

## Prepare next trial's elimination and Schur pairs at tail of previous trial

Moves the point elimination and the Schur pair assembly of the next LM trial into the tail of the current trial's linearisation. The pair assembly is fused with the camera Gram kernel into one launch that splits its blocks between the two jobs. Non-head trials use a separate graph that skips the elimination and pair kernels. Device flags (asm_go, elim_skip) gate the work based on LM control decisions. This removes launches and lets the pair assembly overlap the Gram work, at the cost of more complex graph state and a risk of stale records when lambda changes.

```diff
diff --git a/bundleadjustment_benchmarks_amd/csrc/ba_internal.h b/bundleadjustment_benchmarks_amd/csrc/ba_internal.h
--- a/bundleadjustment_benchmarks_amd/csrc/ba_internal.h
+++ b/bundleadjustment_benchmarks_amd/csrc/ba_internal.h
@@ -64,6 +64,9 @@
 };
 void ba_plan_schur(const ba_structure &s, int wgs_per_cu, int num_cus, int bands, int window, ba_schur_plan &out);
 
+struct ba_tail_grid { int pair_wgs, gram_wgs; };
+inline ba_tail_grid ba_plan_tail_grid(int schur_grid, int ndchunks) { return ba_tail_grid{schur_grid, ndchunks > 0 ? (ndchunks + 7) / 8 : 0}; }
+
 struct ba_forest_plan {
     int ntrees = 0, nodes = 0, kept = 0, dropped = 0, largest = 0, width = 6;
     std::vector<int> tree_ptr, node_cam, node_par ;
diff --git a/bundleadjustment_benchmarks_amd/csrc/ba_kernels.hip.h b/bundleadjustment_benchmarks_amd/csrc/ba_kernels.hip.h
--- a/bundleadjustment_benchmarks_amd/csrc/ba_kernels.hip.h
+++ b/bundleadjustment_benchmarks_amd/csrc/ba_kernels.hip.h
@@ -522,11 +522,13 @@
     ba_point_prep_block<T>(blockIdx.x, Ml, K, pt_ptr, Jp, r, U0, gp, partial_dmax);
 }
 
-template <typename T>
+template <typename T, int PASSES = 2>
 __device__ __forceinline__ void ba_cam_gram_block(int bid, int ndchunks, int K, const int *__restrict__ dchunk_ptr, const int *__restrict__ cam_obs,
                                                   const T *__restrict__ JcA, T *__restrict__ dslab)
 {
-    __shared__ T xch[8][27][33];
+    static_assert(54 % PASSES == 0, "whole passes");
+    constexpr int ROWS = 54 / PASSES;
+    __shared__ T xch[8][ROWS][33];
     const int gl = threadIdx.x >> 5, g = bid * 8 + gl, sub = threadIdx.x & 31;
     const bool gok = g < ndchunks;
     const int e0 = gok ? dchunk_ptr[g] : 0, len = gok ? dchunk_ptr[g + 1] - e0 : 0;
@@ -548,16 +550,16 @@
         for (int c = 0; c < 9; c++) v[45 + c] = -(a0[c] * r0 + a1[c] * r1);
     }
 #pragma unroll
-    for (int pass = 0; pass < 2; pass++) {
+    for (int pass = 0; pass < PASSES; pass++) {
         __syncthreads();
 #pragma unroll
-        for (int q = 0; q < 27; q++) xch[gl][q][sub] = v[27 * pass + q];
+        for (int q = 0; q < ROWS; q++) xch[gl][q][sub] = v[ROWS * pass + q];
         __syncthreads();
-        if (gok && sub < 27) {
+        if (gok && sub < ROWS) {
             T a = 0;
 #pragma unroll
             for (int l = 0; l < 32; l++) a += xch[gl][sub][l];
-            dslab[(size_t)g * BA_SLAB + 27 * pass + sub] = a;
+            dslab[(size_t)g * BA_SLAB + ROWS * pass + sub] = a;
         }
     }
 }
@@ -1018,100 +1020,32 @@
                                                      const T *__restrict__ tvec, int Ml, T *__restrict__ slab, const T *__restrict__ V,
                                                      const T *__restrict__ gc, int D, int ld, T *__restrict__ S)
 {
-    const int lane = threadIdx.x & 63;
-    const int wq = ((blockIdx.x % nband) * (gridDim.x / nband) + blockIdx.x / nband) * 4 + (threadIdx.x >> 6);
-    int slot = wave_ptr[wq];
-    const int slot1 = wave_ptr[wq + 1];
-    if (slot >= slot1) return;
-    const __amdgpu_buffer_rsrc_t rsrc = __builtin_amdgcn_make_buffer_rsrc(const_cast<T *>(rec), 0, (int)rec_bytes, 0x00020000);
-    constexpr unsigned SZ = sizeof(T), RB = BA_REC * SZ, OOB = 0xfffffff0u - 64 * SZ;
-    const int i = lane & 15, k = lane >> 4;
-    const bool la = i < 9;
-    const unsigned lane_off = 3 * i * SZ;
-    typedef typename ba_acc<T>::type acc_t;
-    auto entry_of = [&](const int4 ci) {
-        const int n = ci.y & 0xffff;
-        return ent[ci.x + (lane < n ? lane : n - 1)];
-    };
-    int4 ci0 = chunk_info[slot];
-    int4 ci1 = chunk_info[min(slot + 1, slot1 - 1)];
-    int2 en0 = entry_of(ci0);
-    for (; slot < slot1; slot++) {
-        const int2 en1 = entry_of(ci1);
-        const int4 ci2 = chunk_info[min(slot + 2, slot1 - 1)];
-        const int n = ci0.y & 0xffff;
-        const int hi = ci0.z & 0xffff, lo = (unsigned)ci0.z >> 16, g = ci0.w;
-        const bool diag = hi == lo;
-        const int ia_l = en0.x, ib_l = en0.y;
-        acc_t acc;
-#pragma unroll
-        for (int v = 0; v < 4; v++) acc[v] = 0;
-        constexpr int GB = 2;
-        struct batch_t { T a[3 * GB], d[3 * GB], b[3 * GB]; };
-        auto fetch = [&](int t0, batch_t &o) {
-#pragma unroll
-            for (int u = 0; u < GB; u++) {
-                const int e = 4 * (t0 + u) + k;
-                const bool ok = e < n;
-                const int es = ok ? e : n - 1;
-                const int ia = __shfl(ia_l, es, 64), ibr = __shfl(ib_l, es, 64);
-                const bool self = ibr < 0;
-                const unsigned ra = (unsigned)ia * RB, rb = (unsigned)(self ? ia : ibr) * RB;
-                const unsigned oa = (ok && la) ? ra + lane_off : OOB, ob = (ok && la) ? rb + lane_off : OOB;
-                const unsigned od = (ok && la) ? ra + BA_REC_DINV * SZ : OOB;
-                ba_bufload3(rsrc, oa, o.a[3 * u], o.a[3 * u + 1], o.a[3 * u + 2]);
-                if (SCALED) ba_bufload3(rsrc, od, o.d[3 * u], o.d[3 * u + 1], o.d[3 * u + 2]);
-                ba_bufload3(rsrc, ob, o.b[3 * u], o.b[3 * u + 1], o.b[3 * u + 2]);
-                if (diag && i == 9 && ok && self) {
-#pragma unroll
-                    for (int m = 0; m < 3; m++) o.b[3 * u + m] = tvec[(size_t)m * Ml + (~ibr)];
-                }
-            }
-        };
-        auto multiply = [&](const batch_t &o) {
-#pragma unroll
-            for (int q = 0; q < 3 * GB; q++) acc = ba_mfma(SCALED ? o.a[q] * o.d[q] : o.a[q], o.b[q], acc);
-        };
-        const int ngroups = (n + 3) >> 2;
-        batch_t b0, b1;
-        fetch(0, b0);
-        for (int t0 = 0;;) {
-            if (t0 + GB < ngroups) fetch(t0 + GB, b1);
-            multiply(b0);
-            t0 += GB;
-            if (t0 >= ngroups) break;
-            if (t0 + GB < ngroups) fetch(t0 + GB, b0);
-            multiply(b1);
-            t0 += GB;
-            if (t0 >= ngroups) break;
-        }
-        if (ci0.y & BA_CHUNK_SINGLE) {
-#pragma unroll
-            for (int v = 0; v < 4; v++) {
-                const int r = ba_crow<T>(k, v);
-                if (r >= 9) continue;
-                if (i < 9) {
-                    T val = -acc[v];
-                    if (diag) val += V[(size_t)hi * 81 + 9 * r + i];
-                    S[(size_t)(9 * lo + i) * ld + 9 * hi + r] = val;
-                } else if (i == 9 && diag) {
-                    const T gg = gc[9 * hi + r];
-                    S[(size_t)(9 * hi + r) * ld + D] = gg - acc[v];
-                    S[(size_t)(9 * hi + r) * ld + D + 1] = gg;
-                }
-            }
-        } else {
-            T *o = slab + (size_t)g * BA_SLAB;
-#pragma unroll
-            for (int v = 0; v < 4; v++) {
-                const int r = ba_crow<T>(k, v);
-                if (r >= 9) continue;
-                if (i < 9) o[9 * r + i] = acc[v];
-                else if (i == 9) o[81 + r] = acc[v];
-            }
-        }
-        ci0 = ci1; ci1 = ci2; en0 = en1;
-    }
+#define BA_PAIRS_BLOCK blockIdx.x
+#define BA_PAIRS_GRID gridDim.x
+#include "ba_schur_pairs_body.hip.h"
+#undef BA_PAIRS_BLOCK
+#undef BA_PAIRS_GRID
+}
+
+template <typename T>
+__global__ __launch_bounds__(256) __attribute__((amdgpu_waves_per_eu(4))) void k_pairs_gram(int npw, const int *__restrict__ asm_go, const int *__restrict__ wave_ptr, int nband,
+                                                    const int4 *__restrict__ chunk_info, const int2 *__restrict__ ent, const T *__restrict__ rec,
+                                                    unsigned rec_bytes, const T *__restrict__ tvec, int Ml, T *__restrict__ slab, const T *__restrict__ V,
+                                                    const T *__restrict__ gc, int D, int ld, T *__restrict__ S, const int *__restrict__ go, int ndchunks,
+                                                    int K, const int *__restrict__ dchunk_ptr, const int *__restrict__ cam_obs, const T *__restrict__ JcA,
+                                                    T *__restrict__ dslab)
+{
+    if ((int)blockIdx.x >= npw) {
+        if (*go != 0) ba_cam_gram_block<T, 3>(blockIdx.x - npw, ndchunks, K, dchunk_ptr, cam_obs, JcA, dslab);
+        return;
+    }
+    if (*asm_go == 0) return;
+    constexpr bool SCALED = true;
+#define BA_PAIRS_BLOCK blockIdx.x
+#define BA_PAIRS_GRID ((unsigned)npw)
+#include "ba_schur_pairs_body.hip.h"
+#undef BA_PAIRS_BLOCK
+#undef BA_PAIRS_GRID
 }
 
 template <typename T, bool MARQ = false>
@@ -1421,6 +1355,7 @@
     int prev_go;
     int prev_code;
     int rec_fresh;
+    int asm_go, elim_skip;
 };
 struct ba_lm_row { double iter, accepted, f, rho, lambda, lambda_used, e_test, dx_norm, trial_ticks, ctl_ticks_prev, prev_go, stop; };
 struct ba_lm_host { int done, stop, status, pad; ba_lm_row rows[BA_LM_RING]; };
@@ -1523,6 +1458,8 @@
     scal[sl.lambda] = s.lambda;
     row.stop = failed ? 2.0 : (s.stop ? 1.0 : 0.0);
     s.rec_fresh = 0;
+    s.asm_go = s.stop ? 0 : 1;
+    s.elim_skip = (go || s.stop) ? 1 : 0;
     *lm = s;
     host->rows[t % BA_LM_RING] = row;
     host->stop = s.stop;
diff --git a/bundleadjustment_benchmarks_amd/csrc/ba_schur_pairs_body.hip.h b/bundleadjustment_benchmarks_amd/csrc/ba_schur_pairs_body.hip.h
--- /dev/null
+++ b/bundleadjustment_benchmarks_amd/csrc/ba_schur_pairs_body.hip.h
@@ -0,0 +1,94 @@
+    const int lane = threadIdx.x & 63;
+    const int wq = ((BA_PAIRS_BLOCK % nband) * (BA_PAIRS_GRID / nband) + BA_PAIRS_BLOCK / nband) * 4 + (threadIdx.x >> 6);
+    int slot = wave_ptr[wq];
+    const int slot1 = wave_ptr[wq + 1];
+    if (slot >= slot1) return;
+    const __amdgpu_buffer_rsrc_t rsrc = __builtin_amdgcn_make_buffer_rsrc(const_cast<T *>(rec), 0, (int)rec_bytes, 0x00020000);
+    constexpr unsigned SZ = sizeof(T), RB = BA_REC * SZ, OOB = 0xfffffff0u - 64 * SZ;
+    const int i = lane & 15, k = lane >> 4;
+    const bool la = i < 9;
+    const unsigned lane_off = 3 * i * SZ;
+    typedef typename ba_acc<T>::type acc_t;
+    auto entry_of = [&](const int4 ci) {
+        const int n = ci.y & 0xffff;
+        return ent[ci.x + (lane < n ? lane : n - 1)];
+    };
+    int4 ci0 = chunk_info[slot];
+    int4 ci1 = chunk_info[min(slot + 1, slot1 - 1)];
+    int2 en0 = entry_of(ci0);
+    for (; slot < slot1; slot++) {
+        const int2 en1 = entry_of(ci1);
+        const int4 ci2 = chunk_info[min(slot + 2, slot1 - 1)];
+        const int n = ci0.y & 0xffff;
+        const int hi = ci0.z & 0xffff, lo = (unsigned)ci0.z >> 16, g = ci0.w;
+        const bool diag = hi == lo;
+        const int ia_l = en0.x, ib_l = en0.y;
+        acc_t acc;
+#pragma unroll
+        for (int v = 0; v < 4; v++) acc[v] = 0;
+        constexpr int GB = 2;
+        struct batch_t { T a[3 * GB], d[3 * GB], b[3 * GB]; };
+        auto fetch = [&](int t0, batch_t &o) {
+#pragma unroll
+            for (int u = 0; u < GB; u++) {
+                const int e = 4 * (t0 + u) + k;
+                const bool ok = e < n;
+                const int es = ok ? e : n - 1;
+                const int ia = __shfl(ia_l, es, 64), ibr = __shfl(ib_l, es, 64);
+                const bool self = ibr < 0;
+                const unsigned ra = (unsigned)ia * RB, rb = (unsigned)(self ? ia : ibr) * RB;
+                const unsigned oa = (ok && la) ? ra + lane_off : OOB, ob = (ok && la) ? rb + lane_off : OOB;
+                const unsigned od = (ok && la) ? ra + BA_REC_DINV * SZ : OOB;
+                ba_bufload3(rsrc, oa, o.a[3 * u], o.a[3 * u + 1], o.a[3 * u + 2]);
+                if (SCALED) ba_bufload3(rsrc, od, o.d[3 * u], o.d[3 * u + 1], o.d[3 * u + 2]);
+                ba_bufload3(rsrc, ob, o.b[3 * u], o.b[3 * u + 1], o.b[3 * u + 2]);
+                if (diag && i == 9 && ok && self) {
+#pragma unroll
+                    for (int m = 0; m < 3; m++) o.b[3 * u + m] = tvec[(size_t)m * Ml + (~ibr)];
+                }
+            }
+        };
+        auto multiply = [&](const batch_t &o) {
+#pragma unroll
+            for (int q = 0; q < 3 * GB; q++) acc = ba_mfma(SCALED ? o.a[q] * o.d[q] : o.a[q], o.b[q], acc);
+        };
+        const int ngroups = (n + 3) >> 2;
+        batch_t b0, b1;
+        fetch(0, b0);
+        for (int t0 = 0;;) {
+            if (t0 + GB < ngroups) fetch(t0 + GB, b1);
+            multiply(b0);
+            t0 += GB;
+            if (t0 >= ngroups) break;
+            if (t0 + GB < ngroups) fetch(t0 + GB, b0);
+            multiply(b1);
+            t0 += GB;
+            if (t0 >= ngroups) break;
+        }
+        if (ci0.y & BA_CHUNK_SINGLE) {
+#pragma unroll
+            for (int v = 0; v < 4; v++) {
+                const int r = ba_crow<T>(k, v);
+                if (r >= 9) continue;
+                if (i < 9) {
+                    T val = -acc[v];
+                    if (diag) val += V[(size_t)hi * 81 + 9 * r + i];
+                    S[(size_t)(9 * lo + i) * ld + 9 * hi + r] = val;
+                } else if (i == 9 && diag) {
+                    const T gg = gc[9 * hi + r];
+                    S[(size_t)(9 * hi + r) * ld + D] = gg - acc[v];
+                    S[(size_t)(9 * hi + r) * ld + D + 1] = gg;
+                }
+            }
+        } else {
+            T *o = slab + (size_t)g * BA_SLAB;
+#pragma unroll
+            for (int v = 0; v < 4; v++) {
+                const int r = ba_crow<T>(k, v);
+                if (r >= 9) continue;
+                if (i < 9) o[9 * r + i] = acc[v];
+                else if (i == 9) o[81 + r] = acc[v];
+            }
+        }
+        ci0 = ci1; ci1 = ci2; en0 = en1;
+    }
diff --git a/bundleadjustment_benchmarks_amd/csrc/ba_solver.hip b/bundleadjustment_benchmarks_amd/csrc/ba_solver.hip
--- a/bundleadjustment_benchmarks_amd/csrc/ba_solver.hip
+++ b/bundleadjustment_benchmarks_amd/csrc/ba_solver.hip
@@ -172,6 +172,7 @@
     int schur_window = 0;
     int nred = 0;
     bool no_fold = false;
+    bool trial_head = false;
     bool rec_coop = true;
     int schur_grid = 1, schur_wgs = 4 , schur_bands = 8, schur_nband = 1;
     DevBuf<T> d_r, d_Jc, d_Jp, d_JcA, d_U0, d_gp, d_V, d_gc, d_rec0, d_dinv0, d_tvec0, d_tri0;
@@ -204,7 +205,8 @@
     ba_lm_host *h_log = nullptr, *d_log = nullptr;
     T h_scal[NSCAL];
     T *h_lam = nullptr;
-    hipGraphExec_t g_trial = nullptr, g_a = nullptr, g_b = nullptr, g_ctl = nullptr;
+    hipGraphExec_t g_trial = nullptr, g_trial_nh = nullptr, g_a = nullptr, g_b = nullptr, g_ctl = nullptr;
+    bool seg_head = true;
     bool use_graph = true;
     hipEvent_t ev[EV_N] = {};
     struct EvSlot { hipEvent_t e[RING_NE]; };
@@ -275,6 +277,7 @@
         HIPCHK(hipHostGetDevicePointer((void **)&d_log, (void *)h_log, 0));
         use_graph = getenv("BA_NO_GRAPH") == nullptr;
         no_fold = getenv("BA_NO_FOLD") != nullptr;
+        trial_head = getenv("BA_TRIAL_HEAD") != nullptr && atoi(getenv("BA_TRIAL_HEAD")) != 0;
         rec_coop = getenv("BA_REC_PLAIN") == nullptr;
         dbg_qrcheck = getenv("BA_DBG_QRCHECK") != nullptr;
         dist_factor = getenv("BA_DIST_FACTOR") != nullptr && atoi(getenv("BA_DIST_FACTOR")) != 0;
@@ -485,9 +488,18 @@
         else linearisation(int_c<0>{}, soa);
     }
 
-    void launch_grad(const int *go = nullptr, const ba_red_job *tail = nullptr, bool points = true )
-    {
-        if (!points) {
+    void launch_grad(const int *go = nullptr, const ba_red_job *tail = nullptr, bool points = true ,
+                     bool next_trial = false)
+    {
+        if (next_trial) {
+            if constexpr (sizeof(T) == 8) {
+                launch_eliminate(&d_lm.p->elim_skip);
+                const ba_tail_grid tg = ba_plan_tail_grid(schur_grid, sx.ndchunks);
+                hipLaunchKernelGGL((k_pairs_gram<T>), dim3(tg.pair_wgs + tg.gram_wgs), dim3(256), 0, st, tg.pair_wgs, (const int *)&d_lm.p->asm_go, d_wave_ptr.p,
+                                   schur_nband, d_chunk_info.p, d_ent.p, d_rec.p, (unsigned)(sizeof(T) * d_rec.n), d_tvec.p, Ml, d_slab.p, d_V.p, d_gc.p, D, ld,
+                                   d_S.p, go, sx.ndchunks, Kl, d_dchunk_ptr.p, d_cam_obs.p, d_JcA.p, d_dslab.p);
+            }
+        } else if (!points) {
             if (sx.ndchunks > 0)
                 hipLaunchKernelGGL((k_cam_gram<T>), dim3((sx.ndchunks + 7) / 8), dim3(256), 0, st, sx.ndchunks, Kl,
                                    d_dchunk_ptr.p, d_cam_obs.p, d_JcA.p, d_dslab.p, go);
@@ -504,10 +516,10 @@
                            d_dslab.p, d_V.p, d_gc.p, go, tail ? *tail : ba_red_job{nullptr, 0, 0, 0}, d_scal.p, tail ? &d_lm.p->t_end : (long long *)nullptr);
     }
 
-    void launch_linearisation(int which, const int *go, bool commit, bool fused, const ba_red_job *tail, bool points)
+    void launch_linearisation(int which, const int *go, bool commit, bool fused, const ba_red_job *tail, bool points, bool next_trial = false)
     {
         launch_eval(true, which, go, commit, fused);
-        launch_grad(go, tail, points);
+        launch_grad(go, tail, points, next_trial);
         if (priors()) launch_prior(true, which, go);
         if (relposes()) launch_relpose(true, which, go);
     }
@@ -534,7 +546,7 @@
         return BA_OK;
     }
 
-    int linearize_enqueue(bool want_dmax, const int *go)
+    int linearize_enqueue(bool want_dmax, const int *go, bool next_trial = false)
     {
         int rc;
         if (!go) HIPCHK(hipEventRecord(ev[EV_L0], st));
@@ -543,7 +555,7 @@
         jobs.j[nj++] = {d_part_e.p, gE + 3 * gP + 2 * gR, 0, sharded() ? SC_ELOC : SC_ENERGY};
         const bool tail = go != nullptr && !want_dmax && kind != BA_MOREQR && !priors() && !relposes();
         const bool fz = fuse && go != nullptr && !want_dmax;
-        launch_linearisation(go ? 1 : 0, go, go != nullptr, fz, tail ? &jobs.j[0] : nullptr, !fz);
+        launch_linearisation(go ? 1 : 0, go, go != nullptr, fz, tail ? &jobs.j[0] : nullptr, !fz, next_trial);
         if (kind == BA_MOREQR) {
             launch_elim_qr(d_scal.p + SC_ZERO, d_rec0.p, d_dinv0.p, d_tvec0.p, d_tri0.p, go,  more_qr());
             if (more_qr() && (rc = launch_more_outer(go))) return rc;
@@ -562,13 +574,13 @@
         return BA_OK;
     }
 
-    void launch_eliminate()
+    void launch_eliminate(const int *skip = nullptr)
     {
         if (chol_elim()) {
             with_flags(marq(), rec_coop, [&](auto MARQ, auto COOP) {
                 hipLaunchKernelGGL((k_elim_chol<T, MARQ(), COOP()>), dim3(gK), dim3(256), 0, st, Kl, Ml, d_obs_pt.p, d_pt_ptr.p, d_JcA.p, d_Jp.p,
                                    d_U0.p, d_gp.p, d_scal.p + SC_LAMBDA, d_rec.p, d_dinv.p, d_tvec.p, d_tri.p,
-                                   fused_records() ? (const int *)&d_lm.p->rec_fresh : (const int *)nullptr, damp_args());
+                                   skip ? skip : fused_records() ? (const int *)&d_lm.p->rec_fresh : (const int *)nullptr, damp_args());
             });
         } else if (kind == BA_MOREQR) {
             if (Kl > 0)
@@ -599,10 +611,10 @@
     bool post_folded() const { return !sharded() && nred > 0 && !no_fold; }
     bool ctl_reduces() const { return !sharded() && !no_fold; }
 
-    void launch_schur()
+    void launch_schur(bool pairs = true)
     {
         const T *lamf = post_folded() ? d_scal.p + SC_LAMBDA : nullptr;
-        if (sx.nchunks > 0) {
+        if (pairs && sx.nchunks > 0) {
             const dim3 gp(schur_grid);
 #define BA_PAIRS(SC) hipLaunchKernelGGL((k_schur_pairs<T, SC>), gp, dim3(256), 0, st, d_wave_ptr.p, schur_nband, d_chunk_info.p, d_ent.p, d_rec.p, \
                                                   (unsigned)(sizeof(T) * d_rec.n), d_tvec.p, Ml, d_slab.p, d_V.p, d_gc.p, D, ld, d_S.p)
@@ -1163,7 +1175,7 @@
     }
     void drop_trial_graphs()
     {
-        for (hipGraphExec_t *g : {&g_trial, &g_a, &g_b, &g_ctl})
+        for (hipGraphExec_t *g : {&g_trial, &g_trial_nh, &g_a, &g_b, &g_ctl})
             if (*g) { (void)hipGraphExecDestroy(*g); *g = nullptr; }
     }
     int pcg_stats(ba_pcg_stats *out, int reset) override
@@ -1835,15 +1847,21 @@
         return BA_OK;
     }
 
-    void launch_assemble() { if (dense_qr()) launch_qrkit_build(); else launch_schur(); }
+    void launch_assemble(bool pairs = true) { if (dense_qr()) launch_qrkit_build(); else launch_schur(pairs); }
+    bool tail_prepares() const
+    {
+        return !trial_head && kind == BA_CHOLESKY && sizeof(T) == 8 && fused_records() && !sharded() && !relposes() && !masked && post_folded() &&
+               sx.nchunks > 0 && sx.ndchunks > 0;
+    }
     int mark(int e) { if (step_level) HIPCHK(hipEventRecord(ev[e], st)); return BA_OK; }
     int launch_seg_a()
     {
         int rc;
-        launch_eliminate();
+        const bool head = seg_head || !tail_prepares();
+        if (head) launch_eliminate();
         if ((rc = mark(EV_T1))) return rc;
         if (iterative()) { launch_pcg_prep(); return mark(EV_T2); }
-        launch_assemble();
+        launch_assemble(head);
         if ((rc = mark(EV_T2))) return rc;
         if (dense_qr()) return sharded() ? launch_qr_stack_pack() : BA_OK;
         if (dist_on()) return launch_dist_pack();
@@ -1890,7 +1908,7 @@
     {
         ba_lm_slots sl{SC_ENERGY, SC_ETEST, SC_RHO_P, SC_RHO_C, SC_DN_P, SC_DN_C, SC_LAMBDA, SC_ERR, SC_GUARD, world};
         hipLaunchKernelGGL((k_lm_control<T>), dim3(1), dim3(256 * BA_LM_JOBS), 0, st, d_scal.p, d_lm.p, d_log, sl, test_energy_jobs(), ctl_reduces() ? 3 : 0);
-        int rc = linearize_enqueue(false, &d_lm.p->go);
+        int rc = linearize_enqueue(false, &d_lm.p->go, tail_prepares());
         if (!rc && more_qr() && !sharded()) rc = more_outer_finish(&d_lm.p->go);
         return rc;
     }
@@ -2145,7 +2163,7 @@
         return BA_OK;
     }
 
-    int enqueue_trial(int slot, bool graphs)
+    int enqueue_trial(int slot, bool graphs, bool head)
     {
         int rc;
         EvSlot &e = ring[slot];
@@ -2154,7 +2172,12 @@
             spin_next_s = 0;
         }
         if (!sharded())
-            return run_seg(&g_trial, &Solver::launch_seg_iter, graphs);
+        {
+            seg_head = head || !tail_prepares();
+            rc = run_seg(seg_head ? &g_trial : &g_trial_nh, &Solver::launch_seg_iter, graphs);
+            seg_head = true;
+            return rc;
+        }
         HIPCHK(hipEventRecord(e.e[0], st));
         {
             if ((rc = run_seg(&g_a, &Solver::launch_seg_a, graphs))) return rc;
@@ -2250,6 +2273,7 @@
             };
             for (int attempt = 0;; attempt++) {
                 auto tprog = std::chrono::steady_clock::now();
+                bool head = true;
                 int seen = consumed;
                 while (true) {
                     const int done = drain();
@@ -2261,7 +2285,8 @@
                         else if (h_log->rows[need % BA_LM_RING].stop != 0.0) { may = false; final = true; }
                     }
                     if (may) {
-                        if ((rc = enqueue_trial(launched % RING_EV, graphs))) break;
+                        if ((rc = enqueue_trial(launched % RING_EV, graphs, head))) break;
+                        head = false;
                         launched++;
                         continue;
                     }
@@ -2301,7 +2326,7 @@
                 fprintf(stderr, "ba_mi355x: repeating LM trial %d with the launch-per-step factorisation\n", h.trials - 1);
                 safe_factor = true;
                 recoveries++;
-                for (hipGraphExec_t *g : {&g_trial, &g_b})
+                for (hipGraphExec_t *g : {&g_trial, &g_trial_nh, &g_b})
                     if (*g) { (void)hipGraphExecDestroy(*g); *g = nullptr; }
                 h.trials -= 1; h.fun_evals -= 1;
                 h.status = BA_RUNNING; h.stop = 0; h.deverr = 0; h.go = 0; h.timed = 0; h.prev_go = 0;
@@ -2349,7 +2374,7 @@
         if (which == 2) {
             if ((D + NB - 1) / NB < 2 || safe_factor) return BA_ERR_ARG;
             fault_rowflag = 1;
-            for (hipGraphExec_t *g : {&g_trial, &g_b})
+            for (hipGraphExec_t *g : {&g_trial, &g_trial_nh, &g_b})
                 if (*g) { (void)hipGraphExecDestroy(*g); *g = nullptr; }
             return BA_OK;
         }
```

Result: faster. 1480 LM iterations/s (median of 6 runs) (+1.5%).
